# CarloLucibello/GraphNeuralNetworks.jl

Measured on AMD Instinct MI355X. Metric: edges/sec (fwd) GCNConv+GATConv, ogbn-products-shape; achieved HBM GB/s vs peak, higher is better.
Workload: dtype f32; 1 GPU; products-shape power-law graph N=2449029 E=61859140 (+N self loops, E'=64308169), D=100: GCNConv(100=>100,relu) fwd + GATConv(100=>16,heads=8,relu) fwd per step; edges counted = 2*E' per GPU; parallelism=replicas x1 (independent feature batches, no collective)

## Files before the change

graphneuralnetworks.jl_amd/csrc/common.h:

```cpp
#pragma once
#include <hip/hip_runtime.h>

#include <memory>
#include <mutex>
#include <stdint.h>
#include <type_traits>
#include "gnnmp.h"
#include "headgeom.h"
#include "knobs.h"

namespace gnnmp {

int fail(int status, const char *fmt, ...);
int hip_fail(hipError_t e, const char *what);

#define GNNMP_HIP(expr)                                         \
    do {                                                        \
        hipError_t e__ = (expr);                                \
        if (e__ != hipSuccess) return ::gnnmp::hip_fail(e__, #expr); \
    } while (0)

#define GNNMP_TRY(expr)                                         \
    do {                                                        \
        const int rc__ = (expr);                                \
        if (rc__ != GNNMP_OK) return rc__;                      \
    } while (0)

#define GNNMP_LAUNCH_CHECK(what)                                \
    do {                                                        \
        hipError_t e__ = hipGetLastError();                     \
        if (e__ != hipSuccess) return ::gnnmp::hip_fail(e__, what); \
    } while (0)

constexpr int GNNMP_MAX_DEVICES = 32;
int current_device();

struct DeviceOnce {
    std::mutex m;
    unsigned char done[GNNMP_MAX_DEVICES] = {};
    hipError_t err[GNNMP_MAX_DEVICES] = {};
};
template <class F>
inline hipError_t device_once(DeviceOnce &o, F &&f) {
    const int dev = current_device();
    std::lock_guard<std::mutex> lk(o.m);
    if (!o.done[dev]) {
        o.err[dev] = f();
        o.done[dev] = 1;
    }
    return o.err[dev];
}

#define GNNMP_LDS_OPTIN(what, ...)                                                                                            \
    do {                                                                                                                      \
        static ::gnnmp::DeviceOnce once__;                                                                                    \
        const hipError_t err__ = ::gnnmp::device_once(once__, [] {                                                            \
            return hipFuncSetAttribute(reinterpret_cast<const void *>(__VA_ARGS__), hipFuncAttributeMaxDynamicSharedMemorySize, \
                                       160 * 1024);                                                                           \
        });                                                                                                                   \
        if (err__ != hipSuccess) return ::gnnmp::hip_fail(err__, "hipFuncSetAttribute(" what ")");                            \
    } while (0)

int knob(int k);
static_assert(KNOB_FUSED_WAVES == 14 && KNOB_TGCN == 20 && KNOB_EDGE_DOT_GRAD == 21 && KNOB_HETERO == 22, "knobs.h: indices never change");
inline int block_waves(int auto_value) {
    const int w = knob(KNOB_BLOCK_WAVES);
    return w >= 1 && w <= 4 ? w : auto_value;
}
int device_cus();

__device__ __forceinline__ int64_t load_index(const void *p, int64_t k, int idx_bytes, int base) {
    return idx_bytes == 8 ? (reinterpret_cast<const int64_t *>(p)[k] - base)
                          : (static_cast<int64_t>(reinterpret_cast<const int32_t *>(p)[k]) - base);
}
__device__ __forceinline__ void store_index(void *p, int64_t k, int idx_bytes, int64_t v) {
    if (idx_bytes == 8)
        reinterpret_cast<int64_t *>(p)[k] = v;
    else
        reinterpret_cast<int32_t *>(p)[k] = static_cast<int32_t>(v);
}

__host__ __device__ __forceinline__ uint32_t drop_mix32(uint32_t x) {
    x ^= x >> 16; x *= 0x7feb352du; x ^= x >> 15; x *= 0x846ca68bu; x ^= x >> 16;
    return x;
}
__host__ __device__ __forceinline__ uint32_t drop_bits(uint32_t seed_lo, uint32_t seed_hi, uint32_t e, uint32_t h) {
    return drop_mix32(drop_mix32(e ^ seed_lo) ^ (h * 0x9e3779b9u + seed_hi));
}
struct DropArgs {
    uint32_t thr;
    uint32_t seed_lo, seed_hi;
    float inv;
};
__host__ __forceinline__ DropArgs make_drop(float p, uint64_t seed) {
    DropArgs d;
    const double t = (double)p * 4294967296.0;
    d.thr = t >= 4294967295.0 ? 0xffffffffu : (uint32_t)t;
    d.seed_lo = (uint32_t)seed;
    d.seed_hi = (uint32_t)(seed >> 32);
    d.inv = 1.0f / (1.0f - p);
    return d;
}
__device__ __forceinline__ float softmax_exp(float x) { return __builtin_amdgcn_exp2f(x * 1.44269504088896341f); }

__device__ __forceinline__ float hw_max(float x, float y) {
    float r;
    asm("v_max_f32 %0, %1, %2" : "=v"(r) : "v"(x), "v"(y));
    return r;
}
__device__ __forceinline__ float hw_min(float x, float y) {
    float r;
    asm("v_min_f32 %0, %1, %2" : "=v"(r) : "v"(x), "v"(y));
    return r;
}
__device__ __forceinline__ float jl_max(float x, float y) {
    const float m = hw_max(x, y);
    const float nan_pick = (x != x) ? x : y;
    return __builtin_isunordered(x, y) ? nan_pick : m;
}
__device__ __forceinline__ float jl_min(float x, float y) {
    const float m = hw_min(x, y);
    const float nan_pick = (x != x) ? x : y;
    return __builtin_isunordered(x, y) ? nan_pick : m;
}

enum { OP_SUM = 0, OP_MAX = 1, OP_MIN = 2 };

template <int OP>
__device__ __forceinline__ float op_identity() {
    return OP == OP_SUM ? 0.0f : (OP == OP_MAX ? -__builtin_inff() : __builtin_inff());
}
template <int OP>
__device__ __forceinline__ float op_apply(float a, float b) {
    if (OP == OP_SUM) return a + b;
    if (OP == OP_MAX) return jl_max(a, b);
    return jl_min(a, b);
}

template <int VEC>
struct Vec;
template <>
struct Vec<4> {
    using T = float4;
    static __device__ __forceinline__ void load(const float *p, float v[4]) {
        float4 t = *reinterpret_cast<const float4 *>(p);
        v[0] = t.x; v[1] = t.y; v[2] = t.z; v[3] = t.w;
    }
    static __device__ __forceinline__ void store(float *p, const float v[4]) {
        *reinterpret_cast<float4 *>(p) = make_float4(v[0], v[1], v[2], v[3]);
    }
};
template <>
struct Vec<2> {
    using T = float2;
    static __device__ __forceinline__ void load(const float *p, float v[2]) {
        float2 t = *reinterpret_cast<const float2 *>(p);
        v[0] = t.x; v[1] = t.y;
    }
    static __device__ __forceinline__ void store(float *p, const float v[2]) {
        *reinterpret_cast<float2 *>(p) = make_float2(v[0], v[1]);
    }
};
template <>
struct Vec<1> {
    using T = float;
    static __device__ __forceinline__ void load(const float *p, float v[1]) { v[0] = *p; }
    static __device__ __forceinline__ void store(float *p, const float v[1]) { *p = v[0]; }
};

#if defined(__HIP_DEVICE_COMPILE__) && !(defined(__gfx942__) || defined(__gfx950__))
#error "libgnnmp's cross-workgroup fold (coh_store / coh_load / coh_publish) relies on gfx942 / gfx950 semantics of s_waitcnt vmcnt and sc1; build with ARCH=gfx950"
#endif
template <int VEC>
__device__ __forceinline__ void coh_store(float *p, const float v[VEC]) {
    if (VEC == 1) {
        __hip_atomic_store(reinterpret_cast<unsigned int *>(p), __float_as_uint(v[0]), __ATOMIC_RELAXED, __HIP_MEMORY_SCOPE_AGENT);
    } else {
#pragma unroll
        for (int q = 0; q < VEC; q += 2) {
            const unsigned long long b = (unsigned long long)__float_as_uint(v[q]) | ((unsigned long long)__float_as_uint(v[q + 1 < VEC ? q + 1 : q]) << 32);
            __hip_atomic_store(reinterpret_cast<unsigned long long *>(p + q), b, __ATOMIC_RELAXED, __HIP_MEMORY_SCOPE_AGENT);
        }
    }
}
template <int VEC>
__device__ __forceinline__ void coh_load(const float *p, float v[VEC]) {
    if (VEC == 1) {
        v[0] = __uint_as_float(__hip_atomic_load(reinterpret_cast<const unsigned int *>(p), __ATOMIC_RELAXED, __HIP_MEMORY_SCOPE_AGENT));
    } else {
#pragma unroll
        for (int q = 0; q < VEC; q += 2) {
            const unsigned long long b = __hip_atomic_load(reinterpret_cast<const unsigned long long *>(p + q), __ATOMIC_RELAXED, __HIP_MEMORY_SCOPE_AGENT);
            v[q] = __uint_as_float((unsigned int)b);
            if (q + 1 < VEC) v[q + 1] = __uint_as_float((unsigned int)(b >> 32));
        }
    }
}
__device__ __forceinline__ void coh_store1(float *p, float v) {
    __hip_atomic_store(reinterpret_cast<unsigned int *>(p), __float_as_uint(v), __ATOMIC_RELAXED, __HIP_MEMORY_SCOPE_AGENT);
}
__device__ __forceinline__ float coh_load1(const float *p) {
    return __uint_as_float(__hip_atomic_load(reinterpret_cast<const unsigned int *>(p), __ATOMIC_RELAXED, __HIP_MEMORY_SCOPE_AGENT));
}
__device__ __forceinline__ void coh_publish() { asm volatile("s_waitcnt vmcnt(0) lgkmcnt(0)" ::: "memory"); }

template <int CTRL>
__device__ __forceinline__ float dpp_mov(float v) {
    return __int_as_float(__builtin_amdgcn_update_dpp(0, __float_as_int(v), CTRL, 0xf, 0xf, true));
}
template <int LPH>
__device__ __forceinline__ float group_sum(float d, int lph) {
    if (LPH == 0) {
        if (lph & 0x10000) {
            const int n = lph & 0xff, G = 1 << ((lph >> 8) & 0xff);
            const int lane = (int)__lane_id(), lig = lane & (G - 1);
            const int hb = lane - lig + (lig / n) * n;
            float s = 0.0f;
            for (int k = 0; k < n; ++k) s += __shfl(d, hb + k, 64);
            return s;
        }
        for (int o = 1; o < lph; o <<= 1) d += __shfl_xor(d, o, 64);
        return d;
    }
    if (LPH >= 2) d += dpp_mov<0xB1>(d);
    if (LPH >= 4) d += dpp_mov<0x4E>(d);
    if (LPH >= 8) d += dpp_mov<0x141>(d);
    if (LPH >= 16) d += dpp_mov<0x140>(d);
    if (LPH >= 32) d += __shfl_xor(d, 16, 64);
    if (LPH >= 64) d += __shfl_xor(d, 32, 64);
    return d;
}

__device__ __forceinline__ int xcd_remap(int b, int cpx, int enabled) {
    return enabled ? (b & 7) * cpx + (b >> 3) : b;
}
__device__ __forceinline__ int xcd_remap_after(int b, int nbc, int cpx) {
    return b < nbc ? b : nbc + (b & 7) * cpx + ((b - nbc) >> 3);
}

}

struct gnnmp_graph {
    int64_t n_src = 0, n_dst = 0, n_edges = 0, n_total = 0;
    int self_loops = 0;
    uint32_t *rowptr = nullptr;
    int32_t *col = nullptr;
    int32_t *eid = nullptr;
    int32_t *long_rows = nullptr;
    int32_t *long_cptr = nullptr;
    int32_t *chunk_row = nullptr;
    uint32_t *chunk_beg = nullptr;
    uint32_t *chunk_end = nullptr;
    int n_long = 0;
    int n_chunks = 0;
    int long_thresh = GNNMP_LONG_ROW;
    int64_t max_degree = 0;
    int64_t bytes = 0;
    float *ws = nullptr;
    size_t ws_floats = 0;
    uint32_t *ticket = nullptr;
    int32_t *row_order = nullptr;
    int32_t *chunk_lrow = nullptr;
    uint32_t *arrive = nullptr;
    size_t arrive_n = 0;
    float *spart = nullptr;
    size_t spart_floats = 0;
    void *block = nullptr;
    size_t block_bytes = 0;
    int32_t *status = nullptr;
};

namespace gnnmp {
struct __attribute__((visibility("hidden"))) PlanDeleter {
    void operator()(gnnmp_graph *p) const { (void)gnnmp_plan_destroy(p); }
};
using PlanPtr = std::unique_ptr<gnnmp_graph, PlanDeleter>;
int ensure_workspace(gnnmp_graph *p, size_t floats);
int ensure_arrive(gnnmp_graph *p, size_t n, size_t floats, hipStream_t stream);
bool fold_disabled_by_env();
inline bool use_fold() { return (knob(KNOB_VARIANT) & VARIANT_TWO_KERNEL_FOLD) == 0 && !fold_disabled_by_env(); }
int ensure_ticket(gnnmp_graph *p, hipStream_t stream);
int ensure_row_order(gnnmp_graph *p, hipStream_t stream);
int plan_build_long_rows(gnnmp_graph *p, hipStream_t stream);
int plan_long_thresh(int64_t Etot);
}

namespace gnnmp {
inline int pick_vec(int64_t D, const void *a, const void *b) {
    uintptr_t m = reinterpret_cast<uintptr_t>(a) | reinterpret_cast<uintptr_t>(b);
    int forced = knob(KNOB_FORCE_VEC);
    int v = 1;
    if (D % 4 == 0 && (m & 15) == 0)
        v = 4;
    else if (D % 2 == 0 && (m & 7) == 0)
        v = 2;
    if (forced == 1 || forced == 2 || forced == 4) {
        if (forced <= v) v = forced;
    }
    return v;
}
inline bool use_xcd_remap(int64_t n_src, int64_t D, int64_t chunks) {
    const int k = knob(KNOB_XCD_REMAP);
    if (k == 0 || chunks < 64) return false;
    if (k == 2) return true;
    return n_src * D * (int64_t)sizeof(float) <= ((int64_t)128 << 20);
}
inline bool use_row_order(int64_t n_src, int64_t D) {
    const int k = knob(KNOB_ROW_ORDER);
    if (k == 0) return false;
    if (k == 2) return true;
    return n_src * D * (int64_t)sizeof(float) > ((int64_t)128 << 20);
}
inline int pick_log2g(int64_t lanes_needed) {
    int forced = knob(KNOB_FORCE_LOG2G);
    if (forced >= 0 && forced <= 6) return forced;
    int l = 0;
    while ((1 << l) < lanes_needed && l < 6) ++l;
    return l;
}
inline int feature_tiles(int64_t D, int vec, int log2g) {
    const int64_t G = (int64_t)1 << log2g;
    return (int)(((D + vec - 1) / vec + G - 1) / G);
}
template <class... P>
inline int narrow_vec(int vec, const P *...ptr) {
    uintptr_t m = 0;
    ((m |= reinterpret_cast<uintptr_t>(ptr)), ...);
    return (m & (uintptr_t)(4 * vec - 1)) != 0 ? 1 : vec;
}
template <int V>
using int_c = std::integral_constant<int, V>;
template <class F>
inline auto with_vec(int vec, F &&f) {
    switch (vec) {
        case 4: return f(int_c<4>{});
        case 2: return f(int_c<2>{});
        default: return f(int_c<1>{});
    }
}
template <int VEC, int MAX, class F>
inline auto with_lph(int lph, F &&f) {
    if constexpr (VEC == 4) {
        switch (lph <= MAX ? lph : 0) {
            case 1: return f(int_c<1>{});
            case 2: return f(int_c<2>{});
            case 4: return f(int_c<4>{});
            case 8: return f(int_c<8>{});
            case 16: return f(int_c<16>{});
            case 32: return f(int_c<(MAX >= 32 ? 32 : 0)>{});
            case 64: return f(int_c<(MAX >= 64 ? 64 : 0)>{});
        }
    }
    return f(int_c<0>{});
}
template <class F>
inline auto with_op(int op, F &&f) {
    switch (op) {
        case OP_SUM: return f(int_c<OP_SUM>{});
        case OP_MAX: return f(int_c<OP_MAX>{});
        default: return f(int_c<OP_MIN>{});
    }
}
template <class F>
inline auto with_log2g(int log2g, F &&f) {
    switch (log2g) {
        case 0: return f(int_c<0>{});
        case 1: return f(int_c<1>{});
        case 2: return f(int_c<2>{});
        case 3: return f(int_c<3>{});
        case 4: return f(int_c<4>{});
        case 5: return f(int_c<5>{});
        default: return f(int_c<6>{});
    }
}
}
```

graphneuralnetworks.jl_amd/csrc/knobs.h:

```cpp
#pragma once

#define GNNMP_KNOB_TABLE(X)                                                                                                          \
    X(FORCE_VEC, 0, 0, "0 = auto, else 1|2|4")                                                                                       \
    X(FORCE_LOG2G, 1, -1, "-1 = auto, else 0..6")                                                                                    \
    X(UNROLL, 2, 0, "0 = auto (8: measured best on both bench shapes), else 2|4|8")                                                  \
    X(XCD_REMAP, 3, 1, "0 = off, 1 = auto (default: only when the gathered matrix fits the Infinity Cache), 2 = on")                 \
    X(LONG_ROW, 4, 0, "long-row threshold (0 = auto, at most GNNMP_LONG_ROW)")                                                       \
    X(BLOCK_WAVES, 5, 0, "waves per block in the row kernels: 0 = auto (propagate 4, GAT 1), else 1..4")                             \
    X(DENSE_GENERIC, 6, 0, "0 = auto (dense_plan's whole order, dense_route.h), any other value = never dense_wreg, dense_split, "    \
                           "dense_t16 or dense_narrow (the round-1 kernels only); 1 = not the W-resident 32x32x2 kernel either: "     \
                           "K-chunked on every shape")                                                                               \
    X(DENSE_PREFETCH, 7, 17, "W-resident dense kernel scheduling: bit 4 = per-SIMD matrix-pipe token, low 4 bits = start skew of "   \
                             "waves 4-7 in s_sleep(127) units.  Default 17 (token + 1): 0.83 -> 0.72 ms at 2.4M x 100 => 100.  "     \
                             "Bit 5 = turn the cross-tile register prefetch OFF (on by default; its first version spilled, 270 "     \
                             "VGPRs, and was slower: see dense.hip)")                                                                \
    X(GAT_FAST_EXP, 8, 0, "reserved (retired: the one-pass attention kernel always uses v_exp_f32 now, gat_fused.hip gexp)")         \
    X(GRADW_SLABS, 9, 0, "dW kernel: slabs per CU (0 = auto)")                                                                       \
    X(GRADW_RP, 10, 0, "dW kernel: 0 = the 16x16x4 kernel, < 0 = the round-1 32x32x2 kernel (A/B runs)")                             \
    X(GRADW_MIN_ROWS, 11, 0, "dW kernel: rows-per-slab floor (0 = auto: ~3 slabs per CU on small inputs, 512 on large)")             \
    X(DENSE_T16_WAVES, 12, 0, "dense_t16_kernel: waves per block (0 = auto, else 1..16)")                                            \
    X(T16_DEBUG, 13, 0, "GNNMP_EXPERIMENTS builds only (gnnmp_tune refuses a non-zero value otherwise): phase ablation of "          \
                        "dense_t16_kernel / fused_cat_kernel (1 = no stores, 2 = no x loads, ...: the results are garbage), and the " \
                        "variant number of dense_split_kernel")                                                                      \
    X(FUSED_WAVES, 14, 0, "fused_conv_kernel: 0 = auto (as many waves as LDS holds tiles for, <= 16), > 0 = cap, < 0 = never fuse "  \
                          "- read by the host too (gnnmp/layers.py)")                                                                \
    X(ROW_ORDER, 15, 0, "rows by decreasing length in the row kernels that share a wave between rows: 0 = never, 1 = when the "      \
                        "gathered matrix exceeds the Infinity Cache, 2 = always (use_row_order)")                                    \
    X(SOFTMAX_ROWS, 16, 0, "one-pass narrow-row softmax (softmax_rows.hip): 0 = auto, < 0 = the three-step kernels on every row")    \
    X(DENSE_SPLIT, 17, 0, "split-bf16 dense core (msplit.h, dense_split.hip): 0 = auto (on for its shapes), < 0 = the fp32-MFMA "    \
                          "kernels of rounds 1-2 on every shape")                                                                    \
    X(CHAIN, 18, 0, "fused GraphConv chain kernel (graph_chain.hip): 0 = auto, < 0 = never (layer-by-layer path)")                   \
    X(VARIANT, 19, 0, "A/B switches, a bit field of the VARIANT_* constants below (all variants are correct code)")                  \
    X(TGCN, 20, 0, "TGCN recurrence (temporal.hip): 0 = auto (the one-launch kernel for out <= 128), < 0 = the per-step path (dense " \
                   "launches + the step pointwise kernels, every out) - read by the host layer (gnnmp/layers_temporal.py)")          \
    X(EDGE_DOT_GRAD, 21, 0, "adjoint of the per-edge dot product (linkpred.hip): 0 = auto (the fused kernel for D <= 256), < 0 = "   \
                            "two w_mul_xj propagates (plan and transposed plan) plus an add - read by the host (gnnmp/linkpred.py)") \
    X(HETERO, 22, 0, "heterograph aggregation (hetero.hip): 0 = auto (one hetero_rows_kernel launch per layer, and "                 \
                     "HeteroGraphConv's transform-first path), < 0 = the composition: propagate per relation, then the same kernel " \
                     "over identity relations as the combiner, the A/B baseline - read by the host (gnnmp/hetero.py)")               \
    X(CHUNK_SLOTS, 23, 0, "slots per chunk of a split row, read at plan build (plan.hip: plan_chunk_slots): 0 or anything below "    \
                          "16 = the default of 128; the plan's long-row threshold still caps it")

namespace gnnmp {

enum Knob {
#define GNNMP_KNOB_ENUM(name, index, def, doc) KNOB_##name = index,
    GNNMP_KNOB_TABLE(GNNMP_KNOB_ENUM)
#undef GNNMP_KNOB_ENUM
#define GNNMP_KNOB_ONE(name, index, def, doc) +1
    KNOB_COUNT = 0 GNNMP_KNOB_TABLE(GNNMP_KNOB_ONE)
#undef GNNMP_KNOB_ONE
};

enum Variant {
    VARIANT_CHAIN_WAVES_MASK = 3,
    VARIANT_CHAIN_8_WAVES = 1,
    VARIANT_SPLIT_SERIAL_TILES = 16,
    VARIANT_SPLIT_DIRECT_STORES = 32,
    VARIANT_NO_WREG = 64,
    VARIANT_TWO_KERNEL_FOLD = 128,
    VARIANT_WREG_SMALL = 512,
};

}

#ifdef GNNMP_EXPERIMENTS
#define GNNMP_ABLATION(bits) (bits)
#else
#define GNNMP_ABLATION(bits) 0
#endif
```

graphneuralnetworks.jl_amd/csrc/plan.hip:

```cpp
#include <cstring>
#include <algorithm>
#include <vector>

#include "common.h"
#include "launch.h"
#include "pool.h"
#include "scratch.h"
#include "sort_scan.h"

namespace gnnmp {

int ensure_workspace(gnnmp_graph *p, size_t floats) { return grow(p->ws, p->ws_floats, floats, "hipMalloc(plan workspace)"); }

int ensure_arrive(gnnmp_graph *p, size_t n, size_t floats, hipStream_t stream) {
    GNNMP_TRY(grow(p->spart, p->spart_floats, floats, "hipMalloc(plan slice partials)"));
    if (n <= p->arrive_n) return GNNMP_OK;
    GNNMP_TRY(grow(p->arrive, p->arrive_n, n, "hipMalloc(plan arrival counters)"));
    const hipError_t e = hipMemsetAsync(p->arrive, 0, sizeof(uint32_t) * n, stream);
    if (e != hipSuccess) {
        p->arrive_n = 0;
        return hip_fail(e, "hipMemsetAsync(plan arrival counters)");
    }
    return GNNMP_OK;
}

int ensure_ticket(gnnmp_graph *p, hipStream_t stream) {
    if (p->ticket) return GNNMP_OK;
    size_t cap = 0;
    GNNMP_TRY(grow(p->ticket, cap, 2, "hipMalloc(plan ticket)"));
    const hipError_t e = hipMemsetAsync(p->ticket, 0, 2 * sizeof(uint32_t), stream);
    if (e != hipSuccess) return hip_fail(e, "hipMemsetAsync(plan ticket)");
    return GNNMP_OK;
}

__global__ void plan_degree_keys(const uint32_t *rowptr, int64_t n, uint32_t maxdeg, uint32_t *keys, uint32_t *vals) {
    int64_t i = (int64_t)blockIdx.x * blockDim.x + threadIdx.x;
    if (i >= n) return;
    keys[i] = maxdeg - (rowptr[i + 1] - rowptr[i]);
    vals[i] = (uint32_t)i;
}

int ensure_row_order(gnnmp_graph *p, hipStream_t stream) {
    if (p->row_order || p->n_dst == 0) return GNNMP_OK;
    const size_t n = (size_t)p->n_dst;
    unsigned bits = 1;
    while (bits < 32 && ((int64_t)1 << bits) <= p->max_degree) ++bits;
    DevBuf<int32_t> order;
    DevBuf<uint32_t> vin, kout, kin;
    hipError_t e = hipSuccess;
    if ((e = kin.alloc(n)) != hipSuccess || (e = kout.alloc(n)) != hipSuccess || (e = vin.alloc(n)) != hipSuccess ||
        (e = order.alloc(n)) != hipSuccess)
        return hip_fail(e, "hipMalloc(row order)");
    plan_degree_keys<<<(unsigned)((n + 255) / 256), 256, 0, stream>>>(p->rowptr, p->n_dst, (uint32_t)p->max_degree, kin.get(), vin.get());
    GNNMP_TRY(radix_sort_pairs_u32(kin.get(), kout.get(), vin.get(), reinterpret_cast<uint32_t *>(order.get()), n, 0, (int)bits,
                                   stream));
    p->row_order = order.release();
    p->bytes += (int64_t)(4 * n);
    return GNNMP_OK;
}


__global__ void plan_fill_keys(const void *src, const void *dst, int idx_bytes, int base, int64_t E,
                               int64_t Etot, int64_t n_src, int64_t n_dst, uint32_t *keys,
                               uint32_t *vals, int *bad) {
    int64_t k = (int64_t)blockIdx.x * blockDim.x + threadIdx.x;
    if (k >= Etot) return;
    int64_t d;
    if (k < E) {
        d = load_index(dst, k, idx_bytes, base);
        int64_t s = load_index(src, k, idx_bytes, base);
        if (d < 0 || d >= n_dst || s < 0 || s >= n_src) {
            *bad = 1;
            d = 0;
        }
    } else {
        d = k - E;
    }
    keys[k] = (uint32_t)d;
    vals[k] = (uint32_t)k;
}

__global__ void plan_rowptr(const uint32_t *keys, int64_t Etot, int64_t n_dst, uint32_t *rowptr) {
    int64_t i = (int64_t)blockIdx.x * blockDim.x + threadIdx.x;
    if (i > n_dst) return;
    int64_t lo = 0, hi = Etot;
    while (lo < hi) {
        int64_t mid = (lo + hi) >> 1;
        if ((int64_t)keys[mid] < i)
            lo = mid + 1;
        else
            hi = mid;
    }
    rowptr[i] = (uint32_t)lo;
}

__global__ void plan_col(const void *src, int idx_bytes, int base, int64_t E, int64_t Etot,
                         const uint32_t *eid, int32_t *col) {
    int64_t p = (int64_t)blockIdx.x * blockDim.x + threadIdx.x;
    if (p >= Etot) return;
    int64_t e = eid[p];
    int64_t s = e < E ? load_index(src, e, idx_bytes, base) : e - E;
    col[p] = (int32_t)s;
}

__global__ void csc_rowptr_kernel(const void *colptr, int idx_bytes, int base, int64_t n_dst, int64_t E, uint32_t *rowptr, int *bad) {
    int64_t i = (int64_t)blockIdx.x * blockDim.x + threadIdx.x;
    if (i > n_dst) return;
    const int64_t v = load_index(colptr, i, idx_bytes, base);
    bool ok = v >= 0 && v <= E;
    if (i == 0) ok = ok && v == 0;
    if (i == n_dst) ok = ok && v == E;
    if (i < n_dst) ok = ok && load_index(colptr, i + 1, idx_bytes, base) >= v;
    if (!ok) *bad = 1;
    rowptr[i] = (uint32_t)(ok ? v : (i == n_dst ? E : 0));
}
__global__ void csc_col_kernel(const void *rowval, int idx_bytes, int base, int64_t E, int64_t n_src, int32_t *col, int32_t *eid, int *bad) {
    int64_t p = (int64_t)blockIdx.x * blockDim.x + threadIdx.x;
    if (p >= E) return;
    int64_t s = load_index(rowval, p, idx_bytes, base);
    if (s < 0 || s >= n_src) {
        *bad = 1;
        s = 0;
    }
    col[p] = (int32_t)s;
    eid[p] = (int32_t)(uint32_t)p;
}

__global__ void plan_long_rows(const uint32_t *rowptr, int64_t n_dst, int thresh, int64_t *list,
                               int cap, int *count, unsigned long long *maxdeg) {
    int64_t i = (int64_t)blockIdx.x * blockDim.x + threadIdx.x;
    if (i >= n_dst) return;
    const int64_t beg = rowptr[i], end = rowptr[i + 1];
    const int64_t len = end - beg;
    if (len > 0) atomicMax(maxdeg, (unsigned long long)len);
    if (len > thresh) {
        int pos = atomicAdd(count, 1);
        if (pos < cap) {
            list[3 * pos] = i;
            list[3 * pos + 1] = beg;
            list[3 * pos + 2] = end;
        }
    }
}
__global__ void widen_u32_kernel(const uint32_t *in, int64_t n, int64_t *out) {
    int64_t i = (int64_t)blockIdx.x * blockDim.x + threadIdx.x;
    if (i < n) out[i] = (int64_t)in[i];
}

__global__ void slot_gather_kernel(const int32_t *idx, const float *v, int64_t Etot, int64_t n_valid,
                                   float *out) {
    int64_t p = (int64_t)blockIdx.x * blockDim.x + threadIdx.x;
    if (p >= Etot) return;
    const int64_t k = (uint32_t)idx[p];
    out[p] = k < n_valid ? v[k] : 1.0f;
}

__global__ void self_loops_kernel(const void *src, const void *dst, int idx_bytes, int base,
                                  int64_t E, int64_t n, void *out_src, void *out_dst,
                                  const float *w, float *out_w) {
    int64_t k = (int64_t)blockIdx.x * blockDim.x + threadIdx.x;
    if (k >= E + n) return;
    if (k < E) {
        store_index(out_src, k, idx_bytes, load_index(src, k, idx_bytes, 0));
        store_index(out_dst, k, idx_bytes, load_index(dst, k, idx_bytes, 0));
        if (out_w) out_w[k] = w[k];
    } else {
        int64_t v = (k - E) + base;
        store_index(out_src, k, idx_bytes, v);
        store_index(out_dst, k, idx_bytes, v);
        if (out_w) out_w[k] = 1.0f;
    }
}

__global__ void batch_edges_kernel(const void *src, const void *dst, int idx_bytes,
                                   const int64_t *edge_ptr, const int64_t *node_ptr, int64_t G,
                                   int64_t Etot, void *out_src, void *out_dst) {
    int64_t k = (int64_t)blockIdx.x * blockDim.x + threadIdx.x;
    if (k >= Etot) return;
    int64_t lo = 0, hi = G;
    while (hi - lo > 1) {
        int64_t mid = (lo + hi) >> 1;
        if (edge_ptr[mid] <= k)
            lo = mid;
        else
            hi = mid;
    }
    int64_t off = node_ptr[lo];
    store_index(out_src, k, idx_bytes, load_index(src, k, idx_bytes, 0) + off);
    store_index(out_dst, k, idx_bytes, load_index(dst, k, idx_bytes, 0) + off);
}
__global__ void batch_indicator_kernel(const int64_t *node_ptr, int64_t G, int64_t Ntot,
                                       int idx_bytes, int base, void *gi) {
    int64_t v = (int64_t)blockIdx.x * blockDim.x + threadIdx.x;
    if (v >= Ntot) return;
    int64_t lo = 0, hi = G;
    while (hi - lo > 1) {
        int64_t mid = (lo + hi) >> 1;
        if (node_ptr[mid] <= v)
            lo = mid;
        else
            hi = mid;
    }
    store_index(gi, v, idx_bytes, lo + base);
}

static inline unsigned nblocks(int64_t n, int bs) { return (unsigned)((n + bs - 1) / bs); }

int plan_long_thresh(int64_t Etot) {
    if (knob(KNOB_LONG_ROW) > 0) return knob(KNOB_LONG_ROW);
    int th = GNNMP_MIN_LONG_ROW;
    while (th < GNNMP_LONG_ROW && (double)th < 4e-5 * (double)Etot) th <<= 1;
    return th;
}

static int plan_chunk_slots() {
    const int v = knob(KNOB_CHUNK_SLOTS);
    return v >= 16 ? v : 128;
}

int plan_build_long_rows(gnnmp_graph *p, hipStream_t stream) {
    const int64_t n_dst = p->n_dst, Etot = p->n_total;
    const int BS = 256;
    const int cap = (int)std::min<int64_t>(Etot / std::max(1, p->long_thresh) + 1, n_dst + 1);
    DevBuf<int64_t> long_tmp;
    DevBuf<int> flags;
    GNNMP_HIP(flags.alloc(4));
    GNNMP_HIP(hipMemsetAsync(flags.get(), 0, sizeof(int) * 4, stream));
    GNNMP_HIP(long_tmp.alloc(3 * (size_t)std::max(cap, 1)));
    if (n_dst > 0) {
        plan_long_rows<<<nblocks(n_dst, BS), BS, 0, stream>>>(p->rowptr, n_dst, p->long_thresh, long_tmp.get(), cap, flags.get(),
                                                              reinterpret_cast<unsigned long long *>(flags.get() + 2));
        GNNMP_HIP(hipGetLastError());
    }
    int meta[4] = {0, 0, 0, 0};
    GNNMP_HIP(hipMemcpyAsync(meta, flags.get(), sizeof(int) * 4, hipMemcpyDeviceToHost, stream));
    GNNMP_HIP(hipStreamSynchronize(stream));
    unsigned long long md;
    memcpy(&md, meta + 2, sizeof(md));
    p->max_degree = (int64_t)md;
    p->n_long = std::min(meta[0], cap);
    if (p->n_long == 0) return GNNMP_OK;
    struct Tri { int64_t row, beg, end; };
    std::vector<Tri> h((size_t)p->n_long);
    GNNMP_HIP(hipMemcpy(h.data(), long_tmp.get(), sizeof(Tri) * h.size(), hipMemcpyDeviceToHost));
    std::sort(h.begin(), h.end(), [](const Tri &a, const Tri &b) { return a.row < b.row; });
    std::vector<int32_t> rows, cptr, crow, clrow;
    std::vector<uint32_t> cbeg, cend;
    cptr.push_back(0);
    const int64_t clen = std::min<int64_t>(p->long_thresh, plan_chunk_slots());
    for (const Tri &t : h) {
        const int64_t len = t.end - t.beg;
        const int64_t nch = (len + clen - 1) / clen;
        const int64_t csz = (len + nch - 1) / nch;
        for (int64_t c = 0; c < nch; ++c) {
            crow.push_back((int32_t)t.row);
            clrow.push_back((int32_t)rows.size());
            cbeg.push_back((uint32_t)(t.beg + c * csz));
            cend.push_back((uint32_t)std::min(t.beg + (c + 1) * csz, t.end));
        }
        rows.push_back((int32_t)t.row);
        cptr.push_back((int32_t)crow.size());
    }
    if (crow.size() >= (size_t)INT32_MAX)
        return fail(GNNMP_EUNSUPPORTED, "plan_create: %zu chunks of split rows exceed the int32 chunk index", crow.size());
    p->n_chunks = (int)crow.size();
    auto upload = [&](auto *&dst, const auto &v) -> hipError_t {
        const size_t bytes = sizeof(v[0]) * v.size();
        const hipError_t e = alloc_into(dst, v.size());
        if (e != hipSuccess) return e;
        p->bytes += (int64_t)bytes;
        return hipMemcpy(dst, v.data(), bytes, hipMemcpyHostToDevice);
    };
    GNNMP_HIP(upload(p->long_rows, rows));
    GNNMP_HIP(upload(p->long_cptr, cptr));
    GNNMP_HIP(upload(p->chunk_row, crow));
    GNNMP_HIP(upload(p->chunk_lrow, clrow));
    GNNMP_HIP(upload(p->chunk_beg, cbeg));
    GNNMP_HIP(upload(p->chunk_end, cend));
    return GNNMP_OK;
}

}

using namespace gnnmp;

extern "C" {

int gnnmp_plan_destroy(gnnmp_graph_t *p) { return plan_dispose(p, nullptr, false); }

int gnnmp_plan_reset_counters(gnnmp_graph_t *p, gnnmp_stream_t stream_) {
    hipStream_t stream = (hipStream_t)stream_;
    if (!p) return fail(GNNMP_EINVAL, "plan_reset_counters: null plan");
    if (p->arrive && p->arrive_n) GNNMP_HIP(hipMemsetAsync(p->arrive, 0, sizeof(uint32_t) * p->arrive_n, stream));
    if (p->ticket) GNNMP_HIP(hipMemsetAsync(p->ticket, 0, 2 * sizeof(uint32_t), stream));
    return GNNMP_OK;
}

int gnnmp_plan_release(gnnmp_graph_t *p, gnnmp_stream_t stream) { return plan_dispose(p, (hipStream_t)stream, true); }

}

namespace gnnmp {
int plan_dispose(gnnmp_graph_t *p, hipStream_t stream, bool stream_known) {
    if (!p) return GNNMP_OK;
    if (p->block) {
        pool_park(p->block, p->block_bytes, stream, stream_known);
        p->rowptr = nullptr;
        p->col = nullptr;
        p->eid = nullptr;
    }
    void *const owned[] = {p->rowptr, p->col, p->eid, p->long_rows, p->long_cptr, p->chunk_row, p->chunk_lrow, p->arrive, p->spart,
                           p->chunk_beg, p->chunk_end, p->ws, p->ticket, p->row_order};
    for (void *q : owned)
        if (q) (void)dev_free(q);
    delete p;
    return GNNMP_OK;
}
int check_transposed(const char *who, const gnnmp_graph_t *plan, const gnnmp_graph_t *plan_t) {
    if (plan_t->n_dst != plan->n_src || plan_t->n_src != plan->n_dst || plan_t->n_total != plan->n_total)
        return fail(GNNMP_EINVAL, "%s: plan_t is not the transpose of plan (%lld x %lld, %lld edges vs %lld x %lld, %lld)", who,
                    (long long)plan_t->n_dst, (long long)plan_t->n_src, (long long)plan_t->n_total,
                    (long long)plan->n_dst, (long long)plan->n_src, (long long)plan->n_total);
    return GNNMP_OK;
}
}

extern "C" {

int gnnmp_plan_create(gnnmp_graph_t **out, const void *src, const void *dst, int idx_bytes,
                      int index_base, int64_t n_src, int64_t n_dst, int64_t n_edges,
                      int add_self_loops, int validate, gnnmp_stream_t stream_) {
    hipStream_t stream = (hipStream_t)stream_;
    if (!out) return fail(GNNMP_EINVAL, "plan_create: out is NULL");
    *out = nullptr;
    if (idx_bytes != 4 && idx_bytes != 8)
        return fail(GNNMP_EINVAL, "plan_create: idx_bytes must be 4 or 8 (got %d)", idx_bytes);
    if (index_base != 0 && index_base != 1)
        return fail(GNNMP_EINVAL, "plan_create: index_base must be 0 or 1 (got %d)", index_base);
    if (n_src < 0 || n_dst < 0 || n_edges < 0)
        return fail(GNNMP_EINVAL, "plan_create: negative size");
    if (n_edges > 0 && (!src || !dst)) return fail(GNNMP_EINVAL, "plan_create: null edge index");
    if (add_self_loops && n_src != n_dst)
        return fail(GNNMP_EINVAL, "plan_create: add_self_loops needs n_src == n_dst (%lld vs %lld)",
                    (long long)n_src, (long long)n_dst);
    const int64_t Etot = n_edges + (add_self_loops ? n_dst : 0);
    if (Etot >= (int64_t)GNNMP_MAX_SLOTS || n_src >= (int64_t)INT32_MAX || n_dst >= (int64_t)INT32_MAX)
        return fail(GNNMP_EUNSUPPORTED, "plan_create: E' = %lld (limit 2^32 - 65536) / N = %lld (limit 2^31 - 2) exceed the plan format",
                    (long long)Etot, (long long)std::max(n_src, n_dst));

    PlanPtr p(new gnnmp_graph_t());
    p->n_src = n_src;
    p->n_dst = n_dst;
    p->n_edges = n_edges;
    p->n_total = Etot;
    p->self_loops = add_self_loops ? 1 : 0;
    p->long_thresh = plan_long_thresh(Etot);

    const int BS = 256;
    const size_t epad = (size_t)std::max<int64_t>(Etot, 1);
    DevBuf<int> flags;
    DevBuf<unsigned char> sort_keys;
    uint32_t *keys_out = nullptr;
    GNNMP_HIP(alloc_into(p->rowptr, (size_t)(n_dst + 1)));
    GNNMP_HIP(alloc_into(p->col, epad));
    GNNMP_HIP(alloc_into(p->eid, epad));
    GNNMP_HIP(flags.alloc(4));
    GNNMP_HIP(hipMemsetAsync(flags.get(), 0, sizeof(int) * 4, stream));
    p->bytes = (int64_t)(sizeof(int32_t) * ((size_t)(n_dst + 1) + 2 * epad));

    if (Etot > 0) {
        const size_t piece = (sizeof(uint32_t) * epad + 255) & ~(size_t)255;
        GNNMP_HIP(sort_keys.alloc(3 * piece));
        uint32_t *keys_in = reinterpret_cast<uint32_t *>(sort_keys.get());
        keys_out = reinterpret_cast<uint32_t *>(sort_keys.get() + piece);
        uint32_t *vals_in = reinterpret_cast<uint32_t *>(sort_keys.get() + 2 * piece);
        plan_fill_keys<<<nblocks(Etot, BS), BS, 0, stream>>>(src, dst, idx_bytes, index_base,
                                                             n_edges, Etot, n_src, n_dst, keys_in,
                                                             vals_in, flags.get());
        GNNMP_HIP(hipGetLastError());
        if (validate) {
            int bad = 0;
            GNNMP_HIP(hipMemcpyAsync(&bad, flags.get(), sizeof(int), hipMemcpyDeviceToHost, stream));
            GNNMP_HIP(hipStreamSynchronize(stream));
            if (bad)
                return fail(GNNMP_EBOUNDS, "plan_create: edge index outside 1..N (n_src=%lld n_dst=%lld)",
                            (long long)n_src, (long long)n_dst);
        }
        unsigned bits = 1;
        while (bits < 32 && ((int64_t)1 << bits) < n_dst) ++bits;
        GNNMP_TRY(radix_sort_pairs_u32(keys_in, keys_out, vals_in, reinterpret_cast<uint32_t *>(p->eid), (size_t)Etot, 0, (int)bits,
                                       stream));
        plan_col<<<nblocks(Etot, BS), BS, 0, stream>>>(src, idx_bytes, index_base, n_edges, Etot,
                                                       reinterpret_cast<uint32_t *>(p->eid), p->col);
        GNNMP_HIP(hipGetLastError());
    }
    plan_rowptr<<<nblocks(n_dst + 1, BS), BS, 0, stream>>>(keys_out, Etot, n_dst, p->rowptr);
    GNNMP_HIP(hipGetLastError());

    GNNMP_TRY(plan_build_long_rows(p.get(), stream));
    *out = p.release();
    return GNNMP_OK;
}

int gnnmp_plan_from_csc(gnnmp_graph_t **out, const void *colptr, const void *rowval, int idx_bytes, int index_base, int64_t n_src,
                        int64_t n_dst, int64_t n_edges, int validate, gnnmp_stream_t stream_) {
    hipStream_t stream = (hipStream_t)stream_;
    if (!out) return fail(GNNMP_EINVAL, "plan_from_csc: out is NULL");
    *out = nullptr;
    if (idx_bytes != 4 && idx_bytes != 8) return fail(GNNMP_EINVAL, "plan_from_csc: idx_bytes must be 4 or 8 (got %d)", idx_bytes);
    if (index_base != 0 && index_base != 1) return fail(GNNMP_EINVAL, "plan_from_csc: index_base must be 0 or 1 (got %d)", index_base);
    if (n_src < 0 || n_dst < 0 || n_edges < 0) return fail(GNNMP_EINVAL, "plan_from_csc: negative size");
    if (!colptr || (n_edges > 0 && !rowval)) return fail(GNNMP_EINVAL, "plan_from_csc: null colptr / rowval");
    if (n_edges >= (int64_t)GNNMP_MAX_SLOTS || n_src >= (int64_t)INT32_MAX || n_dst >= (int64_t)INT32_MAX)
        return fail(GNNMP_EUNSUPPORTED, "plan_from_csc: E = %lld (limit 2^32 - 65536) / N = %lld (limit 2^31 - 2) exceed the plan format",
                    (long long)n_edges, (long long)std::max(n_src, n_dst));
    PlanPtr p(new gnnmp_graph_t());
    p->n_src = n_src;
    p->n_dst = n_dst;
    p->n_edges = n_edges;
    p->n_total = n_edges;
    p->long_thresh = plan_long_thresh(n_edges);
    const int BS = 256;
    const size_t epad = (size_t)std::max<int64_t>(n_edges, 1);
    DevBuf<int> flags;
    GNNMP_HIP(alloc_into(p->rowptr, (size_t)(n_dst + 1)));
    GNNMP_HIP(alloc_into(p->col, epad));
    GNNMP_HIP(alloc_into(p->eid, epad));
    GNNMP_HIP(flags.alloc(4));
    GNNMP_HIP(hipMemsetAsync(flags.get(), 0, sizeof(int) * 4, stream));
    p->bytes = (int64_t)(sizeof(int32_t) * ((size_t)(n_dst + 1) + 2 * epad));
    csc_rowptr_kernel<<<nblocks(n_dst + 1, BS), BS, 0, stream>>>(colptr, idx_bytes, index_base, n_dst, n_edges, p->rowptr, flags.get());
    GNNMP_HIP(hipGetLastError());
    if (n_edges > 0) {
        csc_col_kernel<<<nblocks(n_edges, BS), BS, 0, stream>>>(rowval, idx_bytes, index_base, n_edges, n_src, p->col, p->eid, flags.get());
        GNNMP_HIP(hipGetLastError());
    }
    (void)validate;
    int bad = 0;
    GNNMP_HIP(hipMemcpyAsync(&bad, flags.get(), sizeof(int), hipMemcpyDeviceToHost, stream));
    GNNMP_HIP(hipStreamSynchronize(stream));
    if (bad)
        return fail(GNNMP_EBOUNDS, "plan_from_csc: colptr is not a monotone 0..E column pointer, or a row index lies outside 1..n_src "
                    "(n_src=%lld n_dst=%lld E=%lld)", (long long)n_src, (long long)n_dst, (long long)n_edges);
    GNNMP_TRY(plan_build_long_rows(p.get(), stream));
    *out = p.release();
    return GNNMP_OK;
}

int gnnmp_plan_slot_gather_f32(gnnmp_graph_t *p, int by, const float *v, float *out_slot,
                               gnnmp_stream_t stream_) {
    hipStream_t stream = (hipStream_t)stream_;
    if (!p) return fail(GNNMP_EINVAL, "plan_slot_gather: null plan");
    if (by != 0 && by != 1) return fail(GNNMP_EINVAL, "plan_slot_gather: `by` must be 0 (node) or 1 (edge)");
    if (p->n_total == 0) return GNNMP_OK;
    if (!v || !out_slot) return fail(GNNMP_EINVAL, "plan_slot_gather: null pointer");
    if (by == 0)
        slot_gather_kernel<<<nblocks(p->n_total, 256), 256, 0, stream>>>(p->col, v, p->n_total, p->n_src, out_slot);
    else
        slot_gather_kernel<<<nblocks(p->n_total, 256), 256, 0, stream>>>(p->eid, v, p->n_total, p->n_edges, out_slot);
    GNNMP_LAUNCH_CHECK("slot_gather_kernel");
    return GNNMP_OK;
}

int gnnmp_plan_info(const gnnmp_graph_t *p, int64_t info[8]) {
    if (!p || !info) return fail(GNNMP_EINVAL, "plan_info: null argument");
    info[0] = p->n_src;
    info[1] = p->n_dst;
    info[2] = p->n_edges;
    info[3] = p->n_total;
    info[4] = p->max_degree;
    info[5] = p->n_long;
    info[6] = p->bytes;
    info[7] = p->long_thresh;
    return GNNMP_OK;
}

int gnnmp_plan_export(const gnnmp_graph_t *p, int32_t *rowptr, int32_t *col, int32_t *eid,
                      gnnmp_stream_t stream_) {
    hipStream_t stream = (hipStream_t)stream_;
    if (!p) return fail(GNNMP_EINVAL, "plan_export: null plan");
    if (p->n_total > (int64_t)INT32_MAX)
        return fail(GNNMP_EUNSUPPORTED, "plan_export: E' = %lld does not fit int32 rowptr / eid (use gnnmp_plan_export64)",
                    (long long)p->n_total);
    if (rowptr)
        GNNMP_HIP(hipMemcpyAsync(rowptr, p->rowptr, sizeof(int32_t) * (size_t)(p->n_dst + 1), hipMemcpyDeviceToDevice, stream));
    if (col && p->n_total > 0)
        GNNMP_HIP(hipMemcpyAsync(col, p->col, sizeof(int32_t) * (size_t)p->n_total,
                                 hipMemcpyDeviceToDevice, stream));
    if (eid && p->n_total > 0)
        GNNMP_HIP(hipMemcpyAsync(eid, p->eid, sizeof(int32_t) * (size_t)p->n_total,
                                 hipMemcpyDeviceToDevice, stream));
    return GNNMP_OK;
}

int gnnmp_plan_export64(const gnnmp_graph_t *p, int64_t *rowptr, int32_t *col, uint32_t *eid, gnnmp_stream_t stream_) {
    hipStream_t stream = (hipStream_t)stream_;
    if (!p) return fail(GNNMP_EINVAL, "plan_export64: null plan");
    if (rowptr) {
        widen_u32_kernel<<<nblocks(p->n_dst + 1, 256), 256, 0, stream>>>(p->rowptr, p->n_dst + 1, rowptr);
        GNNMP_LAUNCH_CHECK("widen_u32_kernel");
    }
    if (col && p->n_total > 0)
        GNNMP_HIP(hipMemcpyAsync(col, p->col, sizeof(int32_t) * (size_t)p->n_total, hipMemcpyDeviceToDevice, stream));
    if (eid && p->n_total > 0)
        GNNMP_HIP(hipMemcpyAsync(eid, p->eid, sizeof(uint32_t) * (size_t)p->n_total, hipMemcpyDeviceToDevice, stream));
    return GNNMP_OK;
}

int gnnmp_add_self_loops(const void *src, const void *dst, int idx_bytes, int index_base,
                         int64_t n_edges, int64_t n, void *out_src, void *out_dst, const float *w,
                         float *out_w, gnnmp_stream_t stream_) {
    hipStream_t stream = (hipStream_t)stream_;
    if (idx_bytes != 4 && idx_bytes != 8) return fail(GNNMP_EINVAL, "add_self_loops: idx_bytes %d", idx_bytes);
    if (index_base != 0 && index_base != 1) return fail(GNNMP_EINVAL, "add_self_loops: index_base %d", index_base);
    if (n_edges < 0 || n < 0) return fail(GNNMP_EINVAL, "add_self_loops: negative size");
    if ((w != nullptr && out_w == nullptr) || (w == nullptr && out_w != nullptr && n_edges > 0))
        return fail(GNNMP_EINVAL, "add_self_loops: w and out_w must both be NULL or both non-NULL");
    if (n_edges + n == 0) return GNNMP_OK;
    if (!out_src || !out_dst || (n_edges > 0 && (!src || !dst)))
        return fail(GNNMP_EINVAL, "add_self_loops: null pointer");
    self_loops_kernel<<<nblocks(n_edges + n, 256), 256, 0, stream>>>(
        src, dst, idx_bytes, index_base, n_edges, n, out_src, out_dst, w, out_w);
    GNNMP_LAUNCH_CHECK("self_loops_kernel");
    return GNNMP_OK;
}

int gnnmp_batch_coo(const void *src, const void *dst, int idx_bytes, int index_base,
                    const int64_t *edge_ptr, const int64_t *node_ptr, int64_t n_graphs,
                    void *out_src, void *out_dst, void *graph_indicator, gnnmp_stream_t stream_) {
    hipStream_t stream = (hipStream_t)stream_;
    if (idx_bytes != 4 && idx_bytes != 8) return fail(GNNMP_EINVAL, "batch_coo: idx_bytes %d", idx_bytes);
    if (index_base != 0 && index_base != 1) return fail(GNNMP_EINVAL, "batch_coo: index_base %d", index_base);
    if (n_graphs <= 0 || !edge_ptr || !node_ptr) return fail(GNNMP_EINVAL, "batch_coo: bad graph table");
    int64_t tot[2] = {0, 0};
    GNNMP_HIP(hipMemcpyAsync(&tot[0], edge_ptr + n_graphs, sizeof(int64_t), hipMemcpyDeviceToHost, stream));
    GNNMP_HIP(hipMemcpyAsync(&tot[1], node_ptr + n_graphs, sizeof(int64_t), hipMemcpyDeviceToHost, stream));
    GNNMP_HIP(hipStreamSynchronize(stream));
    if (tot[0] > 0) {
        if (!src || !dst || !out_src || !out_dst) return fail(GNNMP_EINVAL, "batch_coo: null edge arrays");
        batch_edges_kernel<<<nblocks(tot[0], 256), 256, 0, stream>>>(
            src, dst, idx_bytes, edge_ptr, node_ptr, n_graphs, tot[0], out_src, out_dst);
        GNNMP_LAUNCH_CHECK("batch_edges_kernel");
    }
    if (tot[1] > 0 && graph_indicator) {
        batch_indicator_kernel<<<nblocks(tot[1], 256), 256, 0, stream>>>(
            node_ptr, n_graphs, tot[1], idx_bytes, index_base, graph_indicator);
        GNNMP_LAUNCH_CHECK("batch_indicator_kernel");
    }
    return GNNMP_OK;
}

}
```

graphneuralnetworks.jl_amd/csrc/pool.h:

```cpp
#pragma once
#include <hip/hip_runtime.h>
#include <stddef.h>

namespace gnnmp {
bool pool_take(void **out, size_t *cap, size_t bytes, hipStream_t stream);
void pool_park(void *p, size_t cap, hipStream_t stream, bool stream_known);
int pool_pick(const size_t *caps, int n, size_t bytes);
void pool_trim();
}
```

graphneuralnetworks.jl_amd/csrc/pool.hip:

```cpp
#include <mutex>

#include "pool.h"
#include "common.h"

namespace gnnmp {
namespace {
struct Parked {
    void *p = nullptr;
    size_t cap = 0;
    hipStream_t stream = nullptr;
    hipEvent_t ev = nullptr;
};
constexpr int POOL_SLOTS = 8;
struct DevicePool {
    Parked slots[POOL_SLOTS];
    hipEvent_t free_events[POOL_SLOTS] = {};
    int n_free_events = 0;
};
DevicePool g_pools[GNNMP_MAX_DEVICES];
std::mutex g_lock;

hipEvent_t event_get(DevicePool &dp) {
    if (dp.n_free_events > 0) return dp.free_events[--dp.n_free_events];
    hipEvent_t e = nullptr;
    if (hipEventCreateWithFlags(&e, hipEventDisableTiming) != hipSuccess) return nullptr;
    return e;
}
void event_put(DevicePool &dp, hipEvent_t e) {
    if (!e) return;
    if (dp.n_free_events < POOL_SLOTS) dp.free_events[dp.n_free_events++] = e;
    else (void)hipEventDestroy(e);
}
bool same_stream(hipStream_t a, hipStream_t b) { return a == b && a != hipStreamPerThread; }
}

int pool_pick(const size_t *caps, int n, size_t bytes) {
    int best = -1;
    for (int i = 0; i < n; ++i)
        if (caps[i] && caps[i] >= bytes && (best < 0 || caps[i] < caps[best])) best = i;
    if (best >= 0 && caps[best] <= 2 * bytes + (1 << 20)) return best;
    return -1;
}

bool pool_take(void **out, size_t *cap, size_t bytes, hipStream_t stream) {
    DevicePool &dp = g_pools[current_device()];
    Parked got;
    {
        std::lock_guard<std::mutex> lk(g_lock);
        size_t caps[POOL_SLOTS];
        for (int i = 0; i < POOL_SLOTS; ++i) caps[i] = dp.slots[i].p ? dp.slots[i].cap : 0;
        const int best = pool_pick(caps, POOL_SLOTS, bytes);
        if (best >= 0) {
            got = dp.slots[best];
            dp.slots[best] = Parked();
        }
    }
    if (got.p) {
        bool ok = true;
        if (!got.ev) {
            ok = hipDeviceSynchronize() == hipSuccess;
        } else {
            if (!same_stream(got.stream, stream)) ok = hipStreamWaitEvent(stream, got.ev, 0) == hipSuccess;
            std::lock_guard<std::mutex> lk(g_lock);
            event_put(dp, got.ev);
        }
        if (ok) {
            *out = got.p;
            *cap = got.cap;
            return true;
        }
        (void)hipFree(got.p);
    }
    *cap = bytes;
    return hipMalloc(out, bytes) == hipSuccess;
}

void pool_park(void *p, size_t cap, hipStream_t stream, bool stream_known) {
    if (!p) return;
    int dev = current_device();
    {
        hipPointerAttribute_t at;
        if (hipPointerGetAttributes(&at, p) == hipSuccess && at.device >= 0 && at.device < GNNMP_MAX_DEVICES) {
            if (at.device != dev) stream_known = false;
            dev = at.device;
        } else {
            (void)hipGetLastError();
        }
    }
    DevicePool &dp = g_pools[dev];
    Parked in;
    in.p = p;
    in.cap = cap;
    Parked evict;
    {
        std::lock_guard<std::mutex> lk(g_lock);
        if (stream_known) {
            in.stream = stream;
            in.ev = event_get(dp);
            if (in.ev && hipEventRecord(in.ev, stream) != hipSuccess) {
                (void)hipGetLastError();
                event_put(dp, in.ev);
                in.ev = nullptr;
            }
        }
        int slot = -1;
        for (int i = 0; i < POOL_SLOTS; ++i)
            if (!dp.slots[i].p) { slot = i; break; }
        if (slot < 0) {
            slot = 0;
            for (int i = 1; i < POOL_SLOTS; ++i)
                if (dp.slots[i].cap < dp.slots[slot].cap) slot = i;
            if (dp.slots[slot].cap >= cap) {
                evict = in;
                in = Parked();
            } else {
                evict = dp.slots[slot];
            }
        }
        if (in.p) dp.slots[slot] = in;
        if (evict.ev) { event_put(dp, evict.ev); evict.ev = nullptr; }
    }
    if (evict.p) (void)hipFree(evict.p);
}

void pool_trim() {
    for (int d = 0; d < GNNMP_MAX_DEVICES; ++d) {
        Parked all[POOL_SLOTS];
        bool any = false;
        {
            std::lock_guard<std::mutex> lk(g_lock);
            DevicePool &dp = g_pools[d];
            for (int i = 0; i < POOL_SLOTS; ++i) {
                all[i] = dp.slots[i];
                dp.slots[i] = Parked();
                if (all[i].ev) event_put(dp, all[i].ev);
                any = any || all[i].p;
            }
        }
        if (!any) continue;
        for (int i = 0; i < POOL_SLOTS; ++i)
            if (all[i].p) (void)hipFree(all[i].p);
    }
}
}
```

graphneuralnetworks.jl_amd/csrc/runtime.hip:

```cpp
#include <cstdarg>
#include <cstdio>
#include <cstdlib>
#include <atomic>

#include "common.h"
#include "pool.h"

namespace gnnmp {

static thread_local char g_err[512] = "";
#define GNNMP_KNOB_INDEX(name, index, def, doc) index,
#define GNNMP_KNOB_DEFAULT(name, index, def, doc) def,
#define GNNMP_KNOB_NAME(name, index, def, doc) #name,
static constexpr int g_knob_index[KNOB_COUNT] = {GNNMP_KNOB_TABLE(GNNMP_KNOB_INDEX)};
static constexpr int g_knob_defaults[KNOB_COUNT] = {GNNMP_KNOB_TABLE(GNNMP_KNOB_DEFAULT)};
[[maybe_unused]] static const char *const g_knob_names[KNOB_COUNT] = {GNNMP_KNOB_TABLE(GNNMP_KNOB_NAME)};
static int g_knobs[KNOB_COUNT] = {GNNMP_KNOB_TABLE(GNNMP_KNOB_DEFAULT)};
#undef GNNMP_KNOB_INDEX
#undef GNNMP_KNOB_DEFAULT
#undef GNNMP_KNOB_NAME
constexpr bool knob_table_is_dense() {
    for (int i = 0; i < KNOB_COUNT; ++i)
        if (g_knob_index[i] != i) return false;
    return true;
}
static_assert(knob_table_is_dense(), "knobs.h: the X(...) entries must be listed in index order, 0 .. KNOB_COUNT - 1, without gaps");

int fail(int status, const char *fmt, ...) {
    va_list ap;
    va_start(ap, fmt);
    vsnprintf(g_err, sizeof(g_err), fmt, ap);
    va_end(ap);
    return status;
}
int hip_fail(hipError_t e, const char *what) {
    snprintf(g_err, sizeof(g_err), "HIP error %d (%s) at %s", (int)e, hipGetErrorString(e), what);
    return e == hipErrorOutOfMemory ? GNNMP_EALLOC : GNNMP_ELAUNCH;
}
int knob(int k) { return (k >= 0 && k < KNOB_COUNT) ? g_knobs[k] : 0; }
static thread_local int g_mock_device = -1;
int current_device() {
    if (g_mock_device >= 0) return g_mock_device < GNNMP_MAX_DEVICES ? g_mock_device : GNNMP_MAX_DEVICES - 1;
    int dev = 0;
    if (hipGetDevice(&dev) != hipSuccess || dev < 0) dev = 0;
    return dev < GNNMP_MAX_DEVICES ? dev : GNNMP_MAX_DEVICES - 1;
}
int device_cus() {
    static std::atomic<int> cached[GNNMP_MAX_DEVICES] = {};
    const int dev = current_device();
    int cus = cached[dev].load(std::memory_order_relaxed);
    if (cus == 0) {
        cus = 256;
        if (hipDeviceGetAttribute(&cus, hipDeviceAttributeMultiprocessorCount, dev) != hipSuccess || cus <= 0) cus = 256;
        cached[dev].store(cus, std::memory_order_relaxed);
    }
    return cus;
}

bool fold_disabled_by_env() {
    static const bool off = [] {
        const char *e = getenv("GNNMP_NO_FOLD");
        return e && *e && *e != '0';
    }();
    return off;
}

}

using namespace gnnmp;

extern "C" {

int gnnmp_version(void) { return GNNMP_VERSION; }
const char *gnnmp_last_error(void) { return g_err; }

int gnnmp_tune(int k, int value) {
    if (k < 0 || k >= KNOB_COUNT) return fail(GNNMP_EINVAL, "gnnmp_tune: bad knob %d", k);
#ifndef GNNMP_EXPERIMENTS
    if (k == KNOB_T16_DEBUG && value != 0)
        return fail(GNNMP_EUNSUPPORTED, "gnnmp_tune: knob %d (%s) selects experiment code that this build does not contain; build the library with "
                                        "-DGNNMP_EXPERIMENTS (make EXPERIMENTS=1)", k, g_knob_names[k]);
#endif
    g_knobs[k] = value;
    return GNNMP_OK;
}
int gnnmp_tune_get(int k, int *value, int *default_value) {
    if (k < 0 || k >= KNOB_COUNT) return fail(GNNMP_EINVAL, "gnnmp_tune_get: bad knob %d", k);
    if (value) *value = g_knobs[k];
    if (default_value) *default_value = g_knob_defaults[k];
    return GNNMP_OK;
}

int gnnmp_debug_mock_device(int dev) {
    g_mock_device = dev;
    return current_device();
}
int gnnmp_debug_device_once(const int *devs, int n, int fail_on, int *n_failed) {
    DeviceOnce once;
    int ran = 0, failed = 0;
    const int keep = g_mock_device;
    for (int k = 0; k < n; ++k) {
        g_mock_device = devs[k];
        const hipError_t e = device_once(once, [&] {
            ++ran;
            return current_device() == fail_on ? hipErrorInvalidValue : hipSuccess;
        });
        if (e != hipSuccess) ++failed;
    }
    g_mock_device = keep;
    if (n_failed) *n_failed = failed;
    return ran;
}
void *gnnmp_debug_plan_block(const gnnmp_graph_t *p) { return p ? p->block : nullptr; }
int gnnmp_debug_pool_pick(const uint64_t *caps, int n, uint64_t bytes) {
    size_t c[64];
    if (n < 0 || n > 64) return -2;
    for (int i = 0; i < n; ++i) c[i] = (size_t)caps[i];
    return pool_pick(c, n, (size_t)bytes);
}

}
```

graphneuralnetworks.jl_amd/csrc/scratch.h:

```cpp
#pragma once
#include <stddef.h>
#include <algorithm>
#include "gnnmp.h"

#ifndef GNNMP_SCRATCH_STANDIN
#include "common.h"
namespace gnnmp {
inline hipError_t dev_malloc(void **out, size_t bytes) { return hipMalloc(out, bytes); }
inline hipError_t dev_free(void *p) { return hipFree(p); }
}
#endif

#pragma GCC visibility push(hidden)
namespace gnnmp {

struct PrepBlock { void *p; size_t cap; int dev; };
inline thread_local PrepBlock g_prep_cache[8] = {};
inline hipError_t prep_alloc(void **out, size_t bytes) {
    bytes = std::max<size_t>(bytes, 256);
    const int dev = current_device();
    int best = -1;
    for (int i = 0; i < 8; ++i)
        if (g_prep_cache[i].p && g_prep_cache[i].dev == dev && g_prep_cache[i].cap >= bytes &&
            (best < 0 || g_prep_cache[i].cap < g_prep_cache[best].cap))
            best = i;
    if (best >= 0 && g_prep_cache[best].cap <= 4 * bytes + (1 << 20)) {
        *out = g_prep_cache[best].p;
        g_prep_cache[best] = PrepBlock{nullptr, 0, 0};
        return hipSuccess;
    }
    return dev_malloc(out, bytes);
}
inline void prep_free(void *p, size_t bytes) {
    bytes = std::max<size_t>(bytes, 256);
    const int dev = current_device();
    int slot = -1;
    for (int i = 0; i < 8; ++i)
        if (!g_prep_cache[i].p) { slot = i; break; }
    if (slot < 0) {
        slot = 0;
        for (int i = 1; i < 8; ++i)
            if (g_prep_cache[i].cap < g_prep_cache[slot].cap) slot = i;
        if (g_prep_cache[slot].cap >= bytes) {
            (void)dev_free(p);
            return;
        }
        (void)dev_free(g_prep_cache[slot].p);
    }
    g_prep_cache[slot] = PrepBlock{p, bytes, dev};
}

enum class Scratch { Malloc, PrepCache };

template <class T>
class DevBuf {
public:
    explicit DevBuf(Scratch src = Scratch::Malloc) : src_(src) {}
    DevBuf(DevBuf &&o) noexcept : p_(o.p_), bytes_(o.bytes_), src_(o.src_), synced_(o.synced_) { o.p_ = nullptr; }
    DevBuf &operator=(DevBuf &&o) noexcept {
        if (this != &o) {
            give_back();
            p_ = o.p_;
            bytes_ = o.bytes_;
            src_ = o.src_;
            synced_ = o.synced_;
            o.p_ = nullptr;
        }
        return *this;
    }
    ~DevBuf() { give_back(); }
    hipError_t alloc(size_t n) {
        give_back();
        bytes_ = sizeof(T) * n;
        synced_ = false;
        void *p = nullptr;
        const hipError_t e = src_ == Scratch::PrepCache ? prep_alloc(&p, bytes_) : dev_malloc(&p, bytes_);
        if (e == hipSuccess) p_ = static_cast<T *>(p);
        return e;
    }
    T *get() const { return p_; }
    T *release() {
        T *p = p_;
        p_ = nullptr;
        return p;
    }
    void synced() { synced_ = true; }

private:
    void give_back() {
        if (!p_) return;
        if (src_ == Scratch::PrepCache && synced_)
            prep_free(p_, bytes_);
        else
            (void)dev_free(p_);
        p_ = nullptr;
    }
    T *p_ = nullptr;
    size_t bytes_ = 0;
    Scratch src_;
    bool synced_ = false;
};

template <class T>
inline hipError_t alloc_into(T *&member, size_t n) {
    DevBuf<T> b;
    const hipError_t e = b.alloc(n);
    member = b.release();
    return e;
}

template <class T>
inline int grow(T *&ptr, size_t &cap, size_t need, const char *what) {
    if (need <= cap) return GNNMP_OK;
    if (ptr) (void)dev_free(ptr);
    ptr = nullptr;
    cap = 0;
    const hipError_t e = alloc_into(ptr, need);
    if (e != hipSuccess) return hip_fail(e, what);
    cap = need;
    return GNNMP_OK;
}

}
#pragma GCC visibility pop
```

graphneuralnetworks.jl_amd/csrc/sort_scan.h:

```cpp
#pragma once
#include <hip/hip_runtime.h>
#include <stddef.h>
#include <stdint.h>

namespace gnnmp {
int radix_sort_pairs_u32(const uint32_t *keys_in, uint32_t *keys_out, const uint32_t *vals_in, uint32_t *vals_out, size_t n,
                         int begin_bit, int end_bit, hipStream_t stream);
int radix_sort_keys_u64(const uint64_t *keys_in, uint64_t *keys_out, size_t n, int begin_bit, int end_bit, hipStream_t stream);
int radix_sort_pairs_u64(const uint64_t *keys_in, uint64_t *keys_out, const uint32_t *vals_in, uint32_t *vals_out, size_t n,
                         int begin_bit, int end_bit, hipStream_t stream);
size_t exclusive_scan_workspace(size_t n);
int exclusive_scan_i64(const int64_t *in, int64_t *out, size_t n, hipStream_t stream, int64_t *ws = nullptr);
int exclusive_scan_u32(const uint32_t *in, uint32_t *out, size_t n, hipStream_t stream, uint32_t *ws = nullptr);
}
```

graphneuralnetworks.jl_amd/csrc/sort_scan.hip:

```cpp
#include <algorithm>

#include "common.h"
#include "scratch.h"
#include "sort_scan.h"

namespace gnnmp {

constexpr int RS_WT = 2048;
constexpr int RS_WPB = 4;
constexpr int SC_CHUNK = 4096;

__device__ __forceinline__ void wave_lds_sync() {
    __builtin_amdgcn_fence(__ATOMIC_RELEASE, "wavefront");
    __builtin_amdgcn_wave_barrier();
    __builtin_amdgcn_fence(__ATOMIC_ACQUIRE, "wavefront");
}

template <class K>
__global__ void __launch_bounds__(64 * RS_WPB) rs_hist(const K *__restrict__ keys, size_t n, int shift, uint32_t *__restrict__ counts,
                                                       size_t n_tiles) {
    __shared__ uint32_t h[RS_WPB][256];
    const int lane = threadIdx.x & 63, w = threadIdx.x >> 6;
    const size_t tile = (size_t)blockIdx.x * RS_WPB + w;
    if (tile >= n_tiles) return;
#pragma unroll
    for (int k = 0; k < 4; ++k) h[w][lane + 64 * k] = 0;
    wave_lds_sync();
    const size_t base = tile * RS_WT;
    K kreg[RS_WT / 64];
#pragma unroll
    for (int s = 0; s < RS_WT / 64; ++s) {
        const size_t i = base + (size_t)s * 64 + lane;
        kreg[s] = i < n ? keys[i] : (K)0;
    }
#pragma unroll
    for (int s = 0; s < RS_WT / 64; ++s) {
        const size_t i = base + (size_t)s * 64 + lane;
        if (i < n) atomicAdd(&h[w][(int)((kreg[s] >> shift) & 255)], 1u);
    }
    wave_lds_sync();
#pragma unroll
    for (int k = 0; k < 4; ++k) counts[(size_t)(lane + 64 * k) * n_tiles + tile] = h[w][lane + 64 * k];
}

template <class K, bool PAIRS>
__global__ void __launch_bounds__(64 * RS_WPB) rs_scatter(const K *__restrict__ keys, const uint32_t *__restrict__ vals, size_t n,
                                                          int shift, const uint32_t *__restrict__ offsets, size_t n_tiles,
                                                          K *__restrict__ keys_out, uint32_t *__restrict__ vals_out) {
    constexpr int BT = RS_WT * RS_WPB;
    extern __shared__ __align__(16) unsigned char rs_lds[];
    K *stage_k = reinterpret_cast<K *>(rs_lds);
    uint32_t *stage_v = reinterpret_cast<uint32_t *>(stage_k + BT);
    uint32_t *pos = stage_v + (PAIRS ? BT : 0);
    uint32_t *gstart = pos + 256 * RS_WPB;
    __shared__ uint32_t wsum[RS_WPB];
    const int tid = threadIdx.x, lane = tid & 63, w = tid >> 6;
    const size_t tile0 = (size_t)blockIdx.x * RS_WPB;
    const size_t m = 256 * n_tiles;
    for (int e = tid; e < 256 * RS_WPB; e += 64 * RS_WPB) {
        const int d = e / RS_WPB, ww = e - d * RS_WPB;
        const size_t tile = tile0 + ww;
        uint32_t c = 0;
        if (tile < n_tiles) {
            const size_t idx = (size_t)d * n_tiles + tile;
            const uint32_t lo = offsets[idx], hi = idx + 1 < m ? offsets[idx + 1] : (uint32_t)n;
            c = hi - lo;
            if (ww == 0) gstart[d] = lo;
        }
        pos[e] = c;
    }
    __syncthreads();
    {
        uint32_t c[RS_WPB], tot = 0;
#pragma unroll
        for (int k = 0; k < RS_WPB; ++k) { c[k] = pos[tid * RS_WPB + k]; tot += c[k]; }
        uint32_t inc = tot;
#pragma unroll
        for (int o = 1; o < 64; o <<= 1) {
            const uint32_t u = __shfl_up(inc, o, 64);
            if (lane >= o) inc += u;
        }
        if (lane == 63) wsum[w] = inc;
        __syncthreads();
        uint32_t pre = inc - tot;
        for (int k = 0; k < w; ++k) pre += wsum[k];
#pragma unroll
        for (int k = 0; k < RS_WPB; ++k) { pos[tid * RS_WPB + k] = pre; pre += c[k]; }
    }
    __syncthreads();
    const size_t tile = tile0 + w;
    if (tile < n_tiles) {
        const size_t base = tile * RS_WT;
        const uint64_t lower = (1ull << lane) - 1ull;
        K kreg[RS_WT / 64];
        uint32_t vreg[PAIRS ? RS_WT / 64 : 1];
#pragma unroll
        for (int s = 0; s < RS_WT / 64; ++s) {
            const size_t i = base + (size_t)s * 64 + lane;
            kreg[s] = i < n ? keys[i] : (K)0;
            if (PAIRS) vreg[PAIRS ? s : 0] = i < n ? vals[i] : 0u;
        }
#pragma unroll
        for (int s = 0; s < RS_WT / 64; ++s) {
            const size_t i = base + (size_t)s * 64 + lane;
            const bool valid = i < n;
            const K key = kreg[s];
            const uint32_t val = PAIRS ? vreg[PAIRS ? s : 0] : 0u;
            const int d = (int)((key >> shift) & 255);
            uint64_t same = __ballot(valid);
#pragma unroll
            for (int b = 0; b < 8; ++b) {
                const uint64_t mb = __ballot(valid && ((d >> b) & 1));
                same &= ((d >> b) & 1) ? mb : ~mb;
            }
            const int rank = __popcll(same & lower);
            const uint32_t first = pos[d * RS_WPB + w];
            wave_lds_sync();
            if (valid && rank == 0) pos[d * RS_WPB + w] = first + (uint32_t)__popcll(same);
            wave_lds_sync();
            if (valid) {
                stage_k[first + rank] = key;
                if (PAIRS) stage_v[first + rank] = val;
            }
        }
    }
    __syncthreads();
    const size_t bt_base = tile0 * RS_WT;
    const int valid_n = (int)(n > bt_base ? (n - bt_base < (size_t)BT ? n - bt_base : (size_t)BT) : 0);
    for (int p = tid; p < valid_n; p += 64 * RS_WPB) {
        const K key = stage_k[p];
        const int d = (int)((key >> shift) & 255);
        const uint32_t dfirst = d == 0 ? 0u : pos[(d - 1) * RS_WPB + (RS_WPB - 1)];
        const size_t dst = (size_t)gstart[d] + (uint32_t)p - dfirst;
        keys_out[dst] = key;
        if (PAIRS) vals_out[dst] = stage_v[p];
    }
}

template <class T>
__device__ __forceinline__ T wave_inclusive_scan(T v, int lane) {
#pragma unroll
    for (int o = 1; o < 64; o <<= 1) {
        const T u = __shfl_up(v, o, 64);
        if (lane >= o) v += u;
    }
    return v;
}

template <class T>
__global__ void __launch_bounds__(256) scan_reduce(const T *__restrict__ in, size_t n, T *__restrict__ block_sums) {
    __shared__ T ws[4];
    const size_t base = (size_t)blockIdx.x * SC_CHUNK;
    T s = 0;
    for (int k = 0; k < SC_CHUNK / 256; ++k) {
        const size_t i = base + (size_t)k * 256 + threadIdx.x;
        if (i < n) s += in[i];
    }
    const int lane = threadIdx.x & 63, w = threadIdx.x >> 6;
#pragma unroll
    for (int o = 32; o > 0; o >>= 1) s += __shfl_xor(s, o, 64);
    if (lane == 0) ws[w] = s;
    __syncthreads();
    if (threadIdx.x == 0) block_sums[blockIdx.x] = ws[0] + ws[1] + ws[2] + ws[3];
}

template <class T>
__global__ void __launch_bounds__(1024) scan_block_sums(T *__restrict__ sums, size_t m) {
    __shared__ T ws[16];
    __shared__ T carry_s;
    const int lane = threadIdx.x & 63, w = threadIdx.x >> 6;
    if (threadIdx.x == 0) carry_s = 0;
    __syncthreads();
    for (size_t base = 0; base < m; base += 1024) {
        const size_t i = base + threadIdx.x;
        const T v = i < m ? sums[i] : (T)0;
        const T inc = wave_inclusive_scan(v, lane);
        if (lane == 63) ws[w] = inc;
        __syncthreads();
        T wave_off = 0;
        for (int k = 0; k < w; ++k) wave_off += ws[k];
        const T carry = carry_s;
        if (i < m) sums[i] = carry + wave_off + inc - v;
        __syncthreads();
        if (threadIdx.x == 1023) carry_s = carry + wave_off + inc;
        __syncthreads();
    }
}

template <class T>
__global__ void __launch_bounds__(256) scan_apply(const T *in, size_t n, const T *__restrict__ block_offsets, T *out) {
    __shared__ T ws[4];
    const size_t base = (size_t)blockIdx.x * SC_CHUNK;
    const int lane = threadIdx.x & 63, w = threadIdx.x >> 6;
    T v[SC_CHUNK / 256];
    T tot = 0;
#pragma unroll
    for (int k = 0; k < SC_CHUNK / 256; ++k) {
        const size_t i = base + (size_t)threadIdx.x * (SC_CHUNK / 256) + k;
        v[k] = i < n ? in[i] : (T)0;
        tot += v[k];
    }
    const T inc = wave_inclusive_scan(tot, lane);
    if (lane == 63) ws[w] = inc;
    __syncthreads();
    T pre = block_offsets[blockIdx.x] + inc - tot;
    for (int k = 0; k < w; ++k) pre += ws[k];
#pragma unroll
    for (int k = 0; k < SC_CHUNK / 256; ++k) {
        const size_t i = base + (size_t)threadIdx.x * (SC_CHUNK / 256) + k;
        if (i < n) out[i] = pre;
        pre += v[k];
    }
}

static inline size_t scan_blocks(size_t n) { return (n + SC_CHUNK - 1) / SC_CHUNK; }
template <class T>
static void exclusive_scan_enqueue(const T *in, T *out, size_t n, T *sums, hipStream_t stream) {
    const size_t nb = scan_blocks(n);
    scan_reduce<T><<<(unsigned)nb, 256, 0, stream>>>(in, n, sums);
    scan_block_sums<T><<<1, 1024, 0, stream>>>(sums, nb);
    scan_apply<T><<<(unsigned)nb, 256, 0, stream>>>(in, n, sums, out);
}
template <class T>
static int exclusive_scan_impl(const T *in, T *out, size_t n, hipStream_t stream, T *ws) {
    if (n == 0) return GNNMP_OK;
    if (ws) {
        exclusive_scan_enqueue<T>(in, out, n, ws, stream);
        hipError_t e0 = hipGetLastError();
        if (e0 != hipSuccess) return hip_fail(e0, "exclusive_scan");
        return GNNMP_OK;
    }
    DevBuf<T> sums;
    GNNMP_HIP(sums.alloc(scan_blocks(n)));
    exclusive_scan_enqueue<T>(in, out, n, sums.get(), stream);
    hipError_t e = hipGetLastError();
    if (e == hipSuccess) e = hipStreamSynchronize(stream);
    if (e != hipSuccess) return hip_fail(e, "exclusive_scan");
    return GNNMP_OK;
}

size_t exclusive_scan_workspace(size_t n) { return scan_blocks(n); }
int exclusive_scan_i64(const int64_t *in, int64_t *out, size_t n, hipStream_t stream, int64_t *ws) {
    return exclusive_scan_impl<int64_t>(in, out, n, stream, ws);
}
int exclusive_scan_u32(const uint32_t *in, uint32_t *out, size_t n, hipStream_t stream, uint32_t *ws) {
    return exclusive_scan_impl<uint32_t>(in, out, n, stream, ws);
}

template <class K>
__global__ void __launch_bounds__(256) rs_varying_bits(const K *__restrict__ keys, size_t n, unsigned long long *__restrict__ out) {
    const K k0 = keys[0];
    unsigned long long v = 0;
    for (size_t i = (size_t)blockIdx.x * blockDim.x + threadIdx.x; i < n; i += (size_t)gridDim.x * blockDim.x)
        v |= (unsigned long long)(keys[i] ^ k0);
#pragma unroll
    for (int o = 32; o >= 1; o >>= 1) v |= __shfl_xor(v, o, 64);
    if ((threadIdx.x & 63) == 0 && v) atomicOr(out, v);
}

template <class K, bool PAIRS>
static int radix_sort_impl(const K *keys_in, K *keys_out, const uint32_t *vals_in, uint32_t *vals_out, size_t n, int begin_bit,
                           int end_bit, hipStream_t stream) {
    if (n == 0) return GNNMP_OK;
    if (n >= ((size_t)1 << 32)) return fail(GNNMP_EUNSUPPORTED, "radix sort: %zu elements exceed the 32-bit offset tables", n);
    const int passes = std::max(1, (end_bit - begin_bit + 7) / 8);
    const size_t n_tiles = (n + RS_WT - 1) / RS_WT;
    const size_t m = 256 * n_tiles;
    auto up = [](size_t b) { return (b + 255) & ~(size_t)255; };
    const size_t b_k = up(sizeof(K) * n), b_v = PAIRS ? up(sizeof(uint32_t) * n) : 0, b_c = up(sizeof(uint32_t) * m),
                 b_s = up(sizeof(uint32_t) * scan_blocks(m));
    DevBuf<unsigned char> arena;
    hipError_t e = arena.alloc(b_k + b_v + b_c + b_s + 256);
    if (e != hipSuccess) return hip_fail(e, "hipMalloc(radix sort temporaries)");
    K *ktmp = reinterpret_cast<K *>(arena.get());
    uint32_t *vtmp = PAIRS ? reinterpret_cast<uint32_t *>(arena.get() + b_k) : nullptr;
    uint32_t *counts = reinterpret_cast<uint32_t *>(arena.get() + b_k + b_v);
    uint32_t *sums = reinterpret_cast<uint32_t *>(arena.get() + b_k + b_v + b_c);
    unsigned long long *dvary = reinterpret_cast<unsigned long long *>(arena.get() + b_k + b_v + b_c + b_s), hvary = 0;
    const unsigned blocks = (unsigned)((n_tiles + RS_WPB - 1) / RS_WPB);
    const size_t scatter_lds = (size_t)RS_WT * RS_WPB * (sizeof(K) + (PAIRS ? sizeof(uint32_t) : 0)) + (256 * RS_WPB + 256) * sizeof(uint32_t);
    e = hipFuncSetAttribute(reinterpret_cast<const void *>(&rs_scatter<K, PAIRS>), hipFuncAttributeMaxDynamicSharedMemorySize,
                            (int)scatter_lds);
    if (e != hipSuccess) return hip_fail(e, "hipFuncSetAttribute(rs_scatter)");
    e = hipMemsetAsync(dvary, 0, sizeof(unsigned long long), stream);
    if (e == hipSuccess) {
        const unsigned vb = (unsigned)std::min<size_t>((n + 255) / 256, (size_t)device_cus() * 8);
        rs_varying_bits<K><<<vb, 256, 0, stream>>>(keys_in, n, dvary);
        e = hipMemcpyAsync(&hvary, dvary, sizeof(hvary), hipMemcpyDeviceToHost, stream);
    }
    if (e == hipSuccess) e = hipStreamSynchronize(stream);
    if (e != hipSuccess) return hip_fail(e, "radix sort: varying bits");
    const K *ksrc = keys_in;
    const uint32_t *vsrc = vals_in;
    for (int p = 0; p < passes; ++p) {
        const int shift = begin_bit + 8 * p;
        if (((hvary >> shift) & 255ull) == 0) continue;
        rs_hist<K><<<blocks, 64 * RS_WPB, 0, stream>>>(ksrc, n, shift, counts, n_tiles);
        exclusive_scan_enqueue<uint32_t>(counts, counts, m, sums, stream);
        K *kdst = (ksrc == keys_out) ? ktmp : keys_out;
        uint32_t *vdst = (ksrc == keys_out) ? vtmp : vals_out;
        rs_scatter<K, PAIRS><<<blocks, 64 * RS_WPB, scatter_lds, stream>>>(ksrc, vsrc, n, shift, counts, n_tiles, kdst, vdst);
        e = hipGetLastError();
        if (e != hipSuccess) return hip_fail(e, "radix sort pass");
        ksrc = kdst;
        vsrc = vdst;
    }
    if (ksrc != keys_out) {
        e = hipMemcpyAsync(keys_out, ksrc, sizeof(K) * n, hipMemcpyDeviceToDevice, stream);
        if (e == hipSuccess && PAIRS) e = hipMemcpyAsync(vals_out, vsrc, sizeof(uint32_t) * n, hipMemcpyDeviceToDevice, stream);
        if (e != hipSuccess) return hip_fail(e, "radix sort copy-out");
    }
    e = hipStreamSynchronize(stream);
    if (e != hipSuccess) return hip_fail(e, "radix sort");
    return GNNMP_OK;
}

int radix_sort_pairs_u32(const uint32_t *keys_in, uint32_t *keys_out, const uint32_t *vals_in, uint32_t *vals_out, size_t n,
                         int begin_bit, int end_bit, hipStream_t stream) {
    return radix_sort_impl<uint32_t, true>(keys_in, keys_out, vals_in, vals_out, n, begin_bit, end_bit, stream);
}
int radix_sort_keys_u64(const uint64_t *keys_in, uint64_t *keys_out, size_t n, int begin_bit, int end_bit, hipStream_t stream) {
    return radix_sort_impl<uint64_t, false>(keys_in, keys_out, nullptr, nullptr, n, begin_bit, end_bit, stream);
}
int radix_sort_pairs_u64(const uint64_t *keys_in, uint64_t *keys_out, const uint32_t *vals_in, uint32_t *vals_out, size_t n,
                         int begin_bit, int end_bit, hipStream_t stream) {
    return radix_sort_impl<uint64_t, true>(keys_in, keys_out, vals_in, vals_out, n, begin_bit, end_bit, stream);
}

}
```

graphneuralnetworks.jl_amd/gnnmp/_lib.py:

```python
from __future__ import annotations

import contextlib
import ctypes
import os

from .knobs import Knob, Variant

_PKG = os.path.dirname(os.path.dirname(os.path.abspath(__file__)))
LIB_PATH = os.environ.get("GNNMP_LIB") or os.path.join(_PKG, "lib", "libgnnmp.so")

OK, EINVAL, EBOUNDS, EALLOC, ELAUNCH, EUNSUPPORTED = 0, -1, -2, -3, -4, -5
SUM, MEAN, MAX, MIN = 0, 1, 2, 3
COPY_XJ, W_MUL_XJ = 0, 1
ACT_IDENTITY, ACT_RELU, ACT_SOFTPLUS, ACT_TANH, ACT_SWISH = 0, 1, 2, 3, 4
LONG_ROW = 512

SYMBOLS = (
    "gnnmp_version", "gnnmp_last_error",
    "gnnmp_plan_create", "gnnmp_plan_from_csc", "gnnmp_plan_destroy", "gnnmp_plan_info", "gnnmp_plan_export", "gnnmp_plan_export64",
    "gnnmp_plan_concat", "gnnmp_plan_select", "gnnmp_plan_release", "gnnmp_plan_status", "gnnmp_plan_edge_index",
    "gnnmp_chain_jobs_pack", "gnnmp_chain_jobs_release", "gnnmp_chain_jobs_export",
    "gnnmp_arena_create", "gnnmp_arena_destroy", "gnnmp_arena_alloc", "gnnmp_arena_reset", "gnnmp_arena_class_of", "gnnmp_arena_info",
    "gnnmp_add_self_loops", "gnnmp_batch_coo",
    "gnnmp_sort_edge_index", "gnnmp_is_bidirected", "gnnmp_has_self_loops", "gnnmp_sample_neighbors",
    "gnnmp_unique_append", "gnnmp_induced_subgraph",
    "gnnmp_gather_f32", "gnnmp_edge_sub_f32", "gnnmp_scatter_f32", "gnnmp_scatter_atomic_f32",
    "gnnmp_propagate_f32", "gnnmp_propagate_emul_f32", "gnnmp_propagate_gated_f32", "gnnmp_propagate_slots_f32", "gnnmp_propagate_slots_act_f32", "gnnmp_plan_slot_gather_f32",
    "gnnmp_degree_f32", "gnnmp_inv_sqrt_f32",
    "gnnmp_edge_softmax_f32", "gnnmp_segment_softmax_f32", "gnnmp_gat_node_scores_f32", "gnnmp_gat_aggregate_f32", "gnnmp_gat_conv_f32",
    "gnnmp_gat_conv_edge_f32", "gnnmp_gat_conv_stats_f32", "gnnmp_gat_conv_grad_f32", "gnnmp_attn_conv_f32",
    "gnnmp_gat_conv_train_f32", "gnnmp_gat_conv_grad2_f32",
    "gnnmp_gat_conv_drop_f32", "gnnmp_dropout_keep_u8", "gnnmp_gat_conv_grad_drop_f32", "gnnmp_attn_conv_drop_f32", "gnnmp_attn_conv_grad_drop_f32",
    "gnnmp_attn_conv_grad_f32",
    "gnnmp_bias_act_f32",
    "gnnmp_segment_pool_f32", "gnnmp_segment_bounds", "gnnmp_segment_pool_ptr_f32", "gnnmp_dense_f32", "gnnmp_fused_conv_f32",
    "gnnmp_graphconv_chain_scratch_floats", "gnnmp_graphconv_chain_f32", "gnnmp_chain_jobs_create", "gnnmp_chain_jobs_destroy",
    "gnnmp_chain_jobs_info", "gnnmp_shard_by_size", "gnnmp_allgather_f32",
    "gnnmp_edge_dot_f32", "gnnmp_edge_dot_plan_f32", "gnnmp_propagate_maxmin_grad_f32",
    "gnnmp_head_mean_f32", "gnnmp_head_mean_grad_f32", "gnnmp_add_f32", "gnnmp_axpy_f32", "gnnmp_mul_rows_f32", "gnnmp_is_sorted",
    "gnnmp_act_grad_f32", "gnnmp_dense_grad_workspace", "gnnmp_dense_grad_w_f32",
    "gnnmp_dense_grad_w2_workspace", "gnnmp_dense_grad_w2_f32", "gnnmp_pool_grad_act_f32", "gnnmp_propagate_add_mask_f32",
    "gnnmp_row_normalize_f32", "gnnmp_row_normalize_grad_f32", "gnnmp_propagate_cg_f32", "gnnmp_gru_pointwise_f32", "gnnmp_propagate_nn_f32", "gnnmp_gmm_weights_f32", "gnnmp_row_sqnorm_normalize_f32", "gnnmp_lstm_pointwise_f32", "gnnmp_rowdot_f32",
    "gnnmp_plan_reset_counters",
    "gnnmp_propagate_f64", "gnnmp_gather_f64", "gnnmp_scatter_f64",
    "gnnmp_tgcn_recurrence_f32", "gnnmp_tgcn_recurrence_grad_f32", "gnnmp_tgcn_step_f32", "gnnmp_tgcn_step_grad_f32",
    "gnnmp_negative_sample", "gnnmp_rand_edge_split", "gnnmp_edge_dot_grad_f32",
    "gnnmp_knn_graph_f32", "gnnmp_radius_graph_f32",
    "gnnmp_hetero_propagate_f32", "gnnmp_hetero_propagate_grad_f32",
    "gnnmp_coalesce_edges", "gnnmp_compact_edges", "gnnmp_has_multi_edges", "gnnmp_has_isolated_nodes",
    "gnnmp_random_walk_pe_f32",
    "gnnmp_edge_conv_f32", "gnnmp_edge_conv_grad_f32", "gnnmp_cg_conv_grad_f32",
    "gnnmp_tune", "gnnmp_tune_get", "gnnmp_debug_mock_device", "gnnmp_debug_device_once", "gnnmp_debug_plan_block", "gnnmp_debug_pool_pick",
    "gnnmp_debug_random_walk_pe_f32", "gnnmp_debug_dense_route",
)


HETERO_MAX_REL = 16


class HeteroRel(ctypes.Structure):
    _fields_ = [("plan", ctypes.c_void_p), ("x", ctypes.c_void_p), ("w", ctypes.c_void_p), ("aggr", ctypes.c_int)]


class HeteroDst(ctypes.Structure):
    _fields_ = [("out", ctypes.c_void_p), ("n_dst", ctypes.c_int64), ("combine", ctypes.c_int), ("n_rel", ctypes.c_int),
                ("rels", ctypes.POINTER(HeteroRel))]


class HeteroRelGrad(ctypes.Structure):
    _fields_ = [("plan_t", ctypes.c_void_p), ("dy", ctypes.c_void_p), ("w", ctypes.c_void_p), ("sd", ctypes.c_void_p),
                ("y", ctypes.c_void_p), ("out", ctypes.c_void_p)]


class HeteroSrc(ctypes.Structure):
    _fields_ = [("dx", ctypes.c_void_p), ("x", ctypes.c_void_p), ("n_src", ctypes.c_int64), ("n_rel", ctypes.c_int),
                ("rels", ctypes.POINTER(HeteroRelGrad))]


COALESCE_DIRECTED, COALESCE_MIRRORED, COALESCE_UNDIRECTED = 0, 1, 2
COMPACT_SELF_LOOPS, COMPACT_LIST, COMPACT_RANDOM = 0, 1, 2


class CoalesceJob(ctypes.Structure):
    _fields_ = [("s", ctypes.c_void_p), ("t", ctypes.c_void_p), ("idx_bytes", ctypes.c_int), ("index_base", ctypes.c_int),
                ("n_edges", ctypes.c_int64), ("n_nodes", ctypes.c_int64), ("mode", ctypes.c_int), ("s_out", ctypes.c_void_p),
                ("t_out", ctypes.c_void_p), ("colptr", ctypes.c_void_p), ("rowval", ctypes.c_void_p)]


class CompactJob(ctypes.Structure):
    _fields_ = [("s", ctypes.c_void_p), ("t", ctypes.c_void_p), ("w", ctypes.c_void_p), ("idx_bytes", ctypes.c_int),
                ("index_base", ctypes.c_int), ("n_edges", ctypes.c_int64), ("rule", ctypes.c_int), ("remove", ctypes.c_void_p),
                ("n_remove", ctypes.c_int64), ("p", ctypes.c_float), ("seed", ctypes.c_uint64), ("s_out", ctypes.c_void_p),
                ("t_out", ctypes.c_void_p), ("w_out", ctypes.c_void_p), ("eid_out", ctypes.c_void_p)]


RWPE_TILE, RWPE_MAX_WALK = 16, 1024


class RwpeJob(ctypes.Structure):
    _fields_ = [("w", ctypes.c_void_p), ("graph_ptr", ctypes.c_void_p), ("idx_bytes", ctypes.c_int), ("n_graphs", ctypes.c_int64),
                ("walk_length", ctypes.c_int64), ("out", ctypes.c_void_p)]


class EdgeConvJob(ctypes.Structure):
    _fields_ = [("p", ctypes.c_void_p), ("y", ctypes.c_void_p), ("aggr", ctypes.c_int), ("act", ctypes.c_int)]


class EdgeConvGradJob(ctypes.Structure):
    _fields_ = [("p", ctypes.c_void_p), ("y", ctypes.c_void_p), ("dy", ctypes.c_void_p), ("dp", ctypes.c_void_p),
                ("aggr", ctypes.c_int), ("act", ctypes.c_int)]


class CGConvGradJob(ctypes.Structure):
    _fields_ = [("fs_i", ctypes.c_void_p), ("fs_j", ctypes.c_void_p), ("fs_e", ctypes.c_void_p), ("dy", ctypes.c_void_p),
                ("dfs_i", ctypes.c_void_p), ("dfs_j", ctypes.c_void_p), ("dfs_e", ctypes.c_void_p), ("act", ctypes.c_int)]


class GnnmpError(RuntimeError):
    def __init__(self, status, msg):
        super().__init__(f"libgnnmp status {status}: {msg}")
        self.status = status


_lib = None


def load():
    global _lib
    if _lib is not None:
        return _lib
    if not os.path.exists(LIB_PATH):
        raise ImportError(
            f"{LIB_PATH} not found: build it with `python -c 'import __graft_entry__ as g; g.build()'` "
            "(hipcc --offload-arch=gfx950).  gnnmp has no CPU fallback.")
    L = ctypes.CDLL(LIB_PATH)
    vp, i, i64, f = ctypes.c_void_p, ctypes.c_int, ctypes.c_int64, ctypes.c_float
    u64 = ctypes.c_uint64
    L.gnnmp_version.restype = i
    L.gnnmp_last_error.restype = ctypes.c_char_p
    sig = {
        "gnnmp_plan_create": [ctypes.POINTER(vp), vp, vp, i, i, i64, i64, i64, i, i, vp],
        "gnnmp_plan_from_csc": [ctypes.POINTER(vp), vp, vp, i, i, i64, i64, i64, i, vp],
        "gnnmp_plan_destroy": [vp],
        "gnnmp_plan_info": [vp, ctypes.POINTER(i64)],
        "gnnmp_plan_export": [vp, vp, vp, vp, vp],
        "gnnmp_plan_export64": [vp, vp, vp, vp, vp],
        "gnnmp_plan_concat": [ctypes.POINTER(vp), ctypes.POINTER(vp), i64, vp, vp, i, i, vp],
        "gnnmp_plan_select": [ctypes.POINTER(vp), vp, vp, i64, vp, i, i, i64, i64, i64, vp, vp, vp, vp],
        "gnnmp_plan_release": [vp, vp],
        "gnnmp_plan_status": [vp, vp],
        "gnnmp_plan_edge_index": [vp, i, i, vp, vp, vp],
        "gnnmp_chain_jobs_pack": [ctypes.POINTER(vp), vp, i64, i64, i64, i, vp],
        "gnnmp_chain_jobs_release": [vp, vp],
        "gnnmp_chain_jobs_export": [vp, vp, i64, vp, vp],
        "gnnmp_arena_create": [ctypes.POINTER(vp), i64, i, i64, vp],
        "gnnmp_arena_destroy": [vp],
        "gnnmp_arena_alloc": [vp, i, i64, ctypes.POINTER(vp)],
        "gnnmp_arena_reset": [vp],
        "gnnmp_arena_class_of": [vp, vp, i64, ctypes.POINTER(i), vp],
        "gnnmp_arena_info": [vp, ctypes.POINTER(i64)],
        "gnnmp_add_self_loops": [vp, vp, i, i, i64, i64, vp, vp, vp, vp, vp],
        "gnnmp_batch_coo": [vp, vp, i, i, vp, vp, i64, vp, vp, vp, vp],
        "gnnmp_sort_edge_index": [vp, vp, i, i, i64, vp, vp, vp],
        "gnnmp_is_bidirected": [vp, vp, i, i, i64, ctypes.POINTER(i), vp],
        "gnnmp_has_self_loops": [vp, vp, i, i64, ctypes.POINTER(i), vp],
        "gnnmp_sample_neighbors": [vp, vp, i, i, i64, i64, i, ctypes.c_uint64, vp, vp, i64, ctypes.POINTER(i64), vp],
        "gnnmp_unique_append": [vp, vp, i64, vp, i, i, i64, i64, vp, ctypes.POINTER(i64), vp],
        "gnnmp_induced_subgraph": [vp, vp, vp, i, i, i64, vp, vp, vp, vp, i64, ctypes.POINTER(i64), vp],
        "gnnmp_gather_f32": [vp, vp, i, i, i64, vp, i64, vp],
        "gnnmp_edge_sub_f32": [vp, vp, vp, vp, i, i, i64, i, vp, i64, vp],
        "gnnmp_scatter_f32": [vp, i, vp, vp, i64, vp],
        "gnnmp_scatter_atomic_f32": [i, vp, vp, i, i, i64, vp, i64, vp],
        "gnnmp_propagate_f32": [vp, i, i, vp, vp, vp, vp, vp, i64, vp],
        "gnnmp_propagate_emul_f32": [vp, i, vp, vp, vp, i64, vp],
        "gnnmp_propagate_gated_f32": [vp, i, vp, vp, vp, i64, vp],
        "gnnmp_propagate_slots_f32": [vp, i, vp, vp, vp, vp, vp, i64, vp],
        "gnnmp_propagate_slots_act_f32": [vp, i, vp, vp, vp, vp, vp, i, vp, i64, vp],
        "gnnmp_plan_slot_gather_f32": [vp, i, vp, vp, vp],
        "gnnmp_gat_conv_f32": [vp, vp, vp, vp, f, vp, i, vp, i64, i64, vp],
        "gnnmp_gat_conv_edge_f32": [vp, vp, vp, vp, vp, f, vp, i, vp, i64, i64, vp],
        "gnnmp_gat_conv_stats_f32": [vp, vp, vp, vp, f, vp, i, vp, vp, i64, i64, vp],
        "gnnmp_gat_conv_train_f32": [vp, vp, vp, vp, f, vp, i, vp, vp, vp, vp, i64, i64, vp],
        "gnnmp_gat_conv_grad2_f32": [vp, vp, vp, vp, vp, f, vp, vp, vp, vp, vp, vp, vp, vp, vp, vp, vp, vp, i64, i64, vp],
        "gnnmp_attn_conv_f32": [vp, i, vp, vp, vp, vp, f, f, vp, i, vp, vp, i64, i64, vp],
        "gnnmp_attn_conv_grad_f32": [vp, vp, i, vp, vp, vp, vp, f, f, vp, vp, vp, vp, vp, vp, vp, vp, i64, i64, vp],
        "gnnmp_gat_conv_grad_f32": [vp, vp, vp, vp, vp, f, vp, vp, vp, vp, vp, vp, vp, vp, i64, i64, vp],
        "gnnmp_gat_conv_drop_f32": [vp, vp, vp, vp, f, f, u64, vp, i, vp, vp, i64, i64, vp],
        "gnnmp_dropout_keep_u8": [u64, f, i64, i64, vp, vp],
        "gnnmp_attn_conv_drop_f32": [vp, i, vp, vp, vp, vp, f, f, f, u64, vp, i, vp, vp, i64, i64, vp],
        "gnnmp_attn_conv_grad_drop_f32": [vp, vp, i, vp, vp, vp, vp, f, f, f, u64, vp, vp, vp, vp, vp, vp, vp, vp, i64, i64, vp],
        "gnnmp_gat_conv_grad_drop_f32": [vp, vp, vp, vp, vp, f, f, u64, vp, vp, vp, vp, vp, vp, vp, vp, i64, i64, vp],
        "gnnmp_degree_f32": [vp, vp, vp, vp],
        "gnnmp_inv_sqrt_f32": [vp, vp, i64, vp],
        "gnnmp_edge_softmax_f32": [vp, vp, vp, i64, vp],
        "gnnmp_segment_softmax_f32": [vp, vp, vp, i64, f, vp],
        "gnnmp_gat_node_scores_f32": [vp, vp, vp, vp, i64, i64, i64, vp],
        "gnnmp_gat_aggregate_f32": [vp, vp, vp, vp, f, vp, i, vp, vp, i64, i64, vp],
        "gnnmp_bias_act_f32": [vp, vp, i, vp, i64, i64, vp],
        "gnnmp_segment_pool_f32": [i, vp, vp, i, i, vp, i64, i64, i64, vp],
        "gnnmp_segment_bounds": [vp, i, i, i64, i64, vp, vp],
        "gnnmp_segment_pool_ptr_f32": [i, vp, vp, vp, i64, i64, i64, vp],
        "gnnmp_dense_f32": [vp, vp, i64, i64, vp, vp, i64, i64, i, vp, i, vp, i64, i64, vp],
        "gnnmp_fused_conv_f32": [vp, i, vp, vp, vp, vp, vp, vp, i64, vp, i64, vp, i64, vp, i64, i, vp, i, vp, i64, vp, vp],
        "gnnmp_edge_dot_f32": [vp, vp, vp, vp, i, i, i64, i64, vp, vp],
        "gnnmp_edge_dot_plan_f32": [vp, vp, vp, vp, i64, vp],
        "gnnmp_head_mean_f32": [vp, vp, i, vp, i64, i64, i64, vp],
        "gnnmp_head_mean_grad_f32": [vp, vp, i64, i64, i64, vp],
        "gnnmp_row_normalize_f32": [vp, vp, vp, i64, i64, vp],
        "gnnmp_propagate_cg_f32": [vp, vp, vp, vp, i, vp, i64, vp],
        "gnnmp_propagate_nn_f32": [vp, i, vp, vp, vp, i64, i64, vp],
        "gnnmp_gmm_weights_f32": [vp, vp, vp, vp, i64, i64, i64, i64, vp],
        "gnnmp_row_sqnorm_normalize_f32": [vp, vp, vp, f, i64, i64, vp],
        "gnnmp_lstm_pointwise_f32": [vp, vp, vp, vp, vp, vp, i64, i64, vp],
        "gnnmp_rowdot_f32": [vp, vp, vp, i64, i64, vp],
        "gnnmp_gru_pointwise_f32": [vp, vp, vp, vp, vp, i64, i64, vp],
        "gnnmp_row_normalize_grad_f32": [vp, vp, vp, vp, vp, vp, vp, f, i64, i64, vp],
        "gnnmp_add_f32": [vp, vp, vp, i64, vp],
        "gnnmp_axpy_f32": [f, vp, vp, vp, i64, vp],
        "gnnmp_mul_rows_f32": [vp, i64, vp, vp, i64, i64, vp],
        "gnnmp_is_sorted": [vp, i, i64, ctypes.POINTER(i), vp],
        "gnnmp_propagate_maxmin_grad_f32": [vp, vp, vp, vp, vp, i64, vp],
        "gnnmp_act_grad_f32": [vp, vp, i, vp, i64, vp],
        "gnnmp_dense_grad_w_f32": [vp, vp, i64, i64, i64, vp, vp, vp, i64, vp],
        "gnnmp_dense_grad_w2_f32": [vp, vp, i64, vp, i64, i64, i64, vp, vp, i64, vp],
        "gnnmp_pool_grad_act_f32": [vp, vp, i, i, vp, vp, i, vp, i64, i64, i64, vp],
        "gnnmp_propagate_add_mask_f32": [vp, i, vp, vp, vp, vp, vp, i64, vp],
        "gnnmp_shard_by_size": [ctypes.POINTER(i64), i64, i, ctypes.POINTER(ctypes.c_int32), ctypes.POINTER(i64), ctypes.POINTER(i64)],
        "gnnmp_allgather_f32": [vp, vp, vp, i64, vp],
        "gnnmp_chain_jobs_create": [ctypes.POINTER(vp), vp, i64, vp],
        "gnnmp_chain_jobs_destroy": [vp],
        "gnnmp_chain_jobs_info": [vp, ctypes.POINTER(i64)],
        "gnnmp_graphconv_chain_f32": [vp, vp, vp, i64, vp, i, ctypes.POINTER(i64), ctypes.POINTER(vp), ctypes.POINTER(vp),
                                      ctypes.POINTER(vp), ctypes.POINTER(i), i, i, i, vp, vp, i64, vp, vp, vp],
        "gnnmp_tune": [i, i],
        "gnnmp_tune_get": [i, ctypes.POINTER(i), ctypes.POINTER(i)],
        "gnnmp_plan_reset_counters": [vp, vp],
        "gnnmp_propagate_f64": [vp, i, i, vp, vp, vp, vp, vp, i64, vp],
        "gnnmp_gather_f64": [vp, vp, i, i, i64, vp, i64, vp],
        "gnnmp_scatter_f64": [vp, i, vp, vp, i64, vp],
        "gnnmp_tgcn_recurrence_f32": [vp, vp, vp, vp, i64, vp, vp, i64, i64, i64, vp],
        "gnnmp_tgcn_recurrence_grad_f32": [vp, vp, vp, vp, vp, vp, i64, vp, vp, vp, i64, i64, i64, vp],
        "gnnmp_tgcn_step_f32": [i, vp, vp, vp, i64, vp, vp, vp, i64, i64, i64, i64, vp],
        "gnnmp_tgcn_step_grad_f32": [i, vp, vp, vp, vp, i64, vp, vp, vp, vp, vp, vp, i64, i64, i64, i64, vp],
        "gnnmp_negative_sample": [vp, vp, i, i, i64, i64, i64, i, i, u64, vp, vp, i64, ctypes.POINTER(i64), vp],
        "gnnmp_rand_edge_split": [vp, vp, i, i, i64, i, i64, u64, vp, vp, vp, vp, vp],
        "gnnmp_edge_dot_grad_f32": [vp, vp, vp, vp, vp, vp, vp, i64, vp],
        "gnnmp_knn_graph_f32": [ctypes.POINTER(vp), vp, i64, i64, i64, vp, i, i, i64, i, vp],
        "gnnmp_radius_graph_f32": [ctypes.POINTER(vp), vp, i64, i64, f, vp, i, i, i64, i, vp],
        "gnnmp_hetero_propagate_f32": [ctypes.POINTER(HeteroDst), i, i64, vp],
        "gnnmp_hetero_propagate_grad_f32": [ctypes.POINTER(HeteroSrc), i, i64, vp],
        "gnnmp_coalesce_edges": [ctypes.POINTER(CoalesceJob), ctypes.POINTER(i64), vp],
        "gnnmp_compact_edges": [ctypes.POINTER(CompactJob), ctypes.POINTER(i64), vp],
        "gnnmp_has_multi_edges": [vp, vp, i, i, i64, ctypes.POINTER(i), vp],
        "gnnmp_has_isolated_nodes": [vp, ctypes.POINTER(i), vp],
        "gnnmp_random_walk_pe_f32": [vp, ctypes.POINTER(RwpeJob), vp],
        "gnnmp_edge_conv_f32": [vp, ctypes.POINTER(EdgeConvJob), i64, vp],
        "gnnmp_edge_conv_grad_f32": [vp, vp, ctypes.POINTER(EdgeConvGradJob), i64, vp],
        "gnnmp_cg_conv_grad_f32": [vp, vp, ctypes.POINTER(CGConvGradJob), i64, vp],
        "gnnmp_debug_random_walk_pe_f32": [vp, ctypes.POINTER(RwpeJob), i64, vp],
        "gnnmp_debug_dense_route": [ctypes.POINTER(i)],
    }
    for name, args in sig.items():
        try:
            fn = getattr(L, name)
        except AttributeError:
            if os.environ.get("GNNMP_LIB"):
                continue
            raise
        fn.argtypes = args
        fn.restype = i
    L.gnnmp_dense_grad_workspace.argtypes = [i64, i64, i64]
    L.gnnmp_dense_grad_workspace.restype = i64
    try:
        L.gnnmp_dense_grad_w2_workspace.argtypes = [i64, i64, i64, i64]
        L.gnnmp_dense_grad_w2_workspace.restype = i64
    except AttributeError:
        if not os.environ.get("GNNMP_LIB"):
            raise
    try:
        L.gnnmp_graphconv_chain_scratch_floats.argtypes = [i64, i, ctypes.POINTER(i64), i64]
        L.gnnmp_graphconv_chain_scratch_floats.restype = i64
    except AttributeError:
        if not os.environ.get("GNNMP_LIB"):
            raise
    _lib = L
    for kv in filter(None, os.environ.get("GNNMP_KNOBS", "").split(",")):
        k, v = kv.split("=")
        tune(int(k), int(v))
    return L


def check(rc):
    if rc != OK:
        raise GnnmpError(rc, load().gnnmp_last_error().decode())


def require_gpu():
    import torch
    if not torch.cuda.is_available():
        raise RuntimeError("gnnmp needs an AMD GPU (gfx950); there is no CPU fallback on the product path")


def stream_ptr():
    import torch
    return ctypes.c_void_p(torch.cuda.current_stream().cuda_stream)


def ptr(t):
    if t is None:
        return None
    return ctypes.c_void_p(t.data_ptr())


_probe = None


class EventProbe:

    def __init__(self):
        self.spans = {}

    def begin(self):
        import torch
        e = torch.cuda.Event(enable_timing=True)
        e.record()
        return e

    def end(self, name, e0):
        import torch
        e1 = torch.cuda.Event(enable_timing=True)
        e1.record()
        self.spans.setdefault(name, []).append((e0, e1))

    def times_ms(self, name):
        return [a.elapsed_time(b) for a, b in self.spans.get(name, [])]


def set_probe(p):
    global _probe
    _probe = p


KNOB_TGCN, KNOB_EDGE_DOT_GRAD, KNOB_HETERO = Knob.TGCN, Knob.EDGE_DOT_GRAD, Knob.HETERO


def knob(k: int) -> int:
    v = ctypes.c_int()
    check(load().gnnmp_tune_get(k, ctypes.byref(v), None))
    return v.value


def knob_default(k: int) -> int:
    d = ctypes.c_int()
    check(load().gnnmp_tune_get(k, None, ctypes.byref(d)))
    return d.value


def tune(knob: int, value: int):
    check(load().gnnmp_tune(knob, value))


@contextlib.contextmanager
def tuned(k: int, value: int):
    before = knob(k)
    tune(k, value)
    try:
        yield
    finally:
        tune(k, before)


def tuned_bits(k: int, set: int = 0, clear: int = 0):
    return tuned(k, (knob(k) | int(set)) & ~int(clear))
```

graphneuralnetworks.jl_amd/gnnmp/graph.py:

```python
from __future__ import annotations

import ctypes

import torch

from . import _lib as L


def _as_index(v, device):
    if isinstance(v, torch.Tensor):
        t = v
    else:
        t = torch.as_tensor(v)
    if t.dtype not in (torch.int64, torch.int32):
        t = t.to(torch.int64)
    return t.to(device).contiguous()


def _as_f32(v, device):
    if v is None:
        return None
    t = v if isinstance(v, torch.Tensor) else torch.as_tensor(v)
    return t.to(device=device, dtype=torch.float32).contiguous()


class Plan:

    def __init__(self, s, t, n_src, n_dst, index_base, add_self_loops, validate=True):
        L.require_gpu()
        lib = L.load()
        self._h = ctypes.c_void_p()
        self._lib = lib
        idx_bytes = 8 if s.dtype == torch.int64 else 4
        rc = lib.gnnmp_plan_create(ctypes.byref(self._h), L.ptr(s), L.ptr(t), idx_bytes, index_base,
                                   n_src, n_dst, s.numel(), 1 if add_self_loops else 0,
                                   1 if validate else 0, L.stream_ptr())
        if rc == L.EBOUNDS:
            raise AssertionError(lib.gnnmp_last_error().decode())
        L.check(rc)
        info = (ctypes.c_int64 * 8)()
        L.check(lib.gnnmp_plan_info(self._h, info))
        self.n_src, self.n_dst, self.n_edges, self.n_total = info[0], info[1], info[2], info[3]
        self.max_degree, self.n_long, self.bytes, self.long_thresh = info[4], info[5], info[6], info[7]
        self.device = s.device

    @classmethod
    def from_csc(cls, colptr, rowval, n_src, n_dst, index_base=1, validate=True):
        L.require_gpu()
        self = object.__new__(cls)
        self._lib = L.load()
        self._h = ctypes.c_void_p()
        idx_bytes = 8 if colptr.dtype == torch.int64 else 4
        rc = self._lib.gnnmp_plan_from_csc(ctypes.byref(self._h), L.ptr(colptr), L.ptr(rowval), idx_bytes, index_base, n_src, n_dst,
                                           rowval.numel(), 1 if validate else 0, L.stream_ptr())
        if rc == L.EBOUNDS:
            raise AssertionError(self._lib.gnnmp_last_error().decode())
        L.check(rc)
        info = (ctypes.c_int64 * 8)()
        L.check(self._lib.gnnmp_plan_info(self._h, info))
        self.n_src, self.n_dst, self.n_edges, self.n_total = info[0], info[1], info[2], info[3]
        self.max_degree, self.n_long, self.bytes, self.long_thresh = info[4], info[5], info[6], info[7]
        self.device = colptr.device
        return self

    @classmethod
    def _adopt(cls, handle, device):
        self = object.__new__(cls)
        self._lib = L.load()
        self._h = handle
        self._pooled = True
        self._last_stream = torch.cuda.current_stream()
        info = (ctypes.c_int64 * 8)()
        L.check(self._lib.gnnmp_plan_info(self._h, info))
        self.n_src, self.n_dst, self.n_edges, self.n_total = info[0], info[1], info[2], info[3]
        self.max_degree, self.n_long, self.bytes, self.long_thresh = info[4], info[5], info[6], info[7]
        self.device = device
        return self

    @property
    def handle(self):
        if getattr(self, "_pooled", False):
            self._last_stream = torch.cuda.current_stream()
        return self._h

    def status(self):
        L.check(self._lib.gnnmp_plan_status(self._h, L.stream_ptr()))

    def edge_index(self, dtype=torch.int64, index_base=1):
        s = torch.empty(self.n_edges, dtype=dtype, device=self.device)
        t = torch.empty(self.n_edges, dtype=dtype, device=self.device)
        L.check(self._lib.gnnmp_plan_edge_index(self._h, 8 if dtype == torch.int64 else 4, index_base, L.ptr(s), L.ptr(t), L.stream_ptr()))
        return s, t

    def export(self):
        rowptr = torch.empty(self.n_dst + 1, dtype=torch.int32, device=self.device)
        col = torch.empty(self.n_total, dtype=torch.int32, device=self.device)
        eid = torch.empty(self.n_total, dtype=torch.int32, device=self.device)
        L.check(self._lib.gnnmp_plan_export(self._h, L.ptr(rowptr), L.ptr(col), L.ptr(eid), L.stream_ptr()))
        return rowptr, col, eid

    def export64(self):
        rowptr = torch.empty(self.n_dst + 1, dtype=torch.int64, device=self.device)
        col = torch.empty(self.n_total, dtype=torch.int32, device=self.device)
        eid = torch.empty(self.n_total, dtype=torch.int32, device=self.device)
        L.check(self._lib.gnnmp_plan_export64(self._h, L.ptr(rowptr), L.ptr(col), L.ptr(eid), L.stream_ptr()))
        return rowptr, col, eid.to(torch.int64) & 0xFFFFFFFF

    def __del__(self):
        try:
            if self._h:
                if getattr(self, "_pooled", False):
                    st = getattr(self, "_last_stream", None)
                    if st is not None:
                        self._lib.gnnmp_plan_release(self._h, ctypes.c_void_p(st.cuda_stream))
                    else:
                        self._lib.gnnmp_plan_destroy(self._h)
                else:
                    self._lib.gnnmp_plan_destroy(self._h)
                self._h = ctypes.c_void_p()
        except Exception:
            pass


class GNNGraph:

    def __init__(self, s, t=None, w=None, num_nodes=None, graph_indicator=None, num_graphs=1, x=None,
                 index_base=1, device=None, _validated=False):
        L.require_gpu()
        if t is None and isinstance(s, (tuple, list)) and len(s) in (2, 3) and not isinstance(s[0], (int, float)):
            tup = s
            s, t = tup[0], tup[1]
            w = tup[2] if len(tup) == 3 else w
        device = torch.device(device) if device is not None else (
            s.device if isinstance(s, torch.Tensor) and s.is_cuda else torch.device("cuda", torch.cuda.current_device()))
        self.index_base = int(index_base)
        assert self.index_base in (0, 1)
        s = _as_index(s, device)
        t = _as_index(t, device)
        if s.dtype != t.dtype:
            t = t.to(s.dtype)
        assert s.dim() == 1 and t.dim() == 1 and s.numel() == t.numel(), "length(s) == length(t)"
        self.w = _as_f32(w, device)
        assert self.w is None or self.w.numel() == s.numel(), "length(val) == length(s)"
        if num_nodes is None:
            num_nodes = 0 if s.numel() == 0 else int(max(int(s.max()), int(t.max()))) + (1 - self.index_base)
        self._s, self._t = s, t
        self.num_nodes = int(num_nodes)
        self.num_edges = int(s.numel())
        self.num_graphs = int(num_graphs)
        self.graph_indicator = None if graph_indicator is None else _as_index(graph_indicator, device)
        self.x = _as_f32(x, device)
        if self.x is not None:
            check_num_nodes(self, self.x)
        self.device = device
        self._plans = {}
        self._cache = {}
        self._indices_validated = bool(_validated)
        if not _validated:
            self.plan(False)

    @classmethod
    def _from_plan(cls, plan: "Plan", num_graphs, graph_indicator, x, index_base, idx_dtype, self_loops=False):
        g = object.__new__(cls)
        g.index_base = int(index_base)
        g._s = g._t = None
        g._idx_dtype = idx_dtype
        g.w = None
        g.num_nodes = int(plan.n_dst)
        g.num_edges = int(plan.n_edges)
        g.num_graphs = int(num_graphs)
        g.graph_indicator = graph_indicator
        g.x = x
        g.device = plan.device
        g._plans = {bool(self_loops): plan}
        g._cache = {}
        g._indices_validated = True
        return g

    @classmethod
    def from_sparse(cls, A=None, colptr=None, rowval=None, nzval=None, num_nodes=None, index_base=1, x=None, device=None):
        L.require_gpu()
        device = torch.device(device) if device is not None else torch.device("cuda", torch.cuda.current_device())
        if A is not None:
            if isinstance(A, torch.Tensor):
                A = A.to_sparse_csc() if A.layout != torch.sparse_csc else A
                n = int(A.shape[0])
                assert A.shape[0] == A.shape[1], "adjacency matrix must be square"
                colptr, rowval, nzval = A.ccol_indices() + index_base, A.row_indices() + index_base, A.values()
            else:
                A = A.tocsc()
                A.sort_indices()
                n = int(A.shape[0])
                assert A.shape[0] == A.shape[1], "adjacency matrix must be square"
                import numpy as _np
                colptr = torch.from_numpy(A.indptr.astype(_np.int64) + index_base)
                rowval = torch.from_numpy(A.indices.astype(_np.int64) + index_base)
                nzval = torch.from_numpy(A.data.astype(_np.float32))
            num_nodes = n if num_nodes is None else num_nodes
        colptr, rowval = _as_index(colptr, device), _as_index(rowval, device)
        if rowval.dtype != colptr.dtype:
            rowval = rowval.to(colptr.dtype)
        if num_nodes is None:
            num_nodes = int(colptr.numel()) - 1
        assert colptr.numel() == num_nodes + 1, "length(colptr) == num_nodes + 1"
        plan = Plan.from_csc(colptr, rowval, num_nodes, num_nodes, index_base)
        g = cls._from_plan(plan, 1, None, None, index_base, colptr.dtype)
        g.graph_type = "sparse"
        g.w = _as_f32(nzval, device)
        assert g.w is None or g.w.numel() == g.num_edges, "length(nzval) == nnz"
        g.x = _as_f32(x, device)
        if g.x is not None:
            check_num_nodes(g, g.x)
        return g

    def _materialise(self):
        p = self._plans.get(False) or self._plans.get(True)
        self._s, self._t = p.edge_index(self._idx_dtype, self.index_base)

    @property
    def s(self):
        if self._s is None:
            self._materialise()
        return self._s

    @s.setter
    def s(self, v):
        self._s = v

    @property
    def t(self):
        if self._t is None:
            self._materialise()
        return self._t

    @t.setter
    def t(self, v):
        self._t = v

    def plan(self, add_self_loops: bool = False) -> Plan:
        key = bool(add_self_loops)
        p = self._plans.get(key)
        if p is None:
            p = Plan(self.s, self.t, self.num_nodes, self.num_nodes, self.index_base, key,
                     validate=not self._indices_validated)
            self._indices_validated = True
            self._plans[key] = p
        return p

    def plan_transposed(self, add_self_loops: bool = False) -> Plan:
        key = ("T", bool(add_self_loops))
        p = self._plans.get(key)
        if p is None:
            p = Plan(self.t, self.s, self.num_nodes, self.num_nodes, self.index_base, key[1],
                     validate=not self._indices_validated)
            self._indices_validated = True
            self._plans[key] = p
        return p

    @property
    def idx_bytes(self):
        dt = self._s.dtype if self._s is not None else self._idx_dtype
        return 8 if dt == torch.int64 else 4

    graph_type = "coo"

    def __repr__(self):
        return f"GNNGraph(num_nodes={self.num_nodes}, num_edges={self.num_edges}, num_graphs={self.num_graphs})"


def check_num_nodes(g: GNNGraph, x):
    if x is None:
        return True
    if getattr(g, "is_hetero", False):
        return g._check_num_nodes(x)
    if isinstance(x, dict):
        for v in x.values():
            check_num_nodes(g, v)
        return True
    if isinstance(x, (tuple, list)):
        for v in x:
            check_num_nodes(g, v)
        return True
    assert g.num_nodes == x.shape[0], \
        f"Got {x.shape[0]} as last dimension size instead of num_nodes={g.num_nodes}"
    return True


def check_num_edges(g: GNNGraph, e):
    if e is None:
        return True
    if getattr(g, "is_hetero", False):
        return g._check_num_edges(e)
    if isinstance(e, dict):
        for v in e.values():
            check_num_edges(g, v)
        return True
    if isinstance(e, (tuple, list)):
        for v in e:
            check_num_edges(g, v)
        return True
    assert g.num_edges == e.shape[0], \
        f"Got {e.shape[0]} as last dimension size instead of num_edges={g.num_edges}"
    return True


def edge_index(g: GNNGraph, edge_t=None):
    if getattr(g, "is_hetero", False):
        return g.edge_index(edge_t)
    return g.s, g.t


def get_edge_weight(g: GNNGraph, edge_t=None):
    if getattr(g, "is_hetero", False):
        return g.get_edge_weight(edge_t)
    return g.w


def get_graph_type(g: GNNGraph):
    return g.graph_type


def graph_indicator(g: GNNGraph, edges: bool = False):
    gi = g.graph_indicator
    if gi is None:
        gi = torch.full((g.num_nodes,), g.index_base, dtype=g.s.dtype, device=g.device)
    if edges:
        ge = g._cache.get("edge_indicator")
        if ge is None:
            words = 2 if gi.dtype == torch.int64 else 1
            src = gi.contiguous().view(torch.float32).view(g.num_nodes, words)
            out = torch.empty((g.num_edges, words), dtype=torch.float32, device=g.device)
            L.check(L.load().gnnmp_gather_f32(L.ptr(src), L.ptr(g.s), g.idx_bytes, g.index_base, g.num_edges, L.ptr(out),
                                              words, L.stream_ptr()))
            ge = out.view(gi.dtype).view(g.num_edges)
            g._cache["edge_indicator"] = ge
        return ge
    return gi


def degree(g: GNNGraph, T=None, dir: str = "out", edge_weight=True):
    if getattr(g, "is_hetero", False):
        return g.degree(T, dir=dir)
    assert dir in ("in", "out", "both")
    if isinstance(edge_weight, torch.Tensor) or isinstance(edge_weight, (list, tuple)):
        w = _as_f32(edge_weight, g.device)
        assert w.numel() == g.num_edges
    elif edge_weight is True:
        w = g.w
    else:
        w = None
    out = None
    lib = L.load()
    for d in (("in", "out") if dir == "both" else (dir,)):
        if d == "in":
            plan = g.plan(False)
        else:
            plan = g.plan_transposed()
        deg = torch.empty(g.num_nodes, dtype=torch.float32, device=g.device)
        L.check(lib.gnnmp_degree_f32(plan.handle, L.ptr(w), L.ptr(deg), L.stream_ptr()))
        if out is None:
            out = deg
        else:
            both = torch.empty_like(deg)
            L.check(lib.gnnmp_add_f32(L.ptr(out), L.ptr(deg), L.ptr(both), deg.numel(), L.stream_ptr()))
            out = both
    if T is None:
        T = torch.float32 if w is not None else g.s.dtype
    if T != torch.float32:
        out = out.to(T)
    return out


def add_self_loops(g: GNNGraph) -> GNNGraph:
    n, E = g.num_nodes, g.num_edges
    s2 = torch.empty(E + n, dtype=g.s.dtype, device=g.device)
    t2 = torch.empty(E + n, dtype=g.s.dtype, device=g.device)
    w2 = None if g.w is None else torch.empty(E + n, dtype=torch.float32, device=g.device)
    L.check(L.load().gnnmp_add_self_loops(L.ptr(g.s), L.ptr(g.t), g.idx_bytes, g.index_base, E, n, L.ptr(s2),
                                          L.ptr(t2), L.ptr(g.w), L.ptr(w2), L.stream_ptr()))
    return GNNGraph(s2, t2, w2, num_nodes=n, graph_indicator=g.graph_indicator, num_graphs=g.num_graphs, x=g.x,
                    index_base=g.index_base, device=g.device, _validated=True)


def set_edge_weight(g: GNNGraph, w) -> GNNGraph:
    w = _as_f32(w, g.device)
    assert w.numel() == g.num_edges
    g2 = GNNGraph(g.s, g.t, w, num_nodes=g.num_nodes, graph_indicator=g.graph_indicator,
                  num_graphs=g.num_graphs, x=g.x, index_base=g.index_base, device=g.device, _validated=True)
    g2._plans = g._plans
    return g2


def batch_arrays(members, xs=None, index_base=1, device=None) -> GNNGraph:
    import numpy as np
    L.require_gpu()
    device = torch.device(device) if device is not None else torch.device("cuda", torch.cuda.current_device())
    G = len(members)
    if G == 0:
        raise ValueError("Cannot batch an empty vector of graphs")
    ne = np.zeros(G + 1, np.int64)
    nn = np.zeros(G + 1, np.int64)
    ne[1:] = np.cumsum([len(m[0]) for m in members])
    nn[1:] = np.cumsum([int(m[2]) for m in members])
    s_host = np.concatenate([np.asarray(m[0], np.int64) for m in members])
    t_host = np.concatenate([np.asarray(m[1], np.int64) for m in members])
    hi = np.repeat(np.diff(nn), np.diff(ne)) + (index_base - 1)
    for name, v in (("s", s_host), ("t", t_host)):
        bad = np.nonzero((v < index_base) | (v > hi))[0]
        if bad.size:
            k = int(bad[0])
            gi_bad = int(np.searchsorted(ne, k, side="right") - 1)
            raise AssertionError(f"batch: {name}[{k - int(ne[gi_bad])}] = {int(v[k])} of member graph {gi_bad} is outside "
                                 f"{index_base}..{int(hi[k])}")
    s_cat = torch.from_numpy(s_host).to(device)
    t_cat = torch.from_numpy(t_host).to(device)
    ned, nnd = torch.from_numpy(ne).to(device), torch.from_numpy(nn).to(device)
    s2, t2 = torch.empty_like(s_cat), torch.empty_like(t_cat)
    gi = torch.empty(int(nn[-1]), dtype=torch.int64, device=device)
    L.check(L.load().gnnmp_batch_coo(L.ptr(s_cat), L.ptr(t_cat), 8, index_base, L.ptr(ned), L.ptr(nnd), G, L.ptr(s2),
                                     L.ptr(t2), L.ptr(gi), L.stream_ptr()))
    x = None
    if xs is not None:
        x = torch.from_numpy(np.concatenate([np.asarray(v, np.float32) for v in xs])).to(device)
    return GNNGraph(s2, t2, None, num_nodes=int(nn[-1]), graph_indicator=gi, num_graphs=G, x=x, index_base=index_base,
                    device=device, _validated=True)


def batch(gs) -> GNNGraph:
    gs = list(gs)
    if len(gs) == 0:
        raise ValueError("Cannot batch an empty vector of graphs")
    g0 = gs[0]
    dev, base, dt = g0.device, g0.index_base, g0.s.dtype
    for g in gs:
        if not isinstance(g, GNNGraph):
            raise ValueError("Cannot batch a non-GNNGraph")
        assert g.index_base == base and g.s.dtype == dt
        assert g.num_graphs == 1 or g.graph_indicator is not None
    if any(g.num_graphs != 1 for g in gs):
        raise NotImplementedError("batching already-batched graphs is outside the hot path")
    import itertools
    ne = torch.tensor([0] + list(itertools.accumulate(g.num_edges for g in gs)), dtype=torch.int64, device=dev)
    nn = torch.tensor([0] + list(itertools.accumulate(g.num_nodes for g in gs)), dtype=torch.int64, device=dev)
    Etot, Ntot = int(ne[-1]), int(nn[-1])
    s_cat = torch.cat([g.s for g in gs])
    t_cat = torch.cat([g.t for g in gs])
    s2, t2 = torch.empty_like(s_cat), torch.empty_like(t_cat)
    gi = torch.empty(Ntot, dtype=dt, device=dev)
    L.check(L.load().gnnmp_batch_coo(L.ptr(s_cat), L.ptr(t_cat), g0.idx_bytes, base, L.ptr(ne), L.ptr(nn), len(gs),
                                     L.ptr(s2), L.ptr(t2), L.ptr(gi), L.stream_ptr()))
    ws = [g.w for g in gs]
    w = torch.cat(ws) if all(x is not None for x in ws) else None
    xs = [g.x for g in gs]
    x = torch.cat(xs) if all(v is not None for v in xs) else None
    out = GNNGraph(s2, t2, w, num_nodes=Ntot, graph_indicator=gi, num_graphs=len(gs), x=x, index_base=base,
                   device=dev, _validated=True)
    assert out.num_edges == Etot
    return out
```

graphneuralnetworks.jl_amd/gnnmp/knobs.py:

```python
from __future__ import annotations

import enum


class Knob(enum.IntEnum):
    FORCE_VEC = 0
    FORCE_LOG2G = 1
    UNROLL = 2
    XCD_REMAP = 3
    LONG_ROW = 4
    BLOCK_WAVES = 5
    DENSE_GENERIC = 6
    DENSE_PREFETCH = 7
    GAT_FAST_EXP = 8
    GRADW_SLABS = 9
    GRADW_RP = 10
    GRADW_MIN_ROWS = 11
    DENSE_T16_WAVES = 12
    T16_DEBUG = 13
    FUSED_WAVES = 14
    ROW_ORDER = 15
    SOFTMAX_ROWS = 16
    DENSE_SPLIT = 17
    CHAIN = 18
    VARIANT = 19
    TGCN = 20
    EDGE_DOT_GRAD = 21
    HETERO = 22
    CHUNK_SLOTS = 23


class Variant(enum.IntFlag):
    CHAIN_WAVES_MASK = 3
    CHAIN_8_WAVES = 1
    SPLIT_SERIAL_TILES = 16
    SPLIT_DIRECT_STORES = 32
    NO_WREG = 64
    TWO_KERNEL_FOLD = 128
    WREG_SMALL = 512
```

include/gnnmp.h:

```cpp
#ifndef GNNMP_H
#define GNNMP_H

#include <stdint.h>

#ifdef __cplusplus
extern "C" {
#endif

#define GNNMP_VERSION 100

typedef void *gnnmp_stream_t;
typedef struct gnnmp_graph gnnmp_graph_t;

typedef enum {
    GNNMP_OK = 0,
    GNNMP_EINVAL = -1,
    GNNMP_EBOUNDS = -2,
    GNNMP_EALLOC = -3,
    GNNMP_ELAUNCH = -4,
    GNNMP_EUNSUPPORTED = -5
} gnnmp_status;

typedef enum { GNNMP_SUM = 0, GNNMP_MEAN = 1, GNNMP_MAX = 2, GNNMP_MIN = 3 } gnnmp_aggr;

typedef enum { GNNMP_COPY_XJ = 0, GNNMP_W_MUL_XJ = 1 } gnnmp_msg;

typedef enum {
    GNNMP_ACT_IDENTITY = 0, GNNMP_ACT_RELU = 1, GNNMP_ACT_SOFTPLUS = 2, GNNMP_ACT_TANH = 3, GNNMP_ACT_SWISH = 4
} gnnmp_act;
typedef enum {
    GNNMP_ATTN_GAT = 0,
    GNNMP_ATTN_GATV2 = 1,
    GNNMP_ATTN_DOT = 2,
    GNNMP_ATTN_COS = 3
} gnnmp_attn;

#define GNNMP_LONG_ROW 512
#define GNNMP_MAX_SLOTS 4294901760LL
#define GNNMP_MIN_LONG_ROW 64

int gnnmp_version(void);
const char *gnnmp_last_error(void);

int gnnmp_plan_create(gnnmp_graph_t **out, const void *src, const void *dst, int idx_bytes,
                      int index_base, int64_t n_src, int64_t n_dst, int64_t n_edges,
                      int add_self_loops, int validate, gnnmp_stream_t stream);
int gnnmp_plan_from_csc(gnnmp_graph_t **out, const void *colptr, const void *rowval, int idx_bytes, int index_base, int64_t n_src,
                        int64_t n_dst, int64_t n_edges, int validate, gnnmp_stream_t stream);
int gnnmp_plan_destroy(gnnmp_graph_t *plan);
int gnnmp_plan_info(const gnnmp_graph_t *plan, int64_t info[8]);
int gnnmp_plan_export(const gnnmp_graph_t *plan, int32_t *rowptr, int32_t *col, int32_t *eid,
                      gnnmp_stream_t stream);
int gnnmp_plan_export64(const gnnmp_graph_t *plan, int64_t *rowptr, int32_t *col, uint32_t *eid,
                        gnnmp_stream_t stream);

int gnnmp_plan_concat(gnnmp_graph_t **out, const gnnmp_graph_t *const *members, int64_t k, int64_t *seg_ptr_out,
                      void *graph_indicator_out, int idx_bytes, int index_base, gnnmp_stream_t stream);
int gnnmp_plan_select(gnnmp_graph_t **out, const gnnmp_graph_t *dataset, const int64_t *node_ptr, int64_t n_graphs, const void *ids,
                      int idx_bytes, int index_base, int64_t k, int64_t n_rows, int64_t n_slots, int64_t *seg_ptr_out,
                      int32_t *node_map_out, void *graph_indicator_out, gnnmp_stream_t stream);
int gnnmp_plan_release(gnnmp_graph_t *plan, gnnmp_stream_t stream);
int gnnmp_plan_status(const gnnmp_graph_t *plan, gnnmp_stream_t stream);
int gnnmp_plan_edge_index(const gnnmp_graph_t *plan, int idx_bytes, int index_base, void *out_src, void *out_dst,
                          gnnmp_stream_t stream);

typedef struct gnnmp_arena gnnmp_arena_t;
int gnnmp_arena_create(gnnmp_arena_t **out, int64_t bytes_per_class, int n_classes, int64_t max_probe_bytes, gnnmp_stream_t stream);
int gnnmp_arena_destroy(gnnmp_arena_t *arena);
int gnnmp_arena_alloc(gnnmp_arena_t *arena, int cls, int64_t bytes, void **ptr);
int gnnmp_arena_reset(gnnmp_arena_t *arena);
int gnnmp_arena_class_of(gnnmp_arena_t *arena, const void *ptr, int64_t bytes, int *cls, gnnmp_stream_t stream);
int gnnmp_arena_info(const gnnmp_arena_t *arena, int64_t *info);

int gnnmp_add_self_loops(const void *src, const void *dst, int idx_bytes, int index_base,
                         int64_t n_edges, int64_t n, void *out_src, void *out_dst, const float *w,
                         float *out_w, gnnmp_stream_t stream);

int gnnmp_batch_coo(const void *src, const void *dst, int idx_bytes, int index_base,
                    const int64_t *edge_ptr, const int64_t *node_ptr, int64_t n_graphs,
                    void *out_src, void *out_dst, void *graph_indicator, gnnmp_stream_t stream);

int gnnmp_sort_edge_index(const void *u, const void *v, int idx_bytes, int index_base, int64_t n_edges,
                          void *u_out, void *v_out, gnnmp_stream_t stream);
int gnnmp_is_bidirected(const void *s, const void *t, int idx_bytes, int index_base, int64_t n_edges,
                        int *result, gnnmp_stream_t stream);
int gnnmp_has_self_loops(const void *s, const void *t, int idx_bytes, int64_t n_edges, int *result,
                         gnnmp_stream_t stream);
int gnnmp_sample_neighbors(gnnmp_graph_t *plan, const void *nodes, int idx_bytes, int index_base, int64_t n_nodes,
                           int64_t K, int replace, uint64_t seed, int64_t *offsets, void *eids_out,
                           int64_t capacity, int64_t *total, gnnmp_stream_t stream);

int gnnmp_unique_append(int32_t *map, int32_t *first, int64_t n_nodes, const void *cand, int idx_bytes,
                        int index_base, int64_t n_cand, int64_t set_size, void *list_out, int64_t *n_new,
                        gnnmp_stream_t stream);
int gnnmp_induced_subgraph(gnnmp_graph_t *plan, const int32_t *map, const void *nodes, int idx_bytes,
                           int index_base, int64_t n_nodes, int64_t *offsets, void *s_out, void *t_out,
                           void *eid_out, int64_t capacity, int64_t *total, gnnmp_stream_t stream);

typedef enum { GNNMP_COALESCE_DIRECTED = 0, GNNMP_COALESCE_MIRRORED = 1, GNNMP_COALESCE_UNDIRECTED = 2 } gnnmp_coalesce_mode;
typedef struct {
    const void *s;
    const void *t;
    int idx_bytes;
    int index_base;
    int64_t n_edges;
    int64_t n_nodes;
    int mode;
    void *s_out;
    void *t_out;
    void *colptr;
    void *rowval;
} gnnmp_coalesce_t;
int gnnmp_coalesce_edges(const gnnmp_coalesce_t *job, int64_t *total, gnnmp_stream_t stream);

typedef enum { GNNMP_COMPACT_SELF_LOOPS = 0, GNNMP_COMPACT_LIST = 1, GNNMP_COMPACT_RANDOM = 2 } gnnmp_compact_rule;
typedef struct {
    const void *s;
    const void *t;
    const float *w;
    int idx_bytes;
    int index_base;
    int64_t n_edges;
    int rule;
    const void *remove;
    int64_t n_remove;
    float p;
    uint64_t seed;
    void *s_out;
    void *t_out;
    float *w_out;
    void *eid_out;
} gnnmp_compact_t;
int gnnmp_compact_edges(const gnnmp_compact_t *job, int64_t *total, gnnmp_stream_t stream);

int gnnmp_has_multi_edges(const void *s, const void *t, int idx_bytes, int index_base, int64_t n_edges, int *result,
                          gnnmp_stream_t stream);
int gnnmp_has_isolated_nodes(gnnmp_graph_t *plan, int *result, gnnmp_stream_t stream);

#define GNNMP_RWPE_TILE 16
#define GNNMP_RWPE_MAX_WALK 1024
typedef struct {
    const float *w;
    const void *graph_ptr;
    int idx_bytes;
    int64_t n_graphs;
    int64_t walk_length;
    float *out;
} gnnmp_rwpe_t;
int gnnmp_random_walk_pe_f32(gnnmp_graph_t *plan_t, const gnnmp_rwpe_t *job, gnnmp_stream_t stream);

int gnnmp_gather_f32(const float *x, const void *idx, int idx_bytes, int index_base, int64_t K,
                     float *out, int64_t D, gnnmp_stream_t stream);
int gnnmp_edge_sub_f32(const float *xi, const float *xj, const void *s, const void *t, int idx_bytes, int index_base,
                       int64_t K, int xj_minus_xi, float *out, int64_t D, gnnmp_stream_t stream);
int gnnmp_scatter_f32(gnnmp_graph_t *plan, int aggr, const float *m, float *out, int64_t D,
                      gnnmp_stream_t stream);
int gnnmp_scatter_atomic_f32(int aggr, const float *m, const void *idx, int idx_bytes,
                             int index_base, int64_t K, float *out, int64_t D,
                             gnnmp_stream_t stream);

int gnnmp_propagate_f32(gnnmp_graph_t *plan, int msg, int aggr, const float *xj, const float *w,
                        const float *scale_src, const float *scale_dst, float *out, int64_t D,
                        gnnmp_stream_t stream);

int gnnmp_propagate_emul_f32(gnnmp_graph_t *plan, int aggr, const float *xj, const float *e, float *out, int64_t D,
                             gnnmp_stream_t stream);

int gnnmp_propagate_gated_f32(gnnmp_graph_t *plan, int aggr, const float *gate_i, const float *bv_j, float *out,
                              int64_t D, gnnmp_stream_t stream);

int gnnmp_propagate_cg_f32(gnnmp_graph_t *plan, const float *fs_i, const float *fs_j, const float *fs_e, int act,
                           float *out, int64_t D, gnnmp_stream_t stream);
int gnnmp_propagate_nn_f32(gnnmp_graph_t *plan, int aggr, const float *xj, const float *we, float *out, int64_t Din,
                           int64_t Dout, gnnmp_stream_t stream);
int gnnmp_propagate_slots_f32(gnnmp_graph_t *plan, int aggr, const float *xj, const float *w_slot,
                              const float *ss_slot, const float *scale_dst, float *out, int64_t D,
                              gnnmp_stream_t stream);
int gnnmp_propagate_slots_act_f32(gnnmp_graph_t *plan, int aggr, const float *xj, const float *w_slot, const float *ss_slot,
                                  const float *scale_dst, const float *bias, int act, float *out, int64_t D,
                                  gnnmp_stream_t stream);
int gnnmp_plan_slot_gather_f32(gnnmp_graph_t *plan, int by, const float *v, float *out_slot,
                               gnnmp_stream_t stream);

int gnnmp_degree_f32(gnnmp_graph_t *plan, const float *w, float *deg, gnnmp_stream_t stream);

int gnnmp_inv_sqrt_f32(const float *deg, float *out, int64_t n, gnnmp_stream_t stream);

int gnnmp_edge_softmax_f32(gnnmp_graph_t *plan, const float *logits, float *alpha, int64_t H,
                           gnnmp_stream_t stream);
int gnnmp_segment_softmax_f32(gnnmp_graph_t *plan, const float *x, float *out, int64_t D, float den_add,
                              gnnmp_stream_t stream);

int gnnmp_gat_node_scores_f32(const float *Wx, const float *a, float *score_dst, float *score_src,
                              int64_t N, int64_t H, int64_t C, gnnmp_stream_t stream);
int gnnmp_gat_aggregate_f32(gnnmp_graph_t *plan, const float *Wx_src, const float *score_dst,
                            const float *score_src, float negative_slope, const float *bias, int act,
                            float *out, float *alpha_out, int64_t H, int64_t C,
                            gnnmp_stream_t stream);

int gnnmp_gat_conv_f32(gnnmp_graph_t *plan, const float *Wx_src, const float *Wx_dst, const float *a,
                       float negative_slope, const float *bias, int act, float *out, int64_t H,
                       int64_t C, gnnmp_stream_t stream);

int gnnmp_gat_conv_edge_f32(gnnmp_graph_t *plan, const float *Wx_src, const float *Wx_dst, const float *a,
                            const float *edge_score, float negative_slope, const float *bias, int act, float *out,
                            int64_t H, int64_t C, gnnmp_stream_t stream);

int gnnmp_gat_conv_stats_f32(gnnmp_graph_t *plan, const float *Wx_src, const float *Wx_dst, const float *a,
                             float negative_slope, const float *bias, int act, float *out, float *stats,
                             int64_t H, int64_t C, gnnmp_stream_t stream);

int gnnmp_gat_conv_train_f32(gnnmp_graph_t *plan, const float *Wx_src, const float *Wx_dst, const float *a, float negative_slope,
                             const float *bias, int act, float *out, float *stats, float *oplus, float *pplus, int64_t H, int64_t C,
                             gnnmp_stream_t stream);
int gnnmp_gat_conv_grad2_f32(gnnmp_graph_t *plan, gnnmp_graph_t *plan_t, const float *Wx_src, const float *Wx_dst, const float *a,
                             float negative_slope, const float *stats, const float *out, const float *bias, const float *oplus,
                             const float *pplus, const float *dout, float *line, float *dsd, float *dss, float *dWx_src, float *dWx_dst,
                             float *da, int64_t H, int64_t C, gnnmp_stream_t stream);
int gnnmp_gat_conv_drop_f32(gnnmp_graph_t *plan, const float *Wx_src, const float *Wx_dst, const float *a,
                            float negative_slope, float p, uint64_t seed, const float *bias, int act, float *out,
                            float *stats, int64_t H, int64_t C, gnnmp_stream_t stream);
int gnnmp_dropout_keep_u8(uint64_t seed, float p, int64_t n_edges, int64_t H, uint8_t *keep, gnnmp_stream_t stream);

int gnnmp_attn_conv_f32(gnnmp_graph_t *plan, int mode, const float *Q, const float *K, const float *V,
                        const float *a, float negative_slope, float scale, const float *bias, int act,
                        float *out, float *stats, int64_t H, int64_t C, gnnmp_stream_t stream);

int gnnmp_gat_conv_grad_f32(gnnmp_graph_t *plan, gnnmp_graph_t *plan_t, const float *Wx_src, const float *Wx_dst,
                            const float *a, float negative_slope, const float *stats, const float *dout,
                            float *line, float *dsd, float *dss, float *dWx_src, float *dWx_dst, float *da,
                            int64_t H, int64_t C, gnnmp_stream_t stream);

int gnnmp_gat_conv_grad_drop_f32(gnnmp_graph_t *plan, gnnmp_graph_t *plan_t, const float *Wx_src, const float *Wx_dst,
                                 const float *a, float negative_slope, float p, uint64_t seed, const float *stats,
                                 const float *dout, float *line, float *dsd, float *dss, float *dWx_src, float *dWx_dst,
                                 float *da, int64_t H, int64_t C, gnnmp_stream_t stream);

int gnnmp_attn_conv_drop_f32(gnnmp_graph_t *plan, int mode, const float *Q, const float *K, const float *V, const float *a,
                             float negative_slope, float scale, float p, uint64_t seed, const float *bias, int act, float *out,
                             float *stats, int64_t H, int64_t C, gnnmp_stream_t stream);
int gnnmp_attn_conv_grad_drop_f32(gnnmp_graph_t *plan, gnnmp_graph_t *plan_t, int mode, const float *Q, const float *K,
                                  const float *V, const float *a, float negative_slope, float scale, float p, uint64_t seed,
                                  const float *stats, const float *dout, float *line, float *dQ, float *dK, float *dV, float *dA,
                                  float *da, int64_t H, int64_t C, gnnmp_stream_t stream);

int gnnmp_attn_conv_grad_f32(gnnmp_graph_t *plan, gnnmp_graph_t *plan_t, int mode, const float *Q, const float *K,
                             const float *V, const float *a, float negative_slope, float scale, const float *stats,
                             const float *dout, float *line, float *dQ, float *dK, float *dV, float *dA, float *da,
                             int64_t H, int64_t C, gnnmp_stream_t stream);

int gnnmp_head_mean_f32(const float *y, const float *bias, int act, float *out, int64_t N, int64_t H,
                        int64_t C, gnnmp_stream_t stream);
int gnnmp_head_mean_grad_f32(const float *dz, float *dy, int64_t N, int64_t H, int64_t C, gnnmp_stream_t stream);
int gnnmp_gmm_weights_f32(const float *e, const float *mu, const float *sigma_inv, float *out, int64_t E, int64_t ein,
                          int64_t K, int64_t C, gnnmp_stream_t stream);
int gnnmp_row_sqnorm_normalize_f32(const float *x, float *sq, float *xn, float eps, int64_t N, int64_t D,
                                   gnnmp_stream_t stream);
int gnnmp_lstm_pointwise_f32(const float *gx, const float *gh, const float *b, const float *c, float *h_out, float *c_out,
                             int64_t N, int64_t D, gnnmp_stream_t stream);
int gnnmp_rowdot_f32(const float *a, const float *b, float *out, int64_t N, int64_t D, gnnmp_stream_t stream);
int gnnmp_gru_pointwise_f32(const float *gx, const float *gh, const float *b, const float *h, float *out, int64_t N,
                            int64_t D, gnnmp_stream_t stream);
int gnnmp_row_normalize_f32(const float *x, float *xn, float *rnorm, int64_t N, int64_t D, gnnmp_stream_t stream);
int gnnmp_row_normalize_grad_f32(const float *dq, const float *dk, const float *xn, const float *rnorm,
                                 const float *base, float *dx, float *qdot, float qscale, int64_t N, int64_t D,
                                 gnnmp_stream_t stream);
int gnnmp_add_f32(const float *a, const float *b, float *out, int64_t n, gnnmp_stream_t stream);
int gnnmp_mul_rows_f32(const float *a, int64_t Da, const float *b, float *out, int64_t N, int64_t D,
                       gnnmp_stream_t stream);
int gnnmp_axpy_f32(float alpha, const float *x, const float *y, float *out, int64_t n, gnnmp_stream_t stream);
int gnnmp_is_sorted(const void *idx, int idx_bytes, int64_t n, int *result_host, gnnmp_stream_t stream);

int gnnmp_bias_act_f32(const float *x, const float *bias, int act, float *out, int64_t N, int64_t D,
                       gnnmp_stream_t stream);

int gnnmp_segment_pool_f32(int aggr, const float *x, const void *seg_ids, int idx_bytes,
                           int index_base, float *out, int64_t D, int64_t N, int64_t G,
                           gnnmp_stream_t stream);
int gnnmp_segment_bounds(const void *seg_ids, int idx_bytes, int index_base, int64_t N, int64_t G, int64_t *seg_ptr,
                         gnnmp_stream_t stream);
int gnnmp_segment_pool_ptr_f32(int aggr, const float *x, const int64_t *seg_ptr, float *out, int64_t D, int64_t N, int64_t G,
                               gnnmp_stream_t stream);

int gnnmp_dense_f32(const float *x1, const float *W1, int64_t D1, int64_t ldw1, const float *x2,
                    const float *W2, int64_t D2, int64_t ldw2, int w_layout, const float *bias,
                    int act, float *out, int64_t N, int64_t Dout, gnnmp_stream_t stream);

int gnnmp_shard_by_size(const int64_t *sizes, int64_t G, int world, int32_t *rank_of, int64_t *gather_index, int64_t *gmax);
int gnnmp_allgather_f32(void *nccl_comm, const float *send, float *recv, int64_t count, gnnmp_stream_t stream);

int64_t gnnmp_graphconv_chain_scratch_floats(int64_t N, int n_layers, const int64_t *dims, int64_t nout);
typedef struct gnnmp_chain_jobs gnnmp_chain_jobs_t;
int gnnmp_chain_jobs_create(gnnmp_chain_jobs_t **out, const int64_t *seg_ptr, int64_t G, gnnmp_stream_t stream);
int gnnmp_chain_jobs_destroy(gnnmp_chain_jobs_t *jobs);
int gnnmp_chain_jobs_info(const gnnmp_chain_jobs_t *jobs, int64_t *info);
int gnnmp_chain_jobs_pack(gnnmp_chain_jobs_t **out, const int64_t *seg_ptr, int64_t G, int64_t n_rows, int64_t max_graph, int has_empty,
                          gnnmp_stream_t stream);
int gnnmp_chain_jobs_release(gnnmp_chain_jobs_t *jobs, gnnmp_stream_t stream);
int gnnmp_chain_jobs_export(const gnnmp_chain_jobs_t *jobs, int32_t *tab_out, int64_t cap_rows, int32_t *hdr_out, gnnmp_stream_t stream);
int gnnmp_graphconv_chain_f32(gnnmp_graph_t *plan, const gnnmp_chain_jobs_t *jobs, const int64_t *seg_ptr, int64_t G, const float *x, int n_layers,
                              const int64_t *dims, const float *const *W_root, const float *const *W_agg,
                              const float *const *bias, const int *act, int w_layout, int aggr, int pool_aggr, const float *W_head,
                              const float *b_head, int64_t nout, float *scratch, float *out, gnnmp_stream_t stream);

int gnnmp_fused_conv_f32(gnnmp_graph_t *plan, int aggr, const float *xj, const float *w, const float *scale_src,
                         const float *w_slot, const float *ss_slot, const float *scale_dst, int64_t D, const float *xi,
                         int64_t D1, const float *W_root, int64_t ldw_root, const float *W_agg, int64_t ldw_agg,
                         int w_layout, const float *bias, int act, float *out, int64_t Dout, float *agg_out,
                         gnnmp_stream_t stream);

int gnnmp_edge_dot_f32(const float *a_dst, const float *b_src, const void *src, const void *dst,
                       int idx_bytes, int index_base, int64_t n_edges, int64_t D, float *out,
                       gnnmp_stream_t stream);
int gnnmp_edge_dot_plan_f32(gnnmp_graph_t *plan, const float *a_dst, const float *b_src, float *out,
                            int64_t D, gnnmp_stream_t stream);
int gnnmp_propagate_maxmin_grad_f32(gnnmp_graph_t *plan_transposed, const float *x, const float *y,
                                    const float *dy, float *dx, int64_t D, gnnmp_stream_t stream);

int gnnmp_act_grad_f32(const float *dy, const float *y, int act, float *dz, int64_t n, gnnmp_stream_t stream);
int64_t gnnmp_dense_grad_w2_workspace(int64_t N, int64_t Dout, int64_t K1, int64_t K2);
int gnnmp_dense_grad_w2_f32(const float *dz, const float *x1, int64_t K1, const float *x2, int64_t K2, int64_t N, int64_t Dout,
                            float *out, float *workspace, int64_t workspace_floats, gnnmp_stream_t stream);
int gnnmp_pool_grad_act_f32(const float *dpool, const void *graph_indicator, int idx_bytes, int index_base, const float *inv_count,
                            const float *y, int act, float *dz, int64_t N, int64_t G, int64_t D, gnnmp_stream_t stream);
int gnnmp_propagate_add_mask_f32(gnnmp_graph_t *plan, int aggr, const float *xj, const float *scale_dst, const float *addend,
                                 const float *mask_y, float *out, int64_t D, gnnmp_stream_t stream);
int64_t gnnmp_dense_grad_workspace(int64_t N, int64_t Dout, int64_t K);
int gnnmp_dense_grad_w_f32(const float *dz, const float *x, int64_t N, int64_t Dout, int64_t K, float *dW,
                           float *db, float *workspace, int64_t workspace_floats, gnnmp_stream_t stream);

int gnnmp_tgcn_recurrence_f32(const float *P, const float *U_zr, const float *U_h, const float *h0, int64_t h0_stride, float *y,
                              float *gates, int64_t N, int64_t T, int64_t out, gnnmp_stream_t stream);
int gnnmp_tgcn_recurrence_grad_f32(const float *dy, const float *y, const float *gates, const float *U_zr, const float *U_h,
                                   const float *h0, int64_t h0_stride, float *dP, float *S, float *dh0, int64_t N, int64_t T,
                                   int64_t out, gnnmp_stream_t stream);
int gnnmp_tgcn_step_f32(int phase, const float *P, const float *a, const float *h, int64_t ldh, float *gates, float *hout, float *y,
                        int64_t N, int64_t T, int64_t t, int64_t D, gnnmp_stream_t stream);
int gnnmp_tgcn_step_grad_f32(int phase, const float *dy, const float *carry, const float *gates, const float *h, int64_t ldh,
                             const float *drh, float *dP, float *dah, float *dzr, float *part, float *S, int64_t N, int64_t T, int64_t t,
                             int64_t D, gnnmp_stream_t stream);

int gnnmp_negative_sample(const void *s, const void *t, int idx_bytes, int index_base, int64_t n_edges, int64_t n_nodes,
                          int64_t num_neg_edges, int bidirected, int max_trials, uint64_t seed, void *s_out, void *t_out,
                          int64_t capacity, int64_t *total, gnnmp_stream_t stream);
int gnnmp_rand_edge_split(const void *s, const void *t, int idx_bytes, int index_base, int64_t n_edges, int bidirected, int64_t size1,
                          uint64_t seed, void *s1, void *t1, void *s2, void *t2, gnnmp_stream_t stream);
int gnnmp_edge_dot_grad_f32(gnnmp_graph_t *plan, gnnmp_graph_t *plan_transposed, const float *xi, const float *xj, const float *dz,
                            float *dxi, float *dxj, int64_t D, gnnmp_stream_t stream);

int gnnmp_knn_graph_f32(gnnmp_graph_t **out, const float *points, int64_t N, int64_t d, int64_t k, const void *graph_indicator,
                        int idx_bytes, int index_base, int64_t n_graphs, int self_loops, gnnmp_stream_t stream);
int gnnmp_radius_graph_f32(gnnmp_graph_t **out, const float *points, int64_t N, int64_t d, float r, const void *graph_indicator,
                           int idx_bytes, int index_base, int64_t n_graphs, int self_loops, gnnmp_stream_t stream);

#define GNNMP_HETERO_MAX_REL 16
typedef struct {
    const gnnmp_graph_t *plan;
    const float *x;
    const float *w;
    int aggr;
} gnnmp_hetero_rel_t;
typedef struct {
    float *out;
    int64_t n_dst;
    int combine;
    int n_rel;
    const gnnmp_hetero_rel_t *rels;
} gnnmp_hetero_dst_t;
int gnnmp_hetero_propagate_f32(const gnnmp_hetero_dst_t *dsts, int n_dsts, int64_t D, gnnmp_stream_t stream);

typedef struct {
    const gnnmp_graph_t *plan_t;
    const float *dy;
    const float *w;
    const float *sd;
    const float *y;
    const float *out;
} gnnmp_hetero_rel_grad_t;
typedef struct {
    float *dx;
    const float *x;
    int64_t n_src;
    int n_rel;
    const gnnmp_hetero_rel_grad_t *rels;
} gnnmp_hetero_src_t;
int gnnmp_hetero_propagate_grad_f32(const gnnmp_hetero_src_t *srcs, int n_srcs, int64_t D, gnnmp_stream_t stream);

typedef struct {
    const float *p;
    float *y;
    int aggr;
    int act;
} gnnmp_edge_conv_t;
typedef struct {
    const float *p;
    const float *y;
    const float *dy;
    float *dp;
    int aggr;
    int act;
} gnnmp_edge_conv_grad_t;
int gnnmp_edge_conv_f32(const gnnmp_graph_t *plan, const gnnmp_edge_conv_t *job, int64_t C, gnnmp_stream_t stream);
int gnnmp_edge_conv_grad_f32(const gnnmp_graph_t *plan, const gnnmp_graph_t *plan_t, const gnnmp_edge_conv_grad_t *job, int64_t C,
                             gnnmp_stream_t stream);

typedef struct {
    const float *fs_i, *fs_j, *fs_e;
    const float *dy;
    float *dfs_i, *dfs_j, *dfs_e;
    int act;
} gnnmp_cg_conv_grad_t;
int gnnmp_cg_conv_grad_f32(const gnnmp_graph_t *plan, const gnnmp_graph_t *plan_t, const gnnmp_cg_conv_grad_t *job, int64_t C,
                           gnnmp_stream_t stream);

int gnnmp_propagate_f64(gnnmp_graph_t *plan, int msg, int aggr, const double *xj, const double *w, const double *scale_src,
                        const double *scale_dst, double *out, int64_t D, gnnmp_stream_t stream);
int gnnmp_gather_f64(const double *x, const void *idx, int idx_bytes, int index_base, int64_t K, double *out, int64_t D,
                     gnnmp_stream_t stream);
int gnnmp_scatter_f64(gnnmp_graph_t *plan, int aggr, const double *m, double *out, int64_t D, gnnmp_stream_t stream);

int gnnmp_plan_reset_counters(gnnmp_graph_t *plan, gnnmp_stream_t stream);

int gnnmp_tune(int knob, int value);
int gnnmp_tune_get(int knob, int *value, int *default_value);
int gnnmp_debug_mock_device(int dev);
int gnnmp_debug_device_once(const int *devs, int n, int fail_on, int *n_failed);
void *gnnmp_debug_plan_block(const gnnmp_graph_t *plan);
int gnnmp_debug_pool_pick(const uint64_t *caps, int n, uint64_t bytes);
int gnnmp_debug_random_walk_pe_f32(gnnmp_graph_t *plan_t, const gnnmp_rwpe_t *job, int64_t lds_budget_bytes, gnnmp_stream_t stream);
int gnnmp_debug_dense_route(int info[8]);

#ifdef __cplusplus
}
#endif
#endif
```

Measured before the change: 12.53 billion edges/s.

## Build long-row chunk tables on device and pool plan allocations

Moves the long-row chunk table construction from a host loop to two GPU kernels plus an exclusive scan. It also allocates the plan arrays and build scratch from a pool block, and drops the separate identity value array and the varying-bits sync in the radix sort. This is meant to cut plan-creation latency: host synchronizations, hipMallocs and device-host copies. The fwd steady-state throughput metric mostly exercises the message-passing kernels, so plan setup is likely outside the timed loop. In exchange the plan code gains device-side kernels, a new layout of the plan memory block and a host fallback variant.

```diff
diff --git a/graphneuralnetworks.jl_amd/csrc/chunk_math.h b/graphneuralnetworks.jl_amd/csrc/chunk_math.h
--- /dev/null
+++ b/graphneuralnetworks.jl_amd/csrc/chunk_math.h
@@ -0,0 +1,18 @@
+#pragma once
+#include <stdint.h>
+
+#if defined(__HIPCC__)
+#define GNNMP_HD __host__ __device__
+#else
+#define GNNMP_HD
+#endif
+
+namespace gnnmp {
+GNNMP_HD inline int64_t chunk_count(int64_t len, int64_t clen) { return (len + clen - 1) / clen; }
+GNNMP_HD inline int64_t chunk_size(int64_t len, int64_t nch) { return (len + nch - 1) / nch; }
+GNNMP_HD inline int64_t chunk_begin(int64_t beg, int64_t c, int64_t csz) { return beg + c * csz; }
+GNNMP_HD inline int64_t chunk_end(int64_t beg, int64_t end, int64_t c, int64_t csz) {
+    const int64_t e = beg + (c + 1) * csz;
+    return e < end ? e : end;
+}
+}
diff --git a/graphneuralnetworks.jl_amd/csrc/common.h b/graphneuralnetworks.jl_amd/csrc/common.h
--- a/graphneuralnetworks.jl_amd/csrc/common.h
+++ b/graphneuralnetworks.jl_amd/csrc/common.h
@@ -267,6 +267,10 @@
     size_t spart_floats = 0;
     void *block = nullptr;
     size_t block_bytes = 0;
+    size_t tab_off = 0, tab_cap = 0;
+    void *tblock = nullptr;
+    size_t tblock_bytes = 0;
+    bool tables_owned = false;
     int32_t *status = nullptr;
 };
 
@@ -282,6 +286,17 @@
 int ensure_ticket(gnnmp_graph *p, hipStream_t stream);
 int ensure_row_order(gnnmp_graph *p, hipStream_t stream);
 int plan_build_long_rows(gnnmp_graph *p, hipStream_t stream);
+struct __attribute__((visibility("hidden"))) LongWork {
+    int64_t *packed = nullptr;
+    int64_t *pos = nullptr;
+    int *flags = nullptr;
+    int64_t *scan_ws = nullptr;
+    static size_t bytes(int64_t n_dst);
+    LongWork(void *base, int64_t n_dst);
+};
+int plan_long_tables(gnnmp_graph *p, const LongWork &w, hipStream_t stream, int *bad);
+size_t plan_tables_reserve(int64_t n_dst, int64_t Etot, int long_thresh);
+inline bool host_plan_tables() { return (knob(KNOB_VARIANT) & VARIANT_HOST_PLAN_TABLES) != 0; }
 int plan_long_thresh(int64_t Etot);
 }
 
diff --git a/graphneuralnetworks.jl_amd/csrc/knobs.h b/graphneuralnetworks.jl_amd/csrc/knobs.h
--- a/graphneuralnetworks.jl_amd/csrc/knobs.h
+++ b/graphneuralnetworks.jl_amd/csrc/knobs.h
@@ -59,6 +59,7 @@
     VARIANT_SPLIT_DIRECT_STORES = 32,
     VARIANT_NO_WREG = 64,
     VARIANT_TWO_KERNEL_FOLD = 128,
+    VARIANT_HOST_PLAN_TABLES = 256,
     VARIANT_WREG_SMALL = 512,
 };
 
diff --git a/graphneuralnetworks.jl_amd/csrc/plan.hip b/graphneuralnetworks.jl_amd/csrc/plan.hip
--- a/graphneuralnetworks.jl_amd/csrc/plan.hip
+++ b/graphneuralnetworks.jl_amd/csrc/plan.hip
@@ -2,6 +2,7 @@
 #include <algorithm>
 #include <vector>
 
+#include "chunk_math.h"
 #include "common.h"
 #include "launch.h"
 #include "pool.h"
@@ -61,8 +62,7 @@
 
 
 __global__ void plan_fill_keys(const void *src, const void *dst, int idx_bytes, int base, int64_t E,
-                               int64_t Etot, int64_t n_src, int64_t n_dst, uint32_t *keys,
-                               uint32_t *vals, int *bad) {
+                               int64_t Etot, int64_t n_src, int64_t n_dst, uint32_t *keys, int *bad) {
     int64_t k = (int64_t)blockIdx.x * blockDim.x + threadIdx.x;
     if (k >= Etot) return;
     int64_t d;
@@ -77,7 +77,6 @@
         d = k - E;
     }
     keys[k] = (uint32_t)d;
-    vals[k] = (uint32_t)k;
 }
 
 __global__ void plan_rowptr(const uint32_t *keys, int64_t Etot, int64_t n_dst, uint32_t *rowptr) {
@@ -218,7 +217,7 @@
     return v >= 16 ? v : 128;
 }
 
-int plan_build_long_rows(gnnmp_graph *p, hipStream_t stream) {
+static int plan_build_long_rows_host(gnnmp_graph *p, hipStream_t stream) {
     const int64_t n_dst = p->n_dst, Etot = p->n_total;
     const int BS = 256;
     const int cap = (int)std::min<int64_t>(Etot / std::max(1, p->long_thresh) + 1, n_dst + 1);
@@ -234,11 +233,12 @@
     }
     int meta[4] = {0, 0, 0, 0};
     GNNMP_HIP(hipMemcpyAsync(meta, flags.get(), sizeof(int) * 4, hipMemcpyDeviceToHost, stream));
-    GNNMP_HIP(hipStreamSynchronize(stream));
+    GNNMP_HIP(setup_wait(stream));
     unsigned long long md;
     memcpy(&md, meta + 2, sizeof(md));
     p->max_degree = (int64_t)md;
     p->n_long = std::min(meta[0], cap);
+    p->tables_owned = true;
     if (p->n_long == 0) return GNNMP_OK;
     struct Tri { int64_t row, beg, end; };
     std::vector<Tri> h((size_t)p->n_long);
@@ -280,6 +280,142 @@
     return GNNMP_OK;
 }
 
+
+__global__ void __launch_bounds__(256) plan_long_count(const uint32_t *__restrict__ rowptr, int64_t n_dst, int thresh, int clen,
+                                                       int64_t *__restrict__ packed, uint32_t *maxdeg) {
+    uint32_t m = 0;
+    for (int64_t i = (int64_t)blockIdx.x * 256 + threadIdx.x; i <= n_dst; i += (int64_t)gridDim.x * 256) {
+        if (i < n_dst) {
+            const uint32_t len = rowptr[i + 1] - rowptr[i];
+            packed[i] = len > (uint32_t)thresh ? (((int64_t)1 << 32) | chunk_count(len, clen)) : 0;
+            m = max(m, len);
+        } else {
+            packed[i] = 0;
+        }
+    }
+#pragma unroll
+    for (int o = 32; o > 0; o >>= 1) m = max(m, (uint32_t)__shfl_xor((int)m, o, 64));
+    if ((threadIdx.x & 63) == 0 && m > __atomic_load_n(maxdeg, __ATOMIC_RELAXED)) atomicMax(maxdeg, m);
+}
+
+struct ChunkTables {
+    int32_t *long_rows, *long_cptr, *chunk_row, *chunk_lrow;
+    uint32_t *chunk_beg, *chunk_end;
+};
+
+__global__ void __launch_bounds__(256) plan_chunk_fill(const uint32_t *__restrict__ rowptr, int64_t n_dst, const int64_t *__restrict__ packed,
+                                                       const int64_t *__restrict__ pos, int n_long, int n_chunks, ChunkTables t) {
+    const int64_t i = (int64_t)blockIdx.x * 256 + threadIdx.x;
+    if (i > n_dst) return;
+    if (i == n_dst) {
+        t.long_cptr[n_long] = n_chunks;
+        return;
+    }
+    const int64_t pk = packed[i];
+    if (pk == 0) return;
+    const int64_t lrow = pos[i] >> 32, c0 = pos[i] & 0xffffffffll, nch = pk & 0xffffffffll;
+    if (lrow >= n_long || c0 + nch > n_chunks) return;
+    const int64_t beg = rowptr[i], end = rowptr[i + 1];
+    const int64_t csz = chunk_size(end - beg, nch);
+    t.long_rows[lrow] = (int32_t)i;
+    t.long_cptr[lrow] = (int32_t)c0;
+    for (int64_t c = 0; c < nch; ++c) {
+        t.chunk_row[c0 + c] = (int32_t)i;
+        t.chunk_lrow[c0 + c] = (int32_t)lrow;
+        t.chunk_beg[c0 + c] = (uint32_t)chunk_begin(beg, c, csz);
+        t.chunk_end[c0 + c] = (uint32_t)chunk_end(beg, end, c, csz);
+    }
+}
+
+static inline size_t up256(size_t b) { return (b + 255) & ~(size_t)255; }
+
+static size_t tables_room(int64_t n_long, int64_t n_chunks) {
+    return up256(4 * (size_t)n_long) + up256(4 * (size_t)(n_long + 1)) + 4 * up256(4 * (size_t)n_chunks);
+}
+size_t plan_tables_reserve(int64_t n_dst, int64_t Etot, int long_thresh) {
+    const int64_t clen = std::min<int64_t>(long_thresh, plan_chunk_slots());
+    const int64_t max_long = std::min<int64_t>(Etot / ((int64_t)long_thresh + 1), n_dst);
+    if (max_long == 0) return 0;
+    return tables_room(max_long, Etot / clen + max_long);
+}
+
+size_t LongWork::bytes(int64_t n_dst) {
+    return up256(8 * (size_t)(n_dst + 1)) + up256(8 * (size_t)(n_dst + 2)) + up256(8 * exclusive_scan_workspace((size_t)(n_dst + 1)));
+}
+LongWork::LongWork(void *base, int64_t n_dst) {
+    unsigned char *b = static_cast<unsigned char *>(base);
+    packed = reinterpret_cast<int64_t *>(b);
+    pos = reinterpret_cast<int64_t *>(b + up256(8 * (size_t)(n_dst + 1)));
+    scan_ws = reinterpret_cast<int64_t *>(b + up256(8 * (size_t)(n_dst + 1)) + up256(8 * (size_t)(n_dst + 2)));
+    flags = reinterpret_cast<int *>(pos + n_dst + 1);
+}
+
+int plan_long_tables(gnnmp_graph *p, const LongWork &w, hipStream_t stream, int *bad) {
+    const int64_t n_dst = p->n_dst;
+    const int BS = 256;
+    const int clen = (int)std::min<int64_t>(p->long_thresh, plan_chunk_slots());
+    const unsigned count_blocks = std::min<unsigned>(nblocks(n_dst + 1, BS), (unsigned)device_cus() * 4);
+    plan_long_count<<<count_blocks, BS, 0, stream>>>(p->rowptr, n_dst, p->long_thresh, clen, w.packed,
+                                                               reinterpret_cast<uint32_t *>(w.flags + 1));
+    GNNMP_HIP(hipGetLastError());
+    GNNMP_TRY(exclusive_scan_i64(w.packed, w.pos, (size_t)(n_dst + 1), stream, w.scan_ws));
+    int64_t rec[2] = {0, 0};
+    GNNMP_HIP(hipMemcpyAsync(rec, w.pos + n_dst, sizeof(rec), hipMemcpyDeviceToHost, stream));
+    GNNMP_HIP(setup_wait(stream));
+    uint32_t fl[2];
+    memcpy(fl, &rec[1], sizeof(fl));
+    if (bad) {
+        *bad = (int)fl[0];
+        if (fl[0]) return GNNMP_OK;
+    }
+    p->max_degree = (int64_t)fl[1];
+    const int64_t n_long = rec[0] >> 32, n_chunks = rec[0] & 0xffffffffll;
+    p->n_long = (int)n_long;
+    if (n_long == 0) return GNNMP_OK;
+    if (n_chunks >= (int64_t)INT32_MAX)
+        return fail(GNNMP_EUNSUPPORTED, "plan_create: %zu chunks of split rows exceed the int32 chunk index", (size_t)n_chunks);
+    p->n_chunks = (int)n_chunks;
+    const size_t room = tables_room(n_long, n_chunks);
+    unsigned char *b = nullptr;
+    if (p->block && p->tab_cap >= room) {
+        b = static_cast<unsigned char *>(p->block) + p->tab_off;
+    } else {
+        if (!pool_take(&p->tblock, &p->tblock_bytes, room, stream))
+            return fail(GNNMP_EALLOC, "plan_create: hipMalloc of %zu bytes (chunk tables) failed", room);
+        b = static_cast<unsigned char *>(p->tblock);
+    }
+    ChunkTables t;
+    t.long_rows = reinterpret_cast<int32_t *>(b);
+    b += up256(4 * (size_t)n_long);
+    t.long_cptr = reinterpret_cast<int32_t *>(b);
+    b += up256(4 * (size_t)(n_long + 1));
+    const size_t piece = up256(4 * (size_t)n_chunks);
+    t.chunk_row = reinterpret_cast<int32_t *>(b);
+    t.chunk_lrow = reinterpret_cast<int32_t *>(b + piece);
+    t.chunk_beg = reinterpret_cast<uint32_t *>(b + 2 * piece);
+    t.chunk_end = reinterpret_cast<uint32_t *>(b + 3 * piece);
+    p->long_rows = t.long_rows;
+    p->long_cptr = t.long_cptr;
+    p->chunk_row = t.chunk_row;
+    p->chunk_lrow = t.chunk_lrow;
+    p->chunk_beg = t.chunk_beg;
+    p->chunk_end = t.chunk_end;
+    p->bytes += (int64_t)(4 * (size_t)n_long + 4 * (size_t)(n_long + 1) + 16 * (size_t)n_chunks);
+    plan_chunk_fill<<<nblocks(n_dst + 1, BS), BS, 0, stream>>>(p->rowptr, n_dst, w.packed, w.pos, p->n_long, p->n_chunks, t);
+    GNNMP_HIP(hipGetLastError());
+    return GNNMP_OK;
+}
+
+int plan_build_long_rows(gnnmp_graph *p, hipStream_t stream) {
+    if (host_plan_tables()) return plan_build_long_rows_host(p, stream);
+    PoolBlock scratch;
+    if (!scratch.take(LongWork::bytes(p->n_dst), stream))
+        return fail(GNNMP_EALLOC, "plan: hipMalloc of %zu bytes (long-row scratch) failed", LongWork::bytes(p->n_dst));
+    const LongWork w(scratch.p, p->n_dst);
+    GNNMP_HIP(hipMemsetAsync(w.flags, 0, 2 * sizeof(int), stream));
+    return plan_long_tables(p, w, stream, nullptr);
+}
+
 }
 
 using namespace gnnmp;
@@ -303,17 +439,42 @@
 namespace gnnmp {
 int plan_dispose(gnnmp_graph_t *p, hipStream_t stream, bool stream_known) {
     if (!p) return GNNMP_OK;
+    if (!p->tables_owned)
+        p->long_rows = p->long_cptr = p->chunk_row = p->chunk_lrow = nullptr, p->chunk_beg = p->chunk_end = nullptr;
     if (p->block) {
         pool_park(p->block, p->block_bytes, stream, stream_known);
         p->rowptr = nullptr;
         p->col = nullptr;
         p->eid = nullptr;
     }
+    if (p->tblock) pool_park(p->tblock, p->tblock_bytes, stream, stream_known);
     void *const owned[] = {p->rowptr, p->col, p->eid, p->long_rows, p->long_cptr, p->chunk_row, p->chunk_lrow, p->arrive, p->spart,
                            p->chunk_beg, p->chunk_end, p->ws, p->ticket, p->row_order};
     for (void *q : owned)
         if (q) (void)dev_free(q);
     delete p;
+    return GNNMP_OK;
+}
+struct PlanOnStream {
+    hipStream_t stream;
+    void operator()(gnnmp_graph *p) const { (void)plan_dispose(p, stream, true); }
+};
+using StreamPlanPtr = std::unique_ptr<gnnmp_graph, PlanOnStream>;
+
+static int plan_block_take(gnnmp_graph *p, size_t epad, hipStream_t stream) {
+    const size_t o_col = up256(sizeof(uint32_t) * (size_t)(p->n_dst + 1));
+    const size_t o_eid = o_col + up256(sizeof(int32_t) * epad);
+    const size_t o_tab = o_eid + up256(sizeof(int32_t) * epad);
+    const size_t reserve = host_plan_tables() ? 0 : plan_tables_reserve(p->n_dst, p->n_total, p->long_thresh);
+    if (!pool_take(&p->block, &p->block_bytes, o_tab + reserve, stream))
+        return fail(GNNMP_EALLOC, "plan_create: hipMalloc of %zu bytes (plan arrays) failed", o_tab + reserve);
+    unsigned char *b = static_cast<unsigned char *>(p->block);
+    p->rowptr = reinterpret_cast<uint32_t *>(b);
+    p->col = reinterpret_cast<int32_t *>(b + o_col);
+    p->eid = reinterpret_cast<int32_t *>(b + o_eid);
+    p->tab_off = o_tab;
+    p->tab_cap = reserve;
+    p->bytes = (int64_t)(sizeof(int32_t) * ((size_t)(p->n_dst + 1) + 2 * epad));
     return GNNMP_OK;
 }
 int check_transposed(const char *who, const gnnmp_graph_t *plan, const gnnmp_graph_t *plan_t) {
@@ -348,7 +509,7 @@
         return fail(GNNMP_EUNSUPPORTED, "plan_create: E' = %lld (limit 2^32 - 65536) / N = %lld (limit 2^31 - 2) exceed the plan format",
                     (long long)Etot, (long long)std::max(n_src, n_dst));
 
-    PlanPtr p(new gnnmp_graph_t());
+    StreamPlanPtr p(new gnnmp_graph_t(), PlanOnStream{stream});
     p->n_src = n_src;
     p->n_dst = n_dst;
     p->n_edges = n_edges;
@@ -358,38 +519,25 @@
 
     const int BS = 256;
     const size_t epad = (size_t)std::max<int64_t>(Etot, 1);
-    DevBuf<int> flags;
-    DevBuf<unsigned char> sort_keys;
-    uint32_t *keys_out = nullptr;
-    GNNMP_HIP(alloc_into(p->rowptr, (size_t)(n_dst + 1)));
-    GNNMP_HIP(alloc_into(p->col, epad));
-    GNNMP_HIP(alloc_into(p->eid, epad));
-    GNNMP_HIP(flags.alloc(4));
-    GNNMP_HIP(hipMemsetAsync(flags.get(), 0, sizeof(int) * 4, stream));
-    p->bytes = (int64_t)(sizeof(int32_t) * ((size_t)(n_dst + 1) + 2 * epad));
+    GNNMP_TRY(plan_block_take(p.get(), epad, stream));
+    const size_t piece = up256(sizeof(uint32_t) * epad);
+    const size_t sort_ws = Etot > 0 ? radix_sort_pairs_u32_workspace((size_t)Etot) : 0;
+    PoolBlock scratch;
+    const size_t scratch_bytes = 2 * piece + sort_ws + LongWork::bytes(n_dst);
+    if (!scratch.take(scratch_bytes, stream)) return fail(GNNMP_EALLOC, "plan_create: hipMalloc of %zu bytes (build scratch) failed", scratch_bytes);
+    unsigned char *sb = static_cast<unsigned char *>(scratch.p);
+    uint32_t *keys_in = reinterpret_cast<uint32_t *>(sb), *keys_out = reinterpret_cast<uint32_t *>(sb + piece);
+    const LongWork w(sb + 2 * piece + sort_ws, n_dst);
+    GNNMP_HIP(hipMemsetAsync(w.flags, 0, 2 * sizeof(int), stream));
 
     if (Etot > 0) {
-        const size_t piece = (sizeof(uint32_t) * epad + 255) & ~(size_t)255;
-        GNNMP_HIP(sort_keys.alloc(3 * piece));
-        uint32_t *keys_in = reinterpret_cast<uint32_t *>(sort_keys.get());
-        keys_out = reinterpret_cast<uint32_t *>(sort_keys.get() + piece);
-        uint32_t *vals_in = reinterpret_cast<uint32_t *>(sort_keys.get() + 2 * piece);
-        plan_fill_keys<<<nblocks(Etot, BS), BS, 0, stream>>>(src, dst, idx_bytes, index_base,
-                                                             n_edges, Etot, n_src, n_dst, keys_in,
-                                                             vals_in, flags.get());
+        plan_fill_keys<<<nblocks(Etot, BS), BS, 0, stream>>>(src, dst, idx_bytes, index_base, n_edges, Etot, n_src, n_dst, keys_in, w.flags);
         GNNMP_HIP(hipGetLastError());
-        if (validate) {
-            int bad = 0;
-            GNNMP_HIP(hipMemcpyAsync(&bad, flags.get(), sizeof(int), hipMemcpyDeviceToHost, stream));
-            GNNMP_HIP(hipStreamSynchronize(stream));
-            if (bad)
-                return fail(GNNMP_EBOUNDS, "plan_create: edge index outside 1..N (n_src=%lld n_dst=%lld)",
-                            (long long)n_src, (long long)n_dst);
-        }
         unsigned bits = 1;
         while (bits < 32 && ((int64_t)1 << bits) < n_dst) ++bits;
-        GNNMP_TRY(radix_sort_pairs_u32(keys_in, keys_out, vals_in, reinterpret_cast<uint32_t *>(p->eid), (size_t)Etot, 0, (int)bits,
-                                       stream));
+        const uint32_t live = bits >= 32 ? 0xffffffffu : ((1u << bits) - 1u);
+        GNNMP_TRY(radix_sort_pairs_u32_ws(keys_in, keys_out, nullptr, reinterpret_cast<uint32_t *>(p->eid), (size_t)Etot, live, sb + 2 * piece,
+                                          stream));
         plan_col<<<nblocks(Etot, BS), BS, 0, stream>>>(src, idx_bytes, index_base, n_edges, Etot,
                                                        reinterpret_cast<uint32_t *>(p->eid), p->col);
         GNNMP_HIP(hipGetLastError());
@@ -397,7 +545,16 @@
     plan_rowptr<<<nblocks(n_dst + 1, BS), BS, 0, stream>>>(keys_out, Etot, n_dst, p->rowptr);
     GNNMP_HIP(hipGetLastError());
 
-    GNNMP_TRY(plan_build_long_rows(p.get(), stream));
+    int bad = 0;
+    if (host_plan_tables()) {
+        GNNMP_HIP(hipMemcpyAsync(&bad, w.flags, sizeof(int), hipMemcpyDeviceToHost, stream));
+        GNNMP_HIP(setup_wait(stream));
+        if (!(bad && validate)) GNNMP_TRY(plan_build_long_rows(p.get(), stream));
+    } else {
+        GNNMP_TRY(plan_long_tables(p.get(), w, stream, validate ? &bad : nullptr));
+    }
+    if (bad && validate)
+        return fail(GNNMP_EBOUNDS, "plan_create: edge index outside 1..N (n_src=%lld n_dst=%lld)", (long long)n_src, (long long)n_dst);
     *out = p.release();
     return GNNMP_OK;
 }
@@ -414,7 +571,7 @@
     if (n_edges >= (int64_t)GNNMP_MAX_SLOTS || n_src >= (int64_t)INT32_MAX || n_dst >= (int64_t)INT32_MAX)
         return fail(GNNMP_EUNSUPPORTED, "plan_from_csc: E = %lld (limit 2^32 - 65536) / N = %lld (limit 2^31 - 2) exceed the plan format",
                     (long long)n_edges, (long long)std::max(n_src, n_dst));
-    PlanPtr p(new gnnmp_graph_t());
+    StreamPlanPtr p(new gnnmp_graph_t(), PlanOnStream{stream});
     p->n_src = n_src;
     p->n_dst = n_dst;
     p->n_edges = n_edges;
@@ -422,27 +579,30 @@
     p->long_thresh = plan_long_thresh(n_edges);
     const int BS = 256;
     const size_t epad = (size_t)std::max<int64_t>(n_edges, 1);
-    DevBuf<int> flags;
-    GNNMP_HIP(alloc_into(p->rowptr, (size_t)(n_dst + 1)));
-    GNNMP_HIP(alloc_into(p->col, epad));
-    GNNMP_HIP(alloc_into(p->eid, epad));
-    GNNMP_HIP(flags.alloc(4));
-    GNNMP_HIP(hipMemsetAsync(flags.get(), 0, sizeof(int) * 4, stream));
-    p->bytes = (int64_t)(sizeof(int32_t) * ((size_t)(n_dst + 1) + 2 * epad));
-    csc_rowptr_kernel<<<nblocks(n_dst + 1, BS), BS, 0, stream>>>(colptr, idx_bytes, index_base, n_dst, n_edges, p->rowptr, flags.get());
+    GNNMP_TRY(plan_block_take(p.get(), epad, stream));
+    PoolBlock scratch;
+    if (!scratch.take(LongWork::bytes(n_dst), stream))
+        return fail(GNNMP_EALLOC, "plan_from_csc: hipMalloc of %zu bytes (build scratch) failed", LongWork::bytes(n_dst));
+    const LongWork w(scratch.p, n_dst);
+    GNNMP_HIP(hipMemsetAsync(w.flags, 0, 2 * sizeof(int), stream));
+    csc_rowptr_kernel<<<nblocks(n_dst + 1, BS), BS, 0, stream>>>(colptr, idx_bytes, index_base, n_dst, n_edges, p->rowptr, w.flags);
     GNNMP_HIP(hipGetLastError());
     if (n_edges > 0) {
-        csc_col_kernel<<<nblocks(n_edges, BS), BS, 0, stream>>>(rowval, idx_bytes, index_base, n_edges, n_src, p->col, p->eid, flags.get());
+        csc_col_kernel<<<nblocks(n_edges, BS), BS, 0, stream>>>(rowval, idx_bytes, index_base, n_edges, n_src, p->col, p->eid, w.flags);
         GNNMP_HIP(hipGetLastError());
     }
     (void)validate;
     int bad = 0;
-    GNNMP_HIP(hipMemcpyAsync(&bad, flags.get(), sizeof(int), hipMemcpyDeviceToHost, stream));
-    GNNMP_HIP(hipStreamSynchronize(stream));
+    if (host_plan_tables()) {
+        GNNMP_HIP(hipMemcpyAsync(&bad, w.flags, sizeof(int), hipMemcpyDeviceToHost, stream));
+        GNNMP_HIP(setup_wait(stream));
+        if (!bad) GNNMP_TRY(plan_build_long_rows(p.get(), stream));
+    } else {
+        GNNMP_TRY(plan_long_tables(p.get(), w, stream, &bad));
+    }
     if (bad)
         return fail(GNNMP_EBOUNDS, "plan_from_csc: colptr is not a monotone 0..E column pointer, or a row index lies outside 1..n_src "
                     "(n_src=%lld n_dst=%lld E=%lld)", (long long)n_src, (long long)n_dst, (long long)n_edges);
-    GNNMP_TRY(plan_build_long_rows(p.get(), stream));
     *out = p.release();
     return GNNMP_OK;
 }
diff --git a/graphneuralnetworks.jl_amd/csrc/pool.h b/graphneuralnetworks.jl_amd/csrc/pool.h
--- a/graphneuralnetworks.jl_amd/csrc/pool.h
+++ b/graphneuralnetworks.jl_amd/csrc/pool.h
@@ -5,6 +5,21 @@
 namespace gnnmp {
 bool pool_take(void **out, size_t *cap, size_t bytes, hipStream_t stream);
 void pool_park(void *p, size_t cap, hipStream_t stream, bool stream_known);
+struct PoolBlock {
+    void *p = nullptr;
+    size_t cap = 0;
+    hipStream_t stream = nullptr;
+    PoolBlock() = default;
+    PoolBlock(const PoolBlock &) = delete;
+    PoolBlock &operator=(const PoolBlock &) = delete;
+    bool take(size_t bytes, hipStream_t s) {
+        stream = s;
+        return pool_take(&p, &cap, bytes < 256 ? 256 : bytes, s);
+    }
+    ~PoolBlock() {
+        if (p) pool_park(p, cap, stream, true);
+    }
+};
 int pool_pick(const size_t *caps, int n, size_t bytes);
 void pool_trim();
 }
diff --git a/graphneuralnetworks.jl_amd/csrc/pool.hip b/graphneuralnetworks.jl_amd/csrc/pool.hip
--- a/graphneuralnetworks.jl_amd/csrc/pool.hip
+++ b/graphneuralnetworks.jl_amd/csrc/pool.hip
@@ -2,6 +2,7 @@
 
 #include "pool.h"
 #include "common.h"
+#include "scratch.h"
 
 namespace gnnmp {
 namespace {
@@ -10,12 +11,15 @@
     size_t cap = 0;
     hipStream_t stream = nullptr;
     hipEvent_t ev = nullptr;
+    unsigned long long seq = 0;
 };
 constexpr int POOL_SLOTS = 8;
+constexpr size_t POOL_MAX_PARKED = (size_t)4 << 30;
 struct DevicePool {
     Parked slots[POOL_SLOTS];
     hipEvent_t free_events[POOL_SLOTS] = {};
     int n_free_events = 0;
+    unsigned long long parked = 0;
 };
 DevicePool g_pools[GNNMP_MAX_DEVICES];
 std::mutex g_lock;
@@ -58,6 +62,7 @@
     if (got.p) {
         bool ok = true;
         if (!got.ev) {
+            setup_count(SETUP_WAITS);
             ok = hipDeviceSynchronize() == hipSuccess;
         } else {
             if (!same_stream(got.stream, stream)) ok = hipStreamWaitEvent(stream, got.ev, 0) == hipSuccess;
@@ -69,14 +74,18 @@
             *cap = got.cap;
             return true;
         }
-        (void)hipFree(got.p);
+        (void)dev_free(got.p);
     }
     *cap = bytes;
-    return hipMalloc(out, bytes) == hipSuccess;
+    return dev_malloc(out, bytes) == hipSuccess;
 }
 
 void pool_park(void *p, size_t cap, hipStream_t stream, bool stream_known) {
     if (!p) return;
+    if (cap > POOL_MAX_PARKED) {
+        (void)dev_free(p);
+        return;
+    }
     int dev = current_device();
     {
         hipPointerAttribute_t at;
@@ -109,18 +118,14 @@
         if (slot < 0) {
             slot = 0;
             for (int i = 1; i < POOL_SLOTS; ++i)
-                if (dp.slots[i].cap < dp.slots[slot].cap) slot = i;
-            if (dp.slots[slot].cap >= cap) {
-                evict = in;
-                in = Parked();
-            } else {
-                evict = dp.slots[slot];
-            }
+                if (dp.slots[i].seq < dp.slots[slot].seq) slot = i;
+            evict = dp.slots[slot];
         }
+        in.seq = ++dp.parked;
         if (in.p) dp.slots[slot] = in;
         if (evict.ev) { event_put(dp, evict.ev); evict.ev = nullptr; }
     }
-    if (evict.p) (void)hipFree(evict.p);
+    if (evict.p) (void)dev_free(evict.p);
 }
 
 void pool_trim() {
@@ -139,7 +144,7 @@
         }
         if (!any) continue;
         for (int i = 0; i < POOL_SLOTS; ++i)
-            if (all[i].p) (void)hipFree(all[i].p);
+            if (all[i].p) (void)dev_free(all[i].p);
     }
 }
 }
diff --git a/graphneuralnetworks.jl_amd/csrc/runtime.hip b/graphneuralnetworks.jl_amd/csrc/runtime.hip
--- a/graphneuralnetworks.jl_amd/csrc/runtime.hip
+++ b/graphneuralnetworks.jl_amd/csrc/runtime.hip
@@ -5,6 +5,7 @@
 
 #include "common.h"
 #include "pool.h"
+#include "scratch.h"
 
 namespace gnnmp {
 
@@ -56,6 +57,9 @@
     }
     return cus;
 }
+
+static std::atomic<long long> g_setup_counts[SETUP_COUNTS] = {};
+void setup_count(int which) { g_setup_counts[which].fetch_add(1, std::memory_order_relaxed); }
 
 bool fold_disabled_by_env() {
     static const bool off = [] {
@@ -112,6 +116,11 @@
     return ran;
 }
 void *gnnmp_debug_plan_block(const gnnmp_graph_t *p) { return p ? p->block : nullptr; }
+int gnnmp_debug_setup_counters(int64_t counts[3]) {
+    if (!counts) return fail(GNNMP_EINVAL, "gnnmp_debug_setup_counters: null pointer");
+    for (int k = 0; k < SETUP_COUNTS; ++k) counts[k] = (int64_t)g_setup_counts[k].load(std::memory_order_relaxed);
+    return GNNMP_OK;
+}
 int gnnmp_debug_pool_pick(const uint64_t *caps, int n, uint64_t bytes) {
     size_t c[64];
     if (n < 0 || n > 64) return -2;
diff --git a/graphneuralnetworks.jl_amd/csrc/scratch.h b/graphneuralnetworks.jl_amd/csrc/scratch.h
--- a/graphneuralnetworks.jl_amd/csrc/scratch.h
+++ b/graphneuralnetworks.jl_amd/csrc/scratch.h
@@ -6,8 +6,11 @@
 #ifndef GNNMP_SCRATCH_STANDIN
 #include "common.h"
 namespace gnnmp {
-inline hipError_t dev_malloc(void **out, size_t bytes) { return hipMalloc(out, bytes); }
-inline hipError_t dev_free(void *p) { return hipFree(p); }
+enum SetupCount { SETUP_MALLOCS = 0, SETUP_FREES = 1, SETUP_WAITS = 2, SETUP_COUNTS = 3 };
+__attribute__((visibility("hidden"))) void setup_count(int which);
+inline hipError_t dev_malloc(void **out, size_t bytes) { setup_count(SETUP_MALLOCS); return hipMalloc(out, bytes); }
+inline hipError_t dev_free(void *p) { setup_count(SETUP_FREES); return hipFree(p); }
+inline hipError_t setup_wait(hipStream_t stream) { setup_count(SETUP_WAITS); return hipStreamSynchronize(stream); }
 }
 #endif
 
diff --git a/graphneuralnetworks.jl_amd/csrc/sort_scan.h b/graphneuralnetworks.jl_amd/csrc/sort_scan.h
--- a/graphneuralnetworks.jl_amd/csrc/sort_scan.h
+++ b/graphneuralnetworks.jl_amd/csrc/sort_scan.h
@@ -6,6 +6,9 @@
 namespace gnnmp {
 int radix_sort_pairs_u32(const uint32_t *keys_in, uint32_t *keys_out, const uint32_t *vals_in, uint32_t *vals_out, size_t n,
                          int begin_bit, int end_bit, hipStream_t stream);
+size_t radix_sort_pairs_u32_workspace(size_t n);
+int radix_sort_pairs_u32_ws(const uint32_t *keys_in, uint32_t *keys_out, const uint32_t *vals_in, uint32_t *vals_out, size_t n,
+                            uint32_t live_bits, void *ws, hipStream_t stream);
 int radix_sort_keys_u64(const uint64_t *keys_in, uint64_t *keys_out, size_t n, int begin_bit, int end_bit, hipStream_t stream);
 int radix_sort_pairs_u64(const uint64_t *keys_in, uint64_t *keys_out, const uint32_t *vals_in, uint32_t *vals_out, size_t n,
                          int begin_bit, int end_bit, hipStream_t stream);
diff --git a/graphneuralnetworks.jl_amd/csrc/sort_scan.hip b/graphneuralnetworks.jl_amd/csrc/sort_scan.hip
--- a/graphneuralnetworks.jl_amd/csrc/sort_scan.hip
+++ b/graphneuralnetworks.jl_amd/csrc/sort_scan.hip
@@ -98,7 +98,7 @@
         for (int s = 0; s < RS_WT / 64; ++s) {
             const size_t i = base + (size_t)s * 64 + lane;
             kreg[s] = i < n ? keys[i] : (K)0;
-            if (PAIRS) vreg[PAIRS ? s : 0] = i < n ? vals[i] : 0u;
+            if (PAIRS) vreg[PAIRS ? s : 0] = i < n ? (vals ? vals[i] : (uint32_t)i) : 0u;
         }
 #pragma unroll
         for (int s = 0; s < RS_WT / 64; ++s) {
@@ -234,7 +234,7 @@
     GNNMP_HIP(sums.alloc(scan_blocks(n)));
     exclusive_scan_enqueue<T>(in, out, n, sums.get(), stream);
     hipError_t e = hipGetLastError();
-    if (e == hipSuccess) e = hipStreamSynchronize(stream);
+    if (e == hipSuccess) e = setup_wait(stream);
     if (e != hipSuccess) return hip_fail(e, "exclusive_scan");
     return GNNMP_OK;
 }
@@ -259,42 +259,41 @@
 }
 
 template <class K, bool PAIRS>
-static int radix_sort_impl(const K *keys_in, K *keys_out, const uint32_t *vals_in, uint32_t *vals_out, size_t n, int begin_bit,
-                           int end_bit, hipStream_t stream) {
-    if (n == 0) return GNNMP_OK;
-    if (n >= ((size_t)1 << 32)) return fail(GNNMP_EUNSUPPORTED, "radix sort: %zu elements exceed the 32-bit offset tables", n);
+struct RadixWs {
+    size_t b_k, b_v, b_c, b_s;
+    explicit RadixWs(size_t n) {
+        auto up = [](size_t b) { return (b + 255) & ~(size_t)255; };
+        const size_t m = 256 * ((n + RS_WT - 1) / RS_WT);
+        b_k = up(sizeof(K) * n);
+        b_v = PAIRS ? up(sizeof(uint32_t) * n) : 0;
+        b_c = up(sizeof(uint32_t) * m);
+        b_s = up(sizeof(uint32_t) * scan_blocks(m));
+    }
+    size_t bytes() const { return b_k + b_v + b_c + b_s; }
+};
+
+template <class K, bool PAIRS>
+static int radix_sort_enqueue(const K *keys_in, K *keys_out, const uint32_t *vals_in, uint32_t *vals_out, size_t n, int begin_bit,
+                              int end_bit, unsigned long long vary, unsigned char *ws, hipStream_t stream) {
     const int passes = std::max(1, (end_bit - begin_bit + 7) / 8);
     const size_t n_tiles = (n + RS_WT - 1) / RS_WT;
     const size_t m = 256 * n_tiles;
-    auto up = [](size_t b) { return (b + 255) & ~(size_t)255; };
-    const size_t b_k = up(sizeof(K) * n), b_v = PAIRS ? up(sizeof(uint32_t) * n) : 0, b_c = up(sizeof(uint32_t) * m),
-                 b_s = up(sizeof(uint32_t) * scan_blocks(m));
-    DevBuf<unsigned char> arena;
-    hipError_t e = arena.alloc(b_k + b_v + b_c + b_s + 256);
-    if (e != hipSuccess) return hip_fail(e, "hipMalloc(radix sort temporaries)");
-    K *ktmp = reinterpret_cast<K *>(arena.get());
-    uint32_t *vtmp = PAIRS ? reinterpret_cast<uint32_t *>(arena.get() + b_k) : nullptr;
-    uint32_t *counts = reinterpret_cast<uint32_t *>(arena.get() + b_k + b_v);
-    uint32_t *sums = reinterpret_cast<uint32_t *>(arena.get() + b_k + b_v + b_c);
-    unsigned long long *dvary = reinterpret_cast<unsigned long long *>(arena.get() + b_k + b_v + b_c + b_s), hvary = 0;
+    const RadixWs<K, PAIRS> lay(n);
+    K *ktmp = reinterpret_cast<K *>(ws);
+    uint32_t *vtmp = PAIRS ? reinterpret_cast<uint32_t *>(ws + lay.b_k) : nullptr;
+    uint32_t *counts = reinterpret_cast<uint32_t *>(ws + lay.b_k + lay.b_v);
+    uint32_t *sums = reinterpret_cast<uint32_t *>(ws + lay.b_k + lay.b_v + lay.b_c);
     const unsigned blocks = (unsigned)((n_tiles + RS_WPB - 1) / RS_WPB);
     const size_t scatter_lds = (size_t)RS_WT * RS_WPB * (sizeof(K) + (PAIRS ? sizeof(uint32_t) : 0)) + (256 * RS_WPB + 256) * sizeof(uint32_t);
-    e = hipFuncSetAttribute(reinterpret_cast<const void *>(&rs_scatter<K, PAIRS>), hipFuncAttributeMaxDynamicSharedMemorySize,
-                            (int)scatter_lds);
+    hipError_t e = hipFuncSetAttribute(reinterpret_cast<const void *>(&rs_scatter<K, PAIRS>), hipFuncAttributeMaxDynamicSharedMemorySize,
+                                       (int)scatter_lds);
     if (e != hipSuccess) return hip_fail(e, "hipFuncSetAttribute(rs_scatter)");
-    e = hipMemsetAsync(dvary, 0, sizeof(unsigned long long), stream);
-    if (e == hipSuccess) {
-        const unsigned vb = (unsigned)std::min<size_t>((n + 255) / 256, (size_t)device_cus() * 8);
-        rs_varying_bits<K><<<vb, 256, 0, stream>>>(keys_in, n, dvary);
-        e = hipMemcpyAsync(&hvary, dvary, sizeof(hvary), hipMemcpyDeviceToHost, stream);
-    }
-    if (e == hipSuccess) e = hipStreamSynchronize(stream);
-    if (e != hipSuccess) return hip_fail(e, "radix sort: varying bits");
     const K *ksrc = keys_in;
     const uint32_t *vsrc = vals_in;
+    bool moved = false;
     for (int p = 0; p < passes; ++p) {
         const int shift = begin_bit + 8 * p;
-        if (((hvary >> shift) & 255ull) == 0) continue;
+        if (((vary >> shift) & 255ull) == 0) continue;
         rs_hist<K><<<blocks, 64 * RS_WPB, 0, stream>>>(ksrc, n, shift, counts, n_tiles);
         exclusive_scan_enqueue<uint32_t>(counts, counts, m, sums, stream);
         K *kdst = (ksrc == keys_out) ? ktmp : keys_out;
@@ -304,15 +303,48 @@
         if (e != hipSuccess) return hip_fail(e, "radix sort pass");
         ksrc = kdst;
         vsrc = vdst;
-    }
+        moved = true;
+    }
+    if (PAIRS && !vals_in && !moved) return fail(GNNMP_EINVAL, "radix sort: identity payloads need at least one live pass");
     if (ksrc != keys_out) {
         e = hipMemcpyAsync(keys_out, ksrc, sizeof(K) * n, hipMemcpyDeviceToDevice, stream);
         if (e == hipSuccess && PAIRS) e = hipMemcpyAsync(vals_out, vsrc, sizeof(uint32_t) * n, hipMemcpyDeviceToDevice, stream);
         if (e != hipSuccess) return hip_fail(e, "radix sort copy-out");
     }
-    e = hipStreamSynchronize(stream);
+    return GNNMP_OK;
+}
+
+template <class K, bool PAIRS>
+static int radix_sort_impl(const K *keys_in, K *keys_out, const uint32_t *vals_in, uint32_t *vals_out, size_t n, int begin_bit,
+                           int end_bit, hipStream_t stream) {
+    if (n == 0) return GNNMP_OK;
+    if (n >= ((size_t)1 << 32)) return fail(GNNMP_EUNSUPPORTED, "radix sort: %zu elements exceed the 32-bit offset tables", n);
+    const RadixWs<K, PAIRS> lay(n);
+    DevBuf<unsigned char> arena;
+    hipError_t e = arena.alloc(lay.bytes() + 256);
+    if (e != hipSuccess) return hip_fail(e, "hipMalloc(radix sort temporaries)");
+    unsigned long long *dvary = reinterpret_cast<unsigned long long *>(arena.get() + lay.bytes()), hvary = 0;
+    e = hipMemsetAsync(dvary, 0, sizeof(unsigned long long), stream);
+    if (e == hipSuccess) {
+        const unsigned vb = (unsigned)std::min<size_t>((n + 255) / 256, (size_t)device_cus() * 8);
+        rs_varying_bits<K><<<vb, 256, 0, stream>>>(keys_in, n, dvary);
+        e = hipMemcpyAsync(&hvary, dvary, sizeof(hvary), hipMemcpyDeviceToHost, stream);
+    }
+    if (e == hipSuccess) e = setup_wait(stream);
+    if (e != hipSuccess) return hip_fail(e, "radix sort: varying bits");
+    GNNMP_TRY((radix_sort_enqueue<K, PAIRS>(keys_in, keys_out, vals_in, vals_out, n, begin_bit, end_bit, hvary, arena.get(), stream)));
+    e = setup_wait(stream);
     if (e != hipSuccess) return hip_fail(e, "radix sort");
     return GNNMP_OK;
+}
+
+size_t radix_sort_pairs_u32_workspace(size_t n) { return RadixWs<uint32_t, true>(n).bytes(); }
+int radix_sort_pairs_u32_ws(const uint32_t *keys_in, uint32_t *keys_out, const uint32_t *vals_in, uint32_t *vals_out, size_t n,
+                            uint32_t live_bits, void *ws, hipStream_t stream) {
+    if (n == 0) return GNNMP_OK;
+    if (n >= ((size_t)1 << 32)) return fail(GNNMP_EUNSUPPORTED, "radix sort: %zu elements exceed the 32-bit offset tables", n);
+    return radix_sort_enqueue<uint32_t, true>(keys_in, keys_out, vals_in, vals_out, n, 0, 32, live_bits, static_cast<unsigned char *>(ws),
+                                              stream);
 }
 
 int radix_sort_pairs_u32(const uint32_t *keys_in, uint32_t *keys_out, const uint32_t *vals_in, uint32_t *vals_out, size_t n,
diff --git a/graphneuralnetworks.jl_amd/gnnmp/_lib.py b/graphneuralnetworks.jl_amd/gnnmp/_lib.py
--- a/graphneuralnetworks.jl_amd/gnnmp/_lib.py
+++ b/graphneuralnetworks.jl_amd/gnnmp/_lib.py
@@ -51,7 +51,7 @@
     "gnnmp_random_walk_pe_f32",
     "gnnmp_edge_conv_f32", "gnnmp_edge_conv_grad_f32", "gnnmp_cg_conv_grad_f32",
     "gnnmp_tune", "gnnmp_tune_get", "gnnmp_debug_mock_device", "gnnmp_debug_device_once", "gnnmp_debug_plan_block", "gnnmp_debug_pool_pick",
-    "gnnmp_debug_random_walk_pe_f32", "gnnmp_debug_dense_route",
+    "gnnmp_debug_random_walk_pe_f32", "gnnmp_debug_dense_route", "gnnmp_debug_setup_counters",
 )
 
 
@@ -259,6 +259,7 @@
         "gnnmp_cg_conv_grad_f32": [vp, vp, ctypes.POINTER(CGConvGradJob), i64, vp],
         "gnnmp_debug_random_walk_pe_f32": [vp, ctypes.POINTER(RwpeJob), i64, vp],
         "gnnmp_debug_dense_route": [ctypes.POINTER(i)],
+        "gnnmp_debug_setup_counters": [ctypes.POINTER(i64)],
     }
     for name, args in sig.items():
         try:
diff --git a/graphneuralnetworks.jl_amd/gnnmp/graph.py b/graphneuralnetworks.jl_amd/gnnmp/graph.py
--- a/graphneuralnetworks.jl_amd/gnnmp/graph.py
+++ b/graphneuralnetworks.jl_amd/gnnmp/graph.py
@@ -38,6 +38,8 @@
         if rc == L.EBOUNDS:
             raise AssertionError(lib.gnnmp_last_error().decode())
         L.check(rc)
+        self._pooled = True
+        self._last_stream = torch.cuda.current_stream()
         info = (ctypes.c_int64 * 8)()
         L.check(lib.gnnmp_plan_info(self._h, info))
         self.n_src, self.n_dst, self.n_edges, self.n_total = info[0], info[1], info[2], info[3]
@@ -56,6 +58,8 @@
         if rc == L.EBOUNDS:
             raise AssertionError(self._lib.gnnmp_last_error().decode())
         L.check(rc)
+        self._pooled = True
+        self._last_stream = torch.cuda.current_stream()
         info = (ctypes.c_int64 * 8)()
         L.check(self._lib.gnnmp_plan_info(self._h, info))
         self.n_src, self.n_dst, self.n_edges, self.n_total = info[0], info[1], info[2], info[3]
diff --git a/graphneuralnetworks.jl_amd/gnnmp/knobs.py b/graphneuralnetworks.jl_amd/gnnmp/knobs.py
--- a/graphneuralnetworks.jl_amd/gnnmp/knobs.py
+++ b/graphneuralnetworks.jl_amd/gnnmp/knobs.py
@@ -37,4 +37,5 @@
     SPLIT_DIRECT_STORES = 32
     NO_WREG = 64
     TWO_KERNEL_FOLD = 128
+    HOST_PLAN_TABLES = 256
     WREG_SMALL = 512
diff --git a/include/gnnmp.h b/include/gnnmp.h
--- a/include/gnnmp.h
+++ b/include/gnnmp.h
@@ -429,6 +429,7 @@
 int gnnmp_debug_pool_pick(const uint64_t *caps, int n, uint64_t bytes);
 int gnnmp_debug_random_walk_pe_f32(gnnmp_graph_t *plan_t, const gnnmp_rwpe_t *job, int64_t lds_budget_bytes, gnnmp_stream_t stream);
 int gnnmp_debug_dense_route(int info[8]);
+int gnnmp_debug_setup_counters(int64_t counts[3]);
 
 #ifdef __cplusplus
 }
```

Measured after the change: 12.74 billion edges/s (median of 4 runs). No clear change (+1.7%).
